# starlingonearth/MASt3R-SLAM-Quality-dualTSDF

Hardware: AMD Instinct MI355X
Metric: SLAM frames/sec (infer+match+TSDF+GN) @512x384 (higher is better)
Workload: dtype bf16

## Files before the change

include/mslam_hip.h:

```cpp
#ifndef MSLAM_HIP_H
#define MSLAM_HIP_H

#include <stddef.h>
#include <stdint.h>

#ifdef __cplusplus
extern "C" {
#endif

#define MSLAM_OK 0
#define MSLAM_EINVAL (-1)
#define MSLAM_EHIP (-2)
#define MSLAM_ENOMEM (-3)
#define MSLAM_ENODEV (-4)

const char* mslam_last_error(void);
int mslam_abi_version(void);
int mslam_device_check(void);


int mslam_iter_proj(const float* rays_img_with_grad, const float* pts_3d_norm,
                    const float* p_init, float* p_new, uint8_t* converged, int b, int h, int w,
                    int n, int max_iter, float lambda_init, float cost_thresh, void* stream);

int mslam_refine_matches(const uint16_t* D11, const uint16_t* D21, const int64_t* p1,
                         int64_t* p1_new, int b, int h, int w, int n, int fdim, int radius,
                         int dilation_max, void* stream);

int mslam_prep_iter_proj(const float* X11, const float* X21, const int64_t* idx_init,
                         float* rays_img_with_grad, float* pts_3d_norm, float* p_init, int b, int h,
                         int w, void* stream);

int mslam_match_occlusion(const float* X11, const float* X21, const float* p, int64_t* p1,
                          uint8_t* valid, int b, int h, int w, float dist_thresh, void* stream);

int mslam_pixel_to_lin(const int64_t* p1, int64_t* idx, int b, int n, int w, void* stream);

size_t mslam_gn_workspace_bytes(int num_poses, int num_edges, int num_points, int local_edges);

int mslam_gauss_newton_rays(float* Twc, const float* Xs, const float* Cs, const int64_t* ii,
                            const int64_t* jj, const int64_t* idx_ii2jj, const uint8_t* valid_match,
                            const float* Q, int num_poses, int num_points, int num_edges,
                            float sigma_ray, float sigma_dist, float C_thresh, float Q_thresh,
                            int max_iter, float delta_thresh, float* dx, void* workspace,
                            size_t workspace_bytes, void* stream);

int mslam_gauss_newton_calib(float* Twc, const float* Xs, const float* Cs, const float* K,
                             const int64_t* ii, const int64_t* jj, const int64_t* idx_ii2jj,
                             const uint8_t* valid_match, const float* Q, int num_poses, int num_points,
                             int num_edges, int height, int width, int pixel_border, float z_eps,
                             float sigma_pixel, float sigma_depth, float C_thresh, float Q_thresh,
                             int max_iter, float delta_thresh, float* dx, void* workspace,
                             size_t workspace_bytes, void* stream);

int mslam_gauss_newton_points(float* Twc, const float* Xs, const float* Cs, const int64_t* ii,
                              const int64_t* jj, const int64_t* idx_ii2jj, const uint8_t* valid_match,
                              const float* Q, int num_poses, int num_points, int num_edges,
                              float sigma_point, float C_thresh, float Q_thresh, int max_iter,
                              float delta_thresh, float* dx, void* workspace, size_t workspace_bytes,
                              void* stream);

int mslam_gn_begin(const int64_t* ii, const int64_t* jj, int num_poses, int num_edges, int num_points,
                   void* workspace, size_t workspace_bytes, void* stream);
int mslam_gn_compact(const float* Xs, const float* Cs, const int64_t* idx_ii2jj, const uint8_t* valid_match,
                     const float* Q, int num_poses, int num_points, int num_edges, int edge_begin,
                     int edge_count, float C_thresh, float Q_thresh, void* workspace, size_t workspace_bytes,
                     void* stream);
int mslam_gn_compact_at(const float* Xs, const float* Cs, const int64_t* idx_ii2jj, const uint8_t* valid_match,
                        const float* Q, int num_poses, int num_points, int num_edges, int edge_begin, int edge_count,
                        int slot_begin, int range_count, float C_thresh, float Q_thresh, void* workspace,
                        size_t workspace_bytes, void* stream);
int mslam_gn_accumulate(int kind, const float* Twc, const float* K, int num_poses, int num_points,
                        int num_edges, int edge_begin, int edge_count, float sigma_a, float sigma_b,
                        int height, int width, int pixel_border, float z_eps, float* Hs, float* gs,
                        void* workspace, size_t workspace_bytes, void* stream);
int mslam_gn_solve_retract(const float* Hs, const float* gs, int num_poses, int num_edges,
                           int num_points, float* Twc, float* dx, float delta_thresh, void* workspace,
                           size_t workspace_bytes, void* stream);
int mslam_gn_status(int* status4, int num_poses, int num_edges, int num_points, void* workspace,
                    size_t workspace_bytes, void* stream);

int mslam_sim3_act(const float* T, const float* X, float* Y, int num_poses, long long pts_per_pose,
                   int broadcast_pose, void* stream);
int mslam_sim3_op(int op, const float* A, const float* B, float* out, int n, int bcast_a, int bcast_b,
                  void* stream);

size_t mslam_tsdf_table_bytes(uint64_t capacity);
int mslam_tsdf_table_init(void* table, size_t table_bytes, uint64_t capacity, void* stream);

size_t mslam_tsdf_integrate_workspace_bytes(int n_points, double voxel_size, double trunc, double step_scale);
int mslam_tsdf_integrate(void* table, uint64_t capacity, const float* points_world, const double* conf,
                         const float* cam_origin, int n_points, double voxel_size, double trunc,
                         double max_weight, double step_scale, int shard_id, int num_shards,
                         void* workspace, size_t workspace_bytes, void* stream);

int mslam_tsdf_rehash(void* old_table, uint64_t old_capacity, void* new_table, uint64_t new_capacity, void* stream);
int mslam_tsdf_header(void* table, uint64_t capacity, uint32_t* out8_host, void* stream);

int mslam_tsdf_dump(void* table, uint64_t capacity, int64_t* keys, double* tsdf, double* weight,
                    uint32_t max_out, void* stream);

int mslam_tsdf_query(void* table, uint64_t capacity, const float* points, int n, double voxel_size,
                     double min_weight, double* value, double* grad, uint8_t* status, void* stream);

int mslam_tsdf_pose_step(void* table, uint64_t capacity, const float* points, const float* conf, int n,
                         float* pose, int points_in_camera_frame, double voxel_size, double min_weight,
                         double lambda, double damping, int update_pose, double* H_out, double* b_out,
                         int* used_out, void* workspace, size_t workspace_bytes, void* stream);

int mslam_tsdf_lookup7(void* table, uint64_t capacity, const float* points, int n, const float* pose,
                       double voxel_size, double* out, void* stream);
int mslam_tsdf_query_lookup(const double* lookup, int n, double voxel_size, double min_weight, double* value,
                            double* grad, uint8_t* status, void* stream);
int mslam_tsdf_pose_step_lookup(const double* lookup, const float* points, const float* conf, int n, float* pose,
                                int points_in_camera_frame, double voxel_size, double min_weight, double lambda,
                                double damping, int update_pose, double* H_out, double* b_out, int* used_out,
                                void* workspace, size_t workspace_bytes, void* stream);

size_t mslam_tsdf_mesh_workspace_bytes(uint64_t capacity);
int mslam_tsdf_mesh_keys(void* table, uint64_t capacity, double min_weight, int64_t* sort_keys, void* stream);
int mslam_tsdf_mesh_count(void* table, uint64_t capacity, double min_weight, double level, const int64_t* sorted_keys,
                          const int64_t* order, int32_t* counts, void* workspace, size_t workspace_bytes, void* stream);
int mslam_tsdf_mesh_emit(void* table, uint64_t capacity, double voxel_size, double min_weight, double level,
                         const int64_t* sorted_keys, const int64_t* order, const int64_t* vbase, const int64_t* fbase,
                         void* workspace, size_t workspace_bytes, float* vertices, float* normals, int32_t* faces,
                         int64_t n_vertices, int64_t n_faces, void* stream);
int mslam_tsdf_load(void* table, uint64_t capacity, const int64_t* keys, const double* tsdf, const double* weight,
                    int n, void* stream);

size_t mslam_tsdf_render_workspace_bytes(uint64_t capacity);
int mslam_tsdf_render_blocks(void* table, uint64_t capacity, double min_weight, void* workspace, size_t workspace_bytes,
                             void* stream);
int mslam_tsdf_render(void* table, uint64_t capacity, const float* rays, int h, int w, const float* pose8,
                      double voxel_size, double min_weight, double level, double near, double far, double step, int skip,
                      const void* workspace, size_t workspace_bytes, float* range, float* normal, uint8_t* hit,
                      void* stream);

size_t mslam_tsdf_color_bytes(uint64_t capacity);
int mslam_tsdf_color_init(void* color, size_t color_bytes, uint64_t capacity, void* stream);
int mslam_tsdf_integrate_color(void* table, uint64_t capacity, void* color, const float* points_world,
                               const double* conf, const float* rgb, const float* cam_origin, int n_points,
                               double voxel_size, double trunc, double step_scale, void* stream);
int mslam_tsdf_color_rehash(void* old_table, uint64_t old_capacity, const void* old_color, void* new_table,
                            uint64_t new_capacity, void* new_color, void* stream);
int mslam_tsdf_color_dump(void* table, uint64_t capacity, const void* color, const int64_t* keys, int n, uint64_t* sums,
                          void* stream);
int mslam_tsdf_color_load(void* table, uint64_t capacity, void* color, const int64_t* keys, const uint64_t* sums, int n,
                          void* stream);
int mslam_tsdf_color_sample(void* table, uint64_t capacity, const void* color, const float* points, int n, int image_w,
                            double voxel_size, double default_r, double default_g, double default_b, float* out_rgb,
                            uint8_t* out_count, void* stream);

int mslam_mast3r_create(void** handle_out, const int* cfg9_host, void* const* weight_ptrs_host,
                        const long long* weight_numels_host, int n_weights, void* stream);
int mslam_mast3r_destroy(void* handle);
size_t mslam_mast3r_workspace_bytes(void* handle, int batch, int H, int W);

int mslam_mast3r_encode(void* handle, const float* img, int batch, int H, int W, float* feat_out,
                        void* workspace, size_t workspace_bytes, void* stream);

int mslam_mast3r_decode(void* handle, const float* feat1, const float* feat2, int batch, int H, int W,
                        float* X1, float* C1, float* D1, float* Q1, float* X2, float* C2, float* D2,
                        float* Q2, float* dec_last1, float* dec_last2, void* workspace,
                        size_t workspace_bytes, void* stream);

size_t mslam_track_workspace_bytes(int n_points);
int mslam_track_pose(int use_calib, float* T_rel, const float* Xf, const float* Xk, const int64_t* idx_f2k,
                     const float* Qk, const uint8_t* valid, int n_points, const float* K, int width,
                     int height, float sigma_a, float sigma_b, float huber, int pixel_border, float z_eps,
                     int first_iter, int max_iters, float rel_error, float delta_norm, void* status_out, void* workspace,
                     size_t workspace_bytes, void* stream);

size_t mslam_track_prepare_workspace_bytes(int n_points);
int mslam_track_prepare(const int64_t* idx_f2k, const uint8_t* valid_match, const float* Qff, const float* Qkf,
                        const float* Cf_sum, float inv_nf, const float* Ck_sum, float inv_nk, float C_conf, float Q_conf,
                        int n_points, const float* T_WCk, const float* T_WCf, float* Qk, float* Ck_avg,
                        uint8_t* valid_opt, uint8_t* valid_kf, float* T_rel, void* workspace, size_t workspace_bytes,
                        void* stream);
int mslam_track_verdict(const void* prepare_workspace, const void* status, int n_points, float* verdict6, void* stream);
int mslam_track_fuse(const float* T_WCk, const float* T_rel, const float* Xkf, const float* Ckf, const float* X_canon,
                     const float* C, int n_points, float* T_WCf, float* X_new, float* C_new, void* stream);

int mslam_gemm_bf16(const void* A, const void* W, const float* bias, const void* residual_f32, void* out,
                    int M, int N, int K, int act, int out_is_bf16, void* stream);
int mslam_gemm_tile_override(int M, int N, int K, int cfg);
int mslam_gemm_profile_begin(int M, int N, int K, int max_samples);
int mslam_gemm_profile_end(double* avg_us, double* min_us, int* samples);
int mslam_conv2d_nhwc_bf16(const void* in, const void* W, const float* bias, const void* residual_bf16,
                           void* out_bf16, int B, int H, int Wd, int Cin, int Cout, int ks, int stride,
                           int relu_in, int act, void* stream);
int mslam_attention_bf16(const void* Q, const void* K, const void* VT, void* O, int batch, int heads,
                         int nq, int nk, void* stream);
int mslam_layernorm_f32(const float* x, const float* w, const float* b, void* out_bf16, float* out_f32,
                        int rows, int D, float eps, void* stream);

size_t mslam_tsdf_local_workspace_bytes(int n_points);
int mslam_tsdf_local_build(const float* X_world, const float* C, const float* origin, const float* xyz_min,
                           const float* xyz_max, int n_points, int nx, int ny, int nz, double voxel_size,
                           double trunc, float min_confidence, float* tsdf, float* weights, void* workspace,
                           size_t workspace_bytes, void* stream);
int mslam_tsdf_local_raycast(const float* tsdf, int nx, int ny, int nz, const float* xyz_min,
                             const float* xyz_max, const float* X_original, const int64_t* sel_pix, int n_sel,
                             int n_samples, float max_displacement, float* surf, uint8_t* hit, void* stream);

int mslam_quality_reduce_grid(const float* x, const float* y, const uint8_t* valid, int h, int w, int ps, int mode,
                              double c_thr, double q_thr, float* out, void* stream);
int mslam_quality_classify(const float* delta_cov, const float* r, const float* u, int n, float thr_zr, float thr_zu,
                           float thr_dc, int64_t* cls, float* pri, void* stream);

int mslam_room_pair(const float* ki, const float* kj, int batch, int h, int w, int n_frames, double fx, double fy,
                    double cx, double cy, double noise, const double* Wm_3x24, const double* phase_24, float* X1,
                    float* C1, float* D1, float* Q1, float* X2, float* C2, float* D2, float* Q2, void* stream);

int mslam_remap_bilinear_u8(const uint8_t* src, int src_h, int src_w, int channels, const float* mapx,
                            const float* mapy, uint8_t* dst, int dst_h, int dst_w, void* stream);

int mslam_gemm_f64(const void* A, int a_is_f32, const void* B, int b_is_f32, int b_transposed, const double* centre,
                   const double* bias, double* out, int M, int N, int K, void* stream);

int mslam_asmk_aggregate(const float* des, const float* centroids, const int64_t* assign, const int64_t* uniq_words,
                         uint32_t* sig_out, int n_des, int m_assign, int dim, int n_uniq, int n_centroids, void* stream);
int mslam_asmk_search(const int32_t* entry_word, const uint32_t* entry_sig, const int32_t* img_start, int n_images,
                      const int32_t* q_words, const uint32_t* q_sig, int n_q, int sig_words, float similarity_threshold,
                      float alpha, double* scores, void* stream);

#ifdef __cplusplus
}
#endif
#endif
```

mast3r-slam-quality-dualtsdf_amd/csrc/gemm.h:

```cpp
#pragma once
#include <hip/hip_runtime.h>
#include <stdint.h>

namespace mslam {

typedef __bf16 bf16;

enum GemmAct { ACT_NONE = 0, ACT_GELU = 1, ACT_RELU = 2 };
enum GemmKind { KIND_NONE = 0, KIND_F32 = 1, KIND_BF16 = 2 };
enum GemmEpi {
  EPI_PLAIN = 0,
  EPI_ATTN = 1,
  EPI_CONVT = 2,
};

struct GemmArgs {
  const bf16* A;
  const bf16* W;
  int M, N, K;
  int lda;
  int a_conv, cB, cH, cW, cC, cKs, cStride, cPad, cHo, cWo;
  int a_relu;
  const float* bias;
  int act;
  const void* res1; int res1_kind; int ldr1;
  const void* res2; int res2_kind; int ldr2;
  void* out; int out_kind; int ldc;
  int epi;
  bf16* q_out; bf16* k_out; bf16* vt_out;
  int sec_base;
  int sec_dim;
  int heads;
  int ntok;
  int tok_w;
  int kv_ntok;
  const float* rope_cos; const float* rope_sin;
  float q_scale;
  int ct_s, ct_cout, ct_h, ct_w;
  int groups;
  const bf16* W1; const float* bias1;
  size_t a_gstride;
  size_t out_gbytes, res1_gbytes, res2_gbytes;
  size_t qkv_gstride;
  const void* pf_ptr[2]; size_t pf_bytes[2];
  unsigned* pf_sink;
};

constexpr int kGemmPrefetchBlocks = 64;

int launch_gemm(const GemmArgs& a, hipStream_t stream);
int gemm_profile_begin(int M, int N, int K, int max_samples);
int gemm_profile_end(double* avg_us, double* min_us, int* samples);
int gemm_tile_override(int M, int N, int K, int cfg, bool conv);

}
```

mast3r-slam-quality-dualtsdf_amd/csrc/gemm.hip:

```cpp
#include <stdlib.h>
#include <mutex>
#include <unordered_map>
#include <vector>
#include "common.h"
#include "gemm.h"

namespace mslam {

int launch_gemm_t64(const GemmArgs& a, int stages, hipStream_t s);
int launch_gemm_t128(const GemmArgs& a, int waves, int stages, hipStream_t s);
int launch_gemm_t128x64(const GemmArgs& a, int stages, hipStream_t s);
int launch_gemm_t256(const GemmArgs& a, int bn, hipStream_t s);
int launch_gemm_t192(const GemmArgs& a, hipStream_t s);
int launch_gemm_t256w8(const GemmArgs& a, hipStream_t s);
int launch_gemm_8p(const GemmArgs& a, hipStream_t s);
bool gemm8p_supports(const GemmArgs& a);

static std::mutex g_tile_mu;
static inline uint64_t tile_key(int M, int N, int K, bool conv = false) {
  return (uint64_t)M | ((uint64_t)N << 22) | ((uint64_t)K << 42) | ((uint64_t)conv << 63);
}
static std::unordered_map<uint64_t, int> g_tile_override = {
    {tile_key(3072, 3072, 1024), 1262},
    {tile_key(3072, 768, 3072), 643},
    {tile_key(6144, 3072, 768), 1282},
    {tile_key(3072, 4096, 1024), 2192},
    {tile_key(6144, 4096, 1024), 1282},
    {tile_key(9216, 4096, 1024), 1282},
    {tile_key(9216, 1024, 4096), 8256},
    {tile_key(4608, 4096, 1024), 1282},
};

int gemm_tile_override(int M, int N, int K, int cfg, bool conv) {
  std::lock_guard<std::mutex> lk(g_tile_mu);
  if (cfg > 0) g_tile_override[tile_key(M, N, K, conv)] = cfg;
  else g_tile_override.erase(tile_key(M, N, K, conv));
  return 0;
}

static std::mutex g_prof_mu;
static struct {
  bool on = false;
  int M = 0, N = 0, K = 0, cap = 0, n = 0;
  std::vector<hipEvent_t> ev;
} g_prof;

int gemm_profile_begin(int M, int N, int K, int max_samples) {
  std::lock_guard<std::mutex> lk(g_prof_mu);
  MSLAM_REQUIRE(!g_prof.on, "gemm_profile_begin: already profiling");
  MSLAM_REQUIRE(max_samples > 0 && max_samples <= 65536, "gemm_profile_begin: max_samples out of range");
  g_prof.ev.resize(2 * (size_t)max_samples);
  for (auto& e : g_prof.ev) {
    int rc = check_hip(hipEventCreate(&e), "hipEventCreate");
    if (rc) return rc;
  }
  g_prof.M = M; g_prof.N = N; g_prof.K = K; g_prof.cap = max_samples; g_prof.n = 0;
  g_prof.on = true;
  return MSLAM_OK;
}

int gemm_profile_end(double* avg_us, double* min_us, int* samples) {
  std::lock_guard<std::mutex> lk(g_prof_mu);
  MSLAM_REQUIRE(g_prof.on, "gemm_profile_end: not profiling");
  g_prof.on = false;
  double sum = 0.0, mn = 1e30;
  int rc = MSLAM_OK;
  for (int i = 0; i < g_prof.n && !rc; i++) {
    float ms = 0.0f;
    rc = check_hip(hipEventSynchronize(g_prof.ev[2 * i + 1]), "hipEventSynchronize");
    if (!rc) rc = check_hip(hipEventElapsedTime(&ms, g_prof.ev[2 * i], g_prof.ev[2 * i + 1]), "hipEventElapsedTime");
    sum += 1e3 * ms;
    if (1e3 * ms < mn) mn = 1e3 * ms;
  }
  if (samples) *samples = g_prof.n;
  if (avg_us) *avg_us = g_prof.n ? sum / g_prof.n : 0.0;
  if (min_us) *min_us = g_prof.n ? mn : 0.0;
  for (auto& e : g_prof.ev) (void)hipEventDestroy(e);
  g_prof.ev.clear();
  return rc;
}

static int launch_gemm_impl(const GemmArgs& a, hipStream_t stream);

int launch_gemm(const GemmArgs& a, hipStream_t stream) {
  int slot = -1;
  if (g_prof.on) {
    std::lock_guard<std::mutex> lk(g_prof_mu);
    if (g_prof.on && !a.a_conv && a.groups <= 1 && a.M == g_prof.M && a.N == g_prof.N && a.K == g_prof.K &&
        g_prof.n < g_prof.cap) {
      slot = g_prof.n++;
      (void)hipEventRecord(g_prof.ev[2 * slot], stream);
    }
  }
  const int rc = launch_gemm_impl(a, stream);
  if (slot >= 0) (void)hipEventRecord(g_prof.ev[2 * slot + 1], stream);
  return rc;
}

static int launch_gemm_impl(const GemmArgs& a, hipStream_t stream) {
  MSLAM_REQUIRE(a.M > 0 && a.N > 0 && a.K > 0, "gemm: empty problem %dx%dx%d", a.M, a.N, a.K);
  MSLAM_REQUIRE(a.K % 8 == 0, "gemm: K=%d must be a multiple of 8", a.K);
  MSLAM_REQUIRE(!a.a_conv || a.cC % 8 == 0, "gemm: conv channels %d must be a multiple of 8", a.cC);
  MSLAM_REQUIRE(a.a_conv || a.lda % 8 == 0, "gemm: lda=%d must be a multiple of 8", a.lda);
  MSLAM_REQUIRE(!a.a_relu || a.a_conv, "gemm: ReLU-on-load is only built for the implicit-conv view");
  MSLAM_REQUIRE(((uintptr_t)a.A & 15) == 0 && ((uintptr_t)a.W & 15) == 0, "gemm: A and W must be 16-byte aligned");
  const size_t a_bytes = a.a_conv ? (size_t)a.cB * a.cH * a.cW * a.cC * 2 : ((size_t)(a.M - 1) * a.lda + a.K) * 2;
  MSLAM_REQUIRE(a_bytes < (1ull << 31) && (size_t)a.N * a.K * 2 < (1ull << 31), "gemm: operand larger than 2 GiB");
  MSLAM_REQUIRE(a.epi != EPI_ATTN || (a.sec_dim % 64 == 0 && a.ntok % 4 == 0 && a.kv_ntok % 4 == 0),
                "gemm: attention epilogue needs 64-wide heads and token counts divisible by 4");
  static int forced = -2;
  if (forced == -2) {
    const char* e = getenv("MSLAM_GEMM");
    forced = e ? atoi(e) : -1;
  }
  MSLAM_REQUIRE(a.groups <= 2 && (a.groups < 2 || (a.W1 && !a.a_conv)), "gemm: bad group description");
  const long ngrp = a.groups > 1 ? 2 : 1;
  auto blocks = [&](int bm, int bn) { return ngrp * ((a.M + bm - 1) / bm) * ((a.N + bn - 1) / bn); };
  int cfg = forced;
  if (cfg < 0 && a.groups <= 1 && a.M < (1 << 22) && a.N < (1 << 20) && a.K < (1 << 20)) {
    static const bool log_shapes = getenv("MSLAM_GEMM_LOG") != nullptr;
    static std::unordered_map<uint64_t, int> seen;
    std::lock_guard<std::mutex> lk(g_tile_mu);
    const uint64_t key = tile_key(a.M, a.N, a.K, a.a_conv != 0);
    auto it = g_tile_override.find(key);
    if (it != g_tile_override.end()) cfg = it->second;
    if (log_shapes && seen.emplace(key, 1).second) fprintf(stderr, "mslam_gemm_shape conv=%d %d %d %d\n", (int)(a.a_conv != 0), a.M, a.N, a.K);
  }
  if (cfg < 0) {
    const bool narrow = a.N <= 128 || (a.N > 256 && a.N <= 384);
    if (narrow && blocks(256, 128) >= 128) cfg = 2128;
    else if (blocks(256, 256) >= 128) cfg = 2256;
    else if (blocks(128, 128) >= 256) cfg = 1282;
    else if (blocks(64, 64) >= 512) cfg = 642;
    else if (a.K >= 2048) cfg = 644;
    else cfg = 643;
  }
  switch (cfg) {
    case 642: return launch_gemm_t64(a, 2, stream);
    case 643: return launch_gemm_t64(a, 3, stream);
    case 644: return launch_gemm_t64(a, 4, stream);
    case 1262: return launch_gemm_t128x64(a, 2, stream);
    case 1263: return launch_gemm_t128x64(a, 3, stream);
    case 1242: return launch_gemm_t128(a, 4, 2, stream);
    case 1282: return launch_gemm_t128(a, 8, 2, stream);
    case 1283: return launch_gemm_t128(a, 8, 3, stream);
    case 2128: return launch_gemm_t256(a, 128, stream);
    case 2256: return launch_gemm_t256(a, 256, stream);
    case 2192: return launch_gemm_t192(a, stream);
    case 2258: return launch_gemm_t256w8(a, stream);
    case 8256: return gemm8p_supports(a) ? launch_gemm_8p(a, stream) : launch_gemm_t256(a, 256, stream);
    default: MSLAM_REQUIRE(false, "gemm: unknown configuration %d", cfg);
  }
}

}
```

mast3r-slam-quality-dualtsdf_amd/csrc/gemm_kernel.h:

```cpp
#pragma once
#include <stdlib.h>
#include <type_traits>
#include <utility>
#include "common.h"
#include "gemm.h"

namespace mslam {

typedef __attribute__((ext_vector_type(8))) __bf16 bf16x8;
typedef __attribute__((ext_vector_type(8))) short short8;
typedef __attribute__((ext_vector_type(16))) float f32x16;
typedef __attribute__((ext_vector_type(4))) unsigned int u32x4_t;

constexpr int BK = 64;
#ifndef MSLAM_GEMM_ABLATE
#define MSLAM_GEMM_ABLATE 0
#endif
constexpr unsigned kOob = 0x80000000u;

#define MSLAM_LDS_PTR(p) ((__attribute__((address_space(3))) void*)(p))

__device__ __forceinline__ float bf16_to_f32(bf16 v) { return (float)v; }

template <int... Is, typename F>
__device__ __forceinline__ void static_for_impl(std::integer_sequence<int, Is...>, F&& f) {
  (f(std::integral_constant<int, Is>{}), ...);
}
template <int N, typename F>
__device__ __forceinline__ void static_for(F&& f) {
  static_for_impl(std::make_integer_sequence<int, N>{}, f);
}

__device__ __forceinline__ float gelu_erf(float x) {
  const float z = fabsf(x) * 0.70710678118654752f;
  const float t = __builtin_amdgcn_rcpf(fmaf(0.3275911f, z, 1.0f));
  float p = fmaf(1.061405429f, t, -1.453152027f);
  p = fmaf(p, t, 1.421413741f);
  p = fmaf(p, t, -0.284496736f);
  p = fmaf(p, t, 0.254829592f);
  const float erfc_z = p * t * __builtin_amdgcn_exp2f(-1.4426950408889634f * z * z);
  const float one_plus_erf = (x >= 0.0f) ? 2.0f - erfc_z : erfc_z;
  return 0.5f * x * one_plus_erf;
}

typedef __attribute__((ext_vector_type(2))) float f32x2;
__device__ __forceinline__ f32x2 gelu_erf2(f32x2 x) {
  const f32x2 ax = __builtin_elementwise_abs(x);
  const f32x2 z = ax * 0.70710678118654752f;
  const f32x2 den = __builtin_elementwise_fma(f32x2{0.3275911f, 0.3275911f}, z, f32x2{1.0f, 1.0f});
  const f32x2 t = {__builtin_amdgcn_rcpf(den[0]), __builtin_amdgcn_rcpf(den[1])};
  f32x2 p = __builtin_elementwise_fma(f32x2{1.061405429f, 1.061405429f}, t, f32x2{-1.453152027f, -1.453152027f});
  p = __builtin_elementwise_fma(p, t, f32x2{1.421413741f, 1.421413741f});
  p = __builtin_elementwise_fma(p, t, f32x2{-0.284496736f, -0.284496736f});
  p = __builtin_elementwise_fma(p, t, f32x2{0.254829592f, 0.254829592f});
  const f32x2 a = (z * -1.4426950408889634f) * z;
  const f32x2 e = {__builtin_amdgcn_exp2f(a[0]), __builtin_amdgcn_exp2f(a[1])};
  const f32x2 erfc_z = (p * t) * e;
  const f32x2 two_minus = f32x2{2.0f, 2.0f} - erfc_z;
  const f32x2 one_plus_erf = {x[0] >= 0.0f ? two_minus[0] : erfc_z[0], x[1] >= 0.0f ? two_minus[1] : erfc_z[1]};
  return (x * 0.5f) * one_plus_erf;
}

template <int N>
__device__ __forceinline__ void wait_vmcnt() {
  static_assert(N >= 0 && N < 64, "vmcnt is 6 bits");
  __builtin_amdgcn_s_waitcnt((N & 15) | ((N >> 4) << 14) | 0x0F70);
}

template <int WM, int WN, int MI, int NI, int S, bool CONV>
__global__ __launch_bounds__(64 * WM * WN) void gemm_bf16_kernel(GemmArgs g) {
  constexpr int NW = WM * WN;
  constexpr int BM = 32 * MI * WM, BN = 32 * NI * WN;
  static_assert(NW % 2 == 0 && BM % (8 * NW) == 0 && BN % (8 * NW) == 0, "DMA pieces must divide over the waves");
  constexpr int A_PC = BM / (8 * NW), B_PC = BN / (8 * NW);
  constexpr int N_DMA = A_PC + B_PC;
  constexpr int STAGE = (BM + BN) * 128;
  static_assert(S >= 2 && S <= 8, "ring depth");
  static_assert(N_DMA * (S - 1) < 64, "vmcnt range");
  extern __shared__ __attribute__((aligned(1024))) unsigned char smem[];

  const unsigned nbm = (g.M + BM - 1) / BM, nbn = (g.N + BN - 1) / BN;
  const unsigned ngrp = g.groups > 1 ? 2u : 1u;
  if (blockIdx.x >= nbm * nbn * ngrp) {
    typedef __attribute__((ext_vector_type(4))) unsigned int u32x4;
    const unsigned pb = blockIdx.x - nbm * nbn * ngrp, npb = gridDim.x - nbm * nbn * ngrp;
    u32x4 acc = {0u, 0u, 0u, 0u};
#pragma unroll
    for (int r = 0; r < 2; r++) {
      const char* base = reinterpret_cast<const char*>(g.pf_ptr[r]);
      const size_t bytes = g.pf_bytes[r] & ~(size_t)15;
      const size_t stride = (size_t)npb * (64 * NW) * 16;
      size_t off = ((size_t)pb * (64 * NW) + threadIdx.x) * 16;
      for (; off + 15 * stride < bytes; off += 16 * stride) {
        u32x4 v[16];
#pragma unroll
        for (int k = 0; k < 16; k++) v[k] = *reinterpret_cast<const u32x4*>(base + off + k * stride);
#pragma unroll
        for (int k = 0; k < 16; k++) acc ^= v[k];
      }
      for (; off < bytes; off += stride) acc ^= *reinterpret_cast<const u32x4*>(base + off);
    }
    if ((acc[0] ^ acc[1]) == 0x9e3779b9u && (acc[2] ^ acc[3]) == 0x7f4a7c15u && g.pf_sink) *g.pf_sink = acc[0];
    return;
  }
  const unsigned logical = xcd_remap(blockIdx.x, nbm * nbn * ngrp);
  const unsigned prob = logical / (nbm * nbn), tile = logical - prob * (nbm * nbn);
  if (prob) {
    g.A += g.a_gstride; g.W = g.W1; g.bias = g.bias1;
    g.out = reinterpret_cast<char*>(g.out) + g.out_gbytes;
    if (g.res1) g.res1 = reinterpret_cast<const char*>(g.res1) + g.res1_gbytes;
    if (g.res2) g.res2 = reinterpret_cast<const char*>(g.res2) + g.res2_gbytes;
    if (g.epi == EPI_ATTN) { g.q_out += g.qkv_gstride; g.k_out += g.qkv_gstride; g.vt_out += g.qkv_gstride; }
  }
  constexpr unsigned GM = 1024 / BM;
  const unsigned per_group = GM * nbn, grp = tile / per_group, in_grp = tile - grp * per_group;
  const unsigned gsz = min(nbm - grp * GM, GM);
  const int m0 = (grp * GM + in_grp % gsz) * BM, n0 = (in_grp / gsz) * BN;

  const int t = threadIdx.x, lane = t & 63;
  const int wid = __builtin_amdgcn_readfirstlane(t >> 6);
  const int wm = wid / WN, wn = wid % WN;

  const int lcol = lane & 31;
  float bias_v[NI];
#pragma unroll
  for (int ni = 0; ni < NI; ni++) {
    const int col = n0 + wn * NI * 32 + ni * 32 + lcol;
    bias_v[ni] = (g.bias && col < g.N) ? g.bias[g.epi == EPI_CONVT ? col / (g.ct_s * g.ct_s) : col] : 0.0f;
  }

  const int chunk = (lane & 7) ^ (4 * (wid & 1) + (lane >> 4));
  const size_t a_bytes = CONV ? (size_t)g.cB * g.cH * g.cW * g.cC * 2 : ((size_t)(g.M - 1) * g.lda + g.K) * 2;
  const __amdgpu_buffer_rsrc_t rsA = __builtin_amdgcn_make_buffer_rsrc((void*)g.A, 0, (int)a_bytes, 0x00020000);
  const __amdgpu_buffer_rsrc_t rsW =
      __builtin_amdgcn_make_buffer_rsrc((void*)g.W, 0, (int)((size_t)g.N * g.K * 2), 0x00020000);
  unsigned a_off[A_PC];
  int a_iy0[A_PC], a_ix0[A_PC];
#pragma unroll
  for (int i = 0; i < A_PC; i++) {
    const int m = m0 + (wid + NW * i) * 8 + (lane >> 3);
    if constexpr (CONV) {
      const int hw = g.cHo * g.cWo;
      const int b = m / hw, rem = m - b * hw;
      const int oy = rem / g.cWo, ox = rem - oy * g.cWo;
      a_iy0[i] = (m < g.M) ? oy * g.cStride - g.cPad : -(1 << 20);
      a_ix0[i] = ox * g.cStride - g.cPad;
      a_off[i] = (unsigned)b * (unsigned)(g.cH * g.cW * g.cC) * 2u;
    } else {
      a_off[i] = (m < g.M) ? ((unsigned)m * (unsigned)g.lda + (unsigned)chunk * 8u) * 2u : kOob;
      a_iy0[i] = a_ix0[i] = 0;
    }
  }
  unsigned b_off[B_PC];
#pragma unroll
  for (int i = 0; i < B_PC; i++) {
    const int n = n0 + (wid + NW * i) * 8 + (lane >> 3);
    b_off[i] = (n < g.N) ? ((unsigned)n * (unsigned)g.K + (unsigned)chunk * 8u) * 2u : kOob;
  }
  int c_cc = 0, c_dy = 0, c_dx = 0;
  if constexpr (CONV) {
    const int kk = chunk * 8, tap = kk / g.cC;
    c_cc = kk - tap * g.cC;
    c_dy = tap / g.cKs;
    c_dx = tap - c_dy * g.cKs;
  }

  const int nk = (g.K + BK - 1) / BK;
  auto issue = [&](int st, int kt) {
    if (MSLAM_GEMM_ABLATE == 1 && kt >= S - 1) return;
    unsigned char* sbase = smem + st * STAGE + wid * 1024;
    const int k0 = kt * BK;
    const unsigned k_bad = (unsigned)(g.K - 1 - (k0 + chunk * 8)) & kOob;
#pragma unroll
    for (int i = 0; i < A_PC; i++) {
      unsigned off;
      if constexpr (CONV) {
        const int iy = a_iy0[i] + c_dy, ix = a_ix0[i] + c_dx;
        const unsigned bad = (unsigned)(iy | (g.cH - 1 - iy) | ix | (g.cW - 1 - ix)) & kOob;
        off = (a_off[i] + (unsigned)((iy * g.cW + ix) * g.cC + c_cc) * 2u) | bad | k_bad;
      } else {
        off = (a_off[i] + (unsigned)k0 * 2u) | k_bad;
      }
      __builtin_amdgcn_raw_ptr_buffer_load_lds(rsA, MSLAM_LDS_PTR(sbase + i * (NW * 1024)), 16, off, 0, 0, 0);
    }
#pragma unroll
    for (int i = 0; i < B_PC; i++) {
      const unsigned off = (b_off[i] + (unsigned)k0 * 2u) | k_bad;
      __builtin_amdgcn_raw_ptr_buffer_load_lds(rsW, MSLAM_LDS_PTR(sbase + BM * 128 + i * (NW * 1024)), 16, off, 0, 0, 0);
    }
    if constexpr (CONV) {
      c_cc += BK;
      while (c_cc >= g.cC) {
        c_cc -= g.cC;
        if (++c_dx == g.cKs) { c_dx = 0; c_dy++; }
      }
    }
  };

  f32x16 acc[MI][NI];
#pragma unroll
  for (int mi = 0; mi < MI; mi++)
#pragma unroll
    for (int ni = 0; ni < NI; ni++)
#pragma unroll
      for (int r = 0; r < 16; r++) acc[mi][ni][r] = 0.0f;
#if MSLAM_GEMM_ABLATE == 4
  typedef __attribute__((ext_vector_type(4))) float f32x4q;
  f32x4q acc4[MI][NI][4];
#pragma unroll
  for (int mi = 0; mi < MI; mi++)
#pragma unroll
    for (int ni = 0; ni < NI; ni++)
#pragma unroll
      for (int r = 0; r < 4; r++) acc4[mi][ni][r] = f32x4q{0.0f, 0.0f, 0.0f, 0.0f};
#endif

  const int lr = lane & 31, kh = (lane >> 5) ^ ((lr >> 1) & 7);
  const unsigned fragA = (wm * MI * 32 + lr) * 128, fragB = BM * 128 + (wn * NI * 32 + lr) * 128;
  const bool relu_a = g.a_relu != 0;
  auto compute = [&](int st) {
    const unsigned char* sA = smem + st * STAGE + fragA;
    const unsigned char* sB = smem + st * STAGE + fragB;
    constexpr int KS = BK / 16, KG = (NW >= 16) ? 2 : KS;
#pragma unroll
    for (int kg = 0; kg < KS; kg += KG) {
      bf16x8 af[KG][MI], bfr[KG][NI];
#pragma unroll
      for (int k = 0; k < KG; k++) {
        const int so = ((2 * (kg + k)) ^ kh) * 16;
#pragma unroll
        for (int mi = 0; mi < MI; mi++) {
          if (MSLAM_GEMM_ABLATE == 3) af[k][mi] = __builtin_bit_cast(bf16x8, u32x4_t{(unsigned)so, 1u, 2u, 3u});
          else af[k][mi] = *reinterpret_cast<const bf16x8*>(sA + mi * 4096 + so);
        }
#pragma unroll
        for (int ni = 0; ni < NI; ni++) {
          if (MSLAM_GEMM_ABLATE == 3) bfr[k][ni] = __builtin_bit_cast(bf16x8, u32x4_t{(unsigned)so, 5u, 6u, 7u});
          else bfr[k][ni] = *reinterpret_cast<const bf16x8*>(sB + ni * 4096 + so);
        }
      }
      __builtin_amdgcn_sched_barrier(0);
#pragma unroll
      for (int k = 0; k < KG; k++) {
#pragma unroll
        for (int mi = 0; mi < MI; mi++) {
          if (CONV && relu_a) {
            const short8 z = {0, 0, 0, 0, 0, 0, 0, 0};
            af[k][mi] = __builtin_bit_cast(bf16x8, __builtin_elementwise_max(__builtin_bit_cast(short8, af[k][mi]), z));
          }
#pragma unroll
          for (int ni = 0; ni < NI; ni++) {
            if (MSLAM_GEMM_ABLATE == 2) {
              asm volatile("" ::"v"(af[k][mi]), "v"(bfr[k][ni]));
#if MSLAM_GEMM_ABLATE == 4
            } else if (true) {
              acc4[mi][ni][2 * (k & 1)] = __builtin_amdgcn_mfma_f32_16x16x32_bf16(af[k][mi], bfr[k][ni], acc4[mi][ni][2 * (k & 1)], 0, 0, 0);
              acc4[mi][ni][2 * (k & 1) + 1] = __builtin_amdgcn_mfma_f32_16x16x32_bf16(af[k][mi], bfr[k][ni], acc4[mi][ni][2 * (k & 1) + 1], 0, 0, 0);
#endif
            } else {
              acc[mi][ni] = __builtin_amdgcn_mfma_f32_32x32x16_bf16(af[k][mi], bfr[k][ni], acc[mi][ni], 0, 0, 0);
            }
          }
        }
      }
      if (kg + KG < KS) __builtin_amdgcn_sched_barrier(0);
    }
  };

#pragma unroll
  for (int s = 0; s < S - 1; s++)
    if (s < nk) issue(s, s);
  int kt = 0, st = 0, st_issue = S - 1;
  for (; kt < nk - (S - 2); kt++) {
    wait_vmcnt<N_DMA * (S - 2)>();
    __builtin_amdgcn_s_barrier();
    if (kt + S - 1 < nk) issue(st_issue, kt + S - 1);
    compute(st);
    st = (st + 1 == S) ? 0 : st + 1;
    st_issue = (st_issue + 1 == S) ? 0 : st_issue + 1;
  }
  for (; kt < nk; kt++) {
    const int behind = nk - 1 - kt;
    bool waited = false;
    if constexpr (S >= 4) {
      static_for<S - 3>([&](auto j_c) {
        constexpr int b = decltype(j_c)::value + 1;
        if (behind == b) { wait_vmcnt<N_DMA * b>(); waited = true; }
      });
    }
    if (!waited) wait_vmcnt<0>();
    __builtin_amdgcn_s_barrier();
    compute(st);
    st = (st + 1 == S) ? 0 : st + 1;
  }

#if MSLAM_GEMM_ABLATE == 4
#pragma unroll
  for (int mi = 0; mi < MI; mi++)
#pragma unroll
    for (int ni = 0; ni < NI; ni++)
#pragma unroll
      for (int r = 0; r < 16; r++) acc[mi][ni][r] = acc4[mi][ni][r >> 2][r & 3];
#endif
  __builtin_amdgcn_s_barrier();
  constexpr int TBS = 40;
  float* tb = reinterpret_cast<float*>(smem) + wid * (32 * TBS);
  typedef __attribute__((ext_vector_type(8))) __bf16 bf16x8s;
  const int half = lane >> 5;
  const int lrow0 = lane >> 2, lc = (lane & 3) * 8;
  const bool wide_plain = g.epi == EPI_PLAIN && (g.N & 7) == 0 && (g.ldc & 7) == 0 && (g.ldr1 & 7) == 0 && (g.ldr2 & 7) == 0;
  const bool wide_attn = g.epi == EPI_ATTN && (g.ntok & 31) == 0 && (g.kv_ntok & 31) == 0;
  auto load8 = [&](const void* base, int kind, size_t idx, float (&o)[8]) {
    if (kind == KIND_F32) {
      const float4 p = *reinterpret_cast<const float4*>(reinterpret_cast<const float*>(base) + idx);
      const float4 q = *reinterpret_cast<const float4*>(reinterpret_cast<const float*>(base) + idx + 4);
      o[0] += p.x; o[1] += p.y; o[2] += p.z; o[3] += p.w; o[4] += q.x; o[5] += q.y; o[6] += q.z; o[7] += q.w;
    } else if (kind == KIND_BF16) {
      const bf16x8s p = *reinterpret_cast<const bf16x8s*>(reinterpret_cast<const bf16*>(base) + idx);
#pragma unroll
      for (int e = 0; e < 8; e++) o[e] += (float)p[e];
    }
  };
  static_for<MI>([&](auto mi_c) {
    static_for<NI>([&](auto ni_c) {
      constexpr int mi = decltype(mi_c)::value, ni = decltype(ni_c)::value;
      const f32x16 accv = acc[mi][ni];
      const int col_base = n0 + wn * NI * 32 + ni * 32;
      const int col = col_base + lcol;
      const int row_base0 = m0 + wm * MI * 32 + mi * 32;
      const int row_base = row_base0 + 4 * half;
      const bool col_ok = col < g.N;
      const float bias = bias_v[ni];
      float v[16];
      static_for<8>([&](auto r_c) {
        constexpr int r = 2 * decltype(r_c)::value;
        f32x2 x = {accv[r] + bias, accv[r + 1] + bias};
        if (g.act == ACT_GELU) x = gelu_erf2(x);
        else if (g.act == ACT_RELU) x = __builtin_elementwise_max(x, f32x2{0.0f, 0.0f});
        v[r] = x[0]; v[r + 1] = x[1];
      });
      if (wide_plain) {
        static_for<16>([&](auto r_c) {
          constexpr int r = decltype(r_c)::value;
          tb[((r & 3) + 8 * (r >> 2) + 4 * half) * TBS + lcol] = v[r];
        });
#pragma unroll
        for (int j = 0; j < 2; j++) {
          const int lrow = lrow0 + 16 * j;
          const float4 p = *reinterpret_cast<const float4*>(tb + lrow * TBS + lc);
          const float4 q = *reinterpret_cast<const float4*>(tb + lrow * TBS + lc + 4);
          const int row = row_base0 + lrow, c0 = col_base + lc;
          if (row < g.M && c0 < g.N) {
            float o[8] = {p.x, p.y, p.z, p.w, q.x, q.y, q.z, q.w};
            load8(g.res1, g.res1_kind, (size_t)row * g.ldr1 + c0, o);
            load8(g.res2, g.res2_kind, (size_t)row * g.ldr2 + c0, o);
            if (g.out_kind == KIND_F32) {
              float* dst = reinterpret_cast<float*>(g.out) + (size_t)row * g.ldc + c0;
              *reinterpret_cast<float4*>(dst) = make_float4(o[0], o[1], o[2], o[3]);
              *reinterpret_cast<float4*>(dst + 4) = make_float4(o[4], o[5], o[6], o[7]);
            } else {
              bf16x8s pk;
#pragma unroll
              for (int e = 0; e < 8; e++) pk[e] = (bf16)o[e];
              *reinterpret_cast<bf16x8s*>(reinterpret_cast<bf16*>(g.out) + (size_t)row * g.ldc + c0) = pk;
            }
          }
        }
      } else if (wide_attn) {
        const int sec = g.sec_base + col_base / g.sec_dim;
        const int cs = col_base % g.sec_dim;
        const int head = cs >> 6, f0 = cs & 63;
        const int ntok = (sec == 0) ? g.ntok : g.kv_ntok;
        const int b = row_base0 / ntok, nb = row_base0 - b * ntok;
        if (sec < 2) {
          const bool use_y = f0 < 32;
          const bool lo = lcol < 16;
          const float scale = (sec == 0) ? g.q_scale : 1.0f;
          static_for<16>([&](auto r_c) {
            constexpr int r = decltype(r_c)::value;
            const int n = nb + 4 * half + (r & 3) + 8 * (r >> 2);
            const float partner = __shfl_xor(v[r], 16, 64);
            const int p = use_y ? n / g.tok_w : n % g.tok_w;
            const float c = g.rope_cos[p * 16 + (lcol & 15)], sn = g.rope_sin[p * 16 + (lcol & 15)];
            const float x = lo ? (v[r] * c - partner * sn) : (v[r] * c + partner * sn);
            tb[((r & 3) + 8 * (r >> 2) + 4 * half) * TBS + lcol] = x * scale;
          });
          bf16* dst = (sec == 0) ? g.q_out : g.k_out;
#pragma unroll
          for (int j = 0; j < 2; j++) {
            const int lrow = lrow0 + 16 * j;
            const float4 p = *reinterpret_cast<const float4*>(tb + lrow * TBS + lc);
            const float4 q = *reinterpret_cast<const float4*>(tb + lrow * TBS + lc + 4);
            if (row_base0 + lrow < g.M && col_base < g.N) {
              bf16x8s pk;
              pk[0] = (bf16)p.x; pk[1] = (bf16)p.y; pk[2] = (bf16)p.z; pk[3] = (bf16)p.w;
              pk[4] = (bf16)q.x; pk[5] = (bf16)q.y; pk[6] = (bf16)q.z; pk[7] = (bf16)q.w;
              *reinterpret_cast<bf16x8s*>(dst + (((size_t)b * g.heads + head) * ntok + nb + lrow) * 64 + f0 + lc) = pk;
            }
          }
        } else {
          static_for<16>([&](auto r_c) {
            constexpr int r = decltype(r_c)::value;
            tb[((r & 3) + 8 * (r >> 2) + 4 * half) * TBS + lcol] = v[r];
          });
          const int tok0 = half * 16;
          if (row_base0 + tok0 < g.M && col_ok) {
            bf16x8s pk0, pk1;
#pragma unroll
            for (int e = 0; e < 8; e++) {
              pk0[e] = (bf16)tb[(tok0 + e) * TBS + lcol];
              pk1[e] = (bf16)tb[(tok0 + 8 + e) * TBS + lcol];
            }
            bf16* dst = g.vt_out + (((size_t)b * g.heads + head) * 64 + f0 + lcol) * ntok + nb + tok0;
            *reinterpret_cast<bf16x8s*>(dst) = pk0;
            *reinterpret_cast<bf16x8s*>(dst + 8) = pk1;
          }
        }
      } else {
        if (g.epi == EPI_PLAIN) {
          static_for<16>([&](auto r_c) {
            constexpr int r = decltype(r_c)::value;
            const int row = row_base + (r & 3) + 8 * (r >> 2);
            if (row < g.M && col_ok) {
              float x = v[r];
              if (g.res1_kind == KIND_F32) x += reinterpret_cast<const float*>(g.res1)[(size_t)row * g.ldr1 + col];
              else if (g.res1_kind == KIND_BF16) x += bf16_to_f32(reinterpret_cast<const bf16*>(g.res1)[(size_t)row * g.ldr1 + col]);
              if (g.res2_kind == KIND_F32) x += reinterpret_cast<const float*>(g.res2)[(size_t)row * g.ldr2 + col];
              else if (g.res2_kind == KIND_BF16) x += bf16_to_f32(reinterpret_cast<const bf16*>(g.res2)[(size_t)row * g.ldr2 + col]);
              if (g.out_kind == KIND_F32) reinterpret_cast<float*>(g.out)[(size_t)row * g.ldc + col] = x;
              else reinterpret_cast<bf16*>(g.out)[(size_t)row * g.ldc + col] = (bf16)x;
            }
          });
        } else if (g.epi == EPI_ATTN) {
          const int sec = g.sec_base + col / g.sec_dim;
          const int cs = col % g.sec_dim;
          const int head = cs >> 6, f = cs & 63;
          const int ntok = (sec == 0) ? g.ntok : g.kv_ntok;
          if (sec < 2) {
            const bool use_y = f < 32;
            const bool lo = (f & 31) < 16;
            bf16* dst = (sec == 0) ? g.q_out : g.k_out;
            const float scale = (sec == 0) ? g.q_scale : 1.0f;
            static_for<16>([&](auto r_c) {
              constexpr int r = decltype(r_c)::value;
              const int row = row_base + (r & 3) + 8 * (r >> 2);
              const float partner = __shfl_xor(v[r], 16, 64);
              if (row < g.M && col_ok) {
                const int b = row / ntok, n = row - b * ntok;
                const int p = use_y ? n / g.tok_w : n % g.tok_w;
                const float c = g.rope_cos[p * 16 + (f & 15)], sn = g.rope_sin[p * 16 + (f & 15)];
                const float x = lo ? (v[r] * c - partner * sn) : (v[r] * c + partner * sn);
                dst[(((size_t)b * g.heads + head) * ntok + n) * 64 + f] = (bf16)(x * scale);
              }
            });
          } else {
            static_for<4>([&](auto gq_c) {
              constexpr int gq = decltype(gq_c)::value;
              const int row = row_base + 8 * gq;
              if (row < g.M && col_ok) {
                const int b = row / ntok, n = row - b * ntok;
                typedef __attribute__((ext_vector_type(4))) __bf16 bf16x4;
                bf16x4 pk;
                pk[0] = (bf16)v[4 * gq + 0]; pk[1] = (bf16)v[4 * gq + 1];
                pk[2] = (bf16)v[4 * gq + 2]; pk[3] = (bf16)v[4 * gq + 3];
                *reinterpret_cast<bf16x4*>(g.vt_out + (((size_t)b * g.heads + head) * 64 + f) * ntok + n) = pk;
              }
            });
          }
        } else {
          const int ss = g.ct_s * g.ct_s;
          const int co = col / ss, ij = col - co * ss, i = ij / g.ct_s, j = ij - i * g.ct_s;
          static_for<16>([&](auto r_c) {
            constexpr int r = decltype(r_c)::value;
            const int row = row_base + (r & 3) + 8 * (r >> 2);
            if (row < g.M && col_ok) {
              const int hw = g.ct_h * g.ct_w;
              const int b = row / hw, rem = row - b * hw, y = rem / g.ct_w, x = rem - y * g.ct_w;
              const size_t o = (((size_t)b * g.ct_h * g.ct_s + (size_t)y * g.ct_s + i) * (g.ct_w * g.ct_s) +
                                (size_t)x * g.ct_s + j) * g.ct_cout + co;
              reinterpret_cast<bf16*>(g.out)[o] = (bf16)v[r];
            }
          });
        }
      }
    });
  });
}


template <int WM, int WN, int MI, int NI, int S>
int launch_cfg(const GemmArgs& a, hipStream_t stream) {
  constexpr int NW = WM * WN, BM = 32 * MI * WM, BN = 32 * NI * WN;
  constexpr size_t ring = (size_t)S * (BM + BN) * 128, patch = (size_t)NW * 32 * 40 * sizeof(float);
  constexpr size_t shmem = ring > patch ? ring : patch;
  static_assert(shmem <= 160 * 1024, "LDS budget");
  const unsigned blocks = (unsigned)(((a.M + BM - 1) / BM) * ((a.N + BN - 1) / BN)) * (a.groups > 1 ? 2u : 1u) +
                          ((a.pf_bytes[0] + a.pf_bytes[1]) ? (unsigned)kGemmPrefetchBlocks : 0u);
  static bool attr_set = false;
  if (!attr_set) {
    const void* fns[2] = {(const void*)gemm_bf16_kernel<WM, WN, MI, NI, S, false>,
                          (const void*)gemm_bf16_kernel<WM, WN, MI, NI, S, true>};
    for (const void* fn : fns) {
      int rc = check_hip(hipFuncSetAttribute(fn, hipFuncAttributeMaxDynamicSharedMemorySize, (int)shmem), "gemm: attr");
      if (rc) return rc;
    }
    attr_set = true;
  }
  if (!a.a_conv)
    hipLaunchKernelGGL((gemm_bf16_kernel<WM, WN, MI, NI, S, false>), dim3(blocks), dim3(64 * NW), shmem, stream, a);
  else
    hipLaunchKernelGGL((gemm_bf16_kernel<WM, WN, MI, NI, S, true>), dim3(blocks), dim3(64 * NW), shmem, stream, a);
  return check_hip(hipGetLastError(), "gemm launch");
}

}
```

mast3r-slam-quality-dualtsdf_amd/csrc/gemm_t256.hip:

```cpp
#include "gemm_kernel.h"
namespace mslam {
int launch_gemm_t192(const GemmArgs& a, hipStream_t s) { return launch_cfg<2, 4, 3, 2, 2>(a, s); }

int launch_gemm_t256w8(const GemmArgs& a, hipStream_t s) { return launch_cfg<2, 4, 4, 2, 2>(a, s); }

int launch_gemm_t256(const GemmArgs& a, int bn, hipStream_t s) {
  if (bn == 256) return launch_cfg<4, 4, 2, 2, 2>(a, s);
  return launch_cfg<4, 2, 2, 2, 2>(a, s);
}
}
```

mast3r-slam-quality-dualtsdf_amd/csrc/mast3r.hip:

```cpp
#include <stdlib.h>
#include <vector>
#include "common.h"
#include "gemm.h"

namespace mslam {

int launch_attention(const bf16* Q, const bf16* K, const bf16* VT, bf16* O, int batch, int heads, int nq, int nk,
                     hipStream_t stream);

template <typename TIN>
__global__ __launch_bounds__(256) void layernorm_kernel(const TIN* __restrict__ x, const float* __restrict__ w,
                                                        const float* __restrict__ b, bf16* __restrict__ out_bf,
                                                        float* __restrict__ out_f, int rows, int D, float eps) {
  constexpr int MAXV = 32;
  const int row = blockIdx.x * 4 + (threadIdx.x >> 6);
  const int lane = threadIdx.x & 63;
  if (row >= rows) return;
  const TIN* xr = x + (size_t)row * D;
  float v[MAXV];
  float s = 0.0f;
#pragma unroll
  for (int c = 0; c < MAXV; c++) {
    const int i = lane + 64 * c;
    v[c] = (i < D) ? (float)xr[i] : 0.0f;
    s += v[c];
  }
#pragma unroll
  for (int off = 32; off > 0; off >>= 1) s += __shfl_xor(s, off, 64);
  const float mean = s / (float)D;
  float q = 0.0f;
#pragma unroll
  for (int c = 0; c < MAXV; c++) {
    const float d = (lane + 64 * c < D) ? v[c] - mean : 0.0f;
    q += d * d;
  }
#pragma unroll
  for (int off = 32; off > 0; off >>= 1) q += __shfl_xor(q, off, 64);
  const float rstd = rsqrtf(q / (float)D + eps);
#pragma unroll
  for (int c = 0; c < MAXV; c++) {
    const int i = lane + 64 * c;
    if (i < D) {
      const float y = (v[c] - mean) * rstd * w[i] + b[i];
      if (out_bf) out_bf[(size_t)row * D + i] = (bf16)y;
      if (out_f) out_f[(size_t)row * D + i] = y;
    }
  }
}

typedef __attribute__((ext_vector_type(4))) __bf16 bf16x4;

template <int NV>
__device__ __forceinline__ void ln_load_stats(const float* xrow, int lane, float4 (&v)[NV], float& mean, float& rstd,
                                              float eps) {
  constexpr int D = NV * 256;
  const float4* xr = reinterpret_cast<const float4*>(xrow);
#pragma unroll
  for (int c = 0; c < NV; c++) v[c] = xr[lane + 64 * c];
  float s = 0.0f;
#pragma unroll
  for (int c = 0; c < NV; c++) s += (v[c].x + v[c].y) + (v[c].z + v[c].w);
#pragma unroll
  for (int off = 32; off > 0; off >>= 1) s += __shfl_xor(s, off, 64);
  mean = s / (float)D;
  float q = 0.0f;
#pragma unroll
  for (int c = 0; c < NV; c++) {
    const float dx = v[c].x - mean, dy = v[c].y - mean, dz = v[c].z - mean, dw = v[c].w - mean;
    q += (dx * dx + dy * dy) + (dz * dz + dw * dw);
  }
#pragma unroll
  for (int off = 32; off > 0; off >>= 1) q += __shfl_xor(q, off, 64);
  rstd = rsqrtf(q / (float)D + eps);
}

__device__ __forceinline__ float4 ln_affine(const float4& v, float mean, float rstd, const float4& w, const float4& b) {
  float4 y;
  y.x = (v.x - mean) * rstd * w.x + b.x;
  y.y = (v.y - mean) * rstd * w.y + b.y;
  y.z = (v.z - mean) * rstd * w.z + b.z;
  y.w = (v.w - mean) * rstd * w.w + b.w;
  return y;
}

__device__ __forceinline__ void ln_store_bf16(bf16* out_row, int idx, const float4& y) {
  bf16x4 o;
  o[0] = (bf16)y.x; o[1] = (bf16)y.y; o[2] = (bf16)y.z; o[3] = (bf16)y.w;
  reinterpret_cast<bf16x4*>(out_row)[idx] = o;
}

template <int NV>
__global__ __launch_bounds__(256) void layernorm_vec_kernel(const float* __restrict__ x, const float* __restrict__ w,
                                                            const float* __restrict__ b, bf16* __restrict__ out_bf,
                                                            float* __restrict__ out_f, int rows, float eps) {
  constexpr int D = NV * 256;
  const int row = blockIdx.x * 4 + (threadIdx.x >> 6);
  const int lane = threadIdx.x & 63;
  if (row >= rows) return;
  float4 v[NV], wv[NV], bv[NV];
  float mean, rstd;
#pragma unroll
  for (int c = 0; c < NV; c++) {
    wv[c] = reinterpret_cast<const float4*>(w)[lane + 64 * c];
    bv[c] = reinterpret_cast<const float4*>(b)[lane + 64 * c];
  }
  ln_load_stats<NV>(x + (size_t)row * D, lane, v, mean, rstd, eps);
#pragma unroll
  for (int c = 0; c < NV; c++) {
    const float4 y = ln_affine(v[c], mean, rstd, wv[c], bv[c]);
    if (out_bf) ln_store_bf16(out_bf + (size_t)row * D, lane + 64 * c, y);
    if (out_f) reinterpret_cast<float4*>(out_f + (size_t)row * D)[lane + 64 * c] = y;
  }
}

struct LnSet { const float* w; const float* b; };

template <int NV, bool CROSS>
__global__ __launch_bounds__(256) void layernorm_group_vec_kernel(const float* __restrict__ x, LnSet self0, LnSet self1,
                                                                  LnSet mem0, LnSet mem1, bf16* __restrict__ out_self,
                                                                  bf16* __restrict__ out_mem, int M, float eps) {
  constexpr int D = NV * 256;
  const int row = blockIdx.x * 4 + (threadIdx.x >> 6);
  const int lane = threadIdx.x & 63;
  if (row >= 2 * M) return;
  const int side = row >= M;
  float4 v[NV];
  float mean, rstd;
  ln_load_stats<NV>(x + (size_t)row * D, lane, v, mean, rstd, eps);
#pragma unroll
  for (int k = 0; k < (CROSS ? 2 : 1); k++) {
    const LnSet ps = (k == 0) ? (side ? self1 : self0) : (side ? mem0 : mem1);
    bf16* out = (k == 0) ? out_self + (size_t)row * D : out_mem + (size_t)(side ? row - M : row + M) * D;
#pragma unroll
    for (int c = 0; c < NV; c++) {
      const float4 wv = reinterpret_cast<const float4*>(ps.w)[lane + 64 * c];
      const float4 bv = reinterpret_cast<const float4*>(ps.b)[lane + 64 * c];
      ln_store_bf16(out, lane + 64 * c, ln_affine(v[c], mean, rstd, wv, bv));
    }
  }
}

static void launch_layernorm(const float* x, const float* w, const float* b, bf16* out_bf, float* out_f, int rows, int D,
                             float eps, hipStream_t s) {
  const dim3 grid((rows + 3) / 4), block(256);
  if (D == 1024) hipLaunchKernelGGL(layernorm_vec_kernel<4>, grid, block, 0, s, x, w, b, out_bf, out_f, rows, eps);
  else if (D == 768) hipLaunchKernelGGL(layernorm_vec_kernel<3>, grid, block, 0, s, x, w, b, out_bf, out_f, rows, eps);
  else hipLaunchKernelGGL(layernorm_kernel<float>, grid, block, 0, s, x, w, b, out_bf, out_f, rows, D, eps);
}

__global__ void cast_f32_bf16_kernel(const float* __restrict__ x, bf16* __restrict__ y, size_t n) {
  const size_t i = ((size_t)blockIdx.x * blockDim.x + threadIdx.x) * 4;
  if (i + 3 < n) {
    const float4 v = *reinterpret_cast<const float4*>(x + i);
    bf16x4 o;
    o[0] = (bf16)v.x; o[1] = (bf16)v.y; o[2] = (bf16)v.z; o[3] = (bf16)v.w;
    *reinterpret_cast<bf16x4*>(y + i) = o;
  } else {
    for (size_t k = i; k < n; k++) y[k] = (bf16)x[k];
  }
}

__global__ void patchify_kernel(const float* __restrict__ img, bf16* __restrict__ out, int B, int H, int W, int P) {
  const int nh = H / P, nw = W / P, K = 3 * P * P;
  const size_t total = (size_t)B * nh * nw * K;
  const size_t i = (size_t)blockIdx.x * blockDim.x + threadIdx.x;
  if (i >= total) return;
  const int k = (int)(i % K);
  const size_t tok = i / K;
  const int tx = (int)(tok % nw), ty = (int)((tok / nw) % nh), b = (int)(tok / ((size_t)nw * nh));
  const int c = k / (P * P), ky = (k / P) % P, kx = k % P;
  out[i] = (bf16)img[(((size_t)b * 3 + c) * H + ty * P + ky) * W + tx * P + kx];
}

__global__ void concat2_kernel(const bf16* __restrict__ a, int ca, const bf16* __restrict__ b, int cb,
                               bf16* __restrict__ out, size_t rows) {
  const int C = ca + cb;
  const size_t i = (size_t)blockIdx.x * blockDim.x + threadIdx.x;
  if (i >= rows * C) return;
  const size_t r = i / C;
  const int c = (int)(i % C);
  out[i] = c < ca ? a[r * ca + c] : b[r * cb + (c - ca)];
}

__global__ void upsample2x_kernel(const bf16* __restrict__ in, bf16* __restrict__ out, int B, int H, int W, int C) {
  const int Ho = 2 * H, Wo = 2 * W;
  const int c8 = C / 8;
  const size_t total = (size_t)B * Ho * Wo * c8;
  const size_t i = (size_t)blockIdx.x * blockDim.x + threadIdx.x;
  if (i >= total) return;
  const int cc = (int)(i % c8) * 8;
  const size_t pix = i / c8;
  const int ox = (int)(pix % Wo), oy = (int)((pix / Wo) % Ho), b = (int)(pix / ((size_t)Wo * Ho));
  const float sy = Ho > 1 ? (float)(H - 1) / (float)(Ho - 1) : 0.0f;
  const float sx = Wo > 1 ? (float)(W - 1) / (float)(Wo - 1) : 0.0f;
  const float fy = sy * oy, fx = sx * ox;
  const int y0 = min((int)fy, H - 1), x0 = min((int)fx, W - 1);
  const int y1 = min(y0 + 1, H - 1), x1 = min(x0 + 1, W - 1);
  const float wy = fy - y0, wx = fx - x0;
  typedef __attribute__((ext_vector_type(8))) __bf16 bf16x8;
  const bf16* base = in + (size_t)b * H * W * C + cc;
  const bf16x8 v00 = *reinterpret_cast<const bf16x8*>(base + ((size_t)y0 * W + x0) * C);
  const bf16x8 v01 = *reinterpret_cast<const bf16x8*>(base + ((size_t)y0 * W + x1) * C);
  const bf16x8 v10 = *reinterpret_cast<const bf16x8*>(base + ((size_t)y1 * W + x0) * C);
  const bf16x8 v11 = *reinterpret_cast<const bf16x8*>(base + ((size_t)y1 * W + x1) * C);
  bf16x8 o;
#pragma unroll
  for (int k = 0; k < 8; k++) {
    const float top = (float)v00[k] + wx * ((float)v01[k] - (float)v00[k]);
    const float bot = (float)v10[k] + wx * ((float)v11[k] - (float)v10[k]);
    o[k] = (bf16)(top + wy * (bot - top));
  }
  *reinterpret_cast<bf16x8*>(out + pix * C + cc) = o;
}

constexpr int kHP = 16;
__global__ __launch_bounds__(256) void head_post_kernel(const bf16* __restrict__ feat, int fc,
                                                        const float* __restrict__ w4, const float* __restrict__ b4,
                                                        const float* __restrict__ lf, int lf_ld, int desc_dim,
                                                        int B, int H, int W, float* __restrict__ X,
                                                        float* __restrict__ Cf, float* __restrict__ D,
                                                        float* __restrict__ Q) {
  typedef __attribute__((ext_vector_type(8))) __bf16 bf16x8;
  __shared__ float l_s[kHP * kHP][4];
  __shared__ __attribute__((aligned(16))) float d_s[kHP * kHP * 24];
  __shared__ __attribute__((aligned(16))) float x_s[kHP * kHP * 3];
  const int t = threadIdx.x;
  const int nw = W / kHP, nh = H / kHP;
  const int tok = blockIdx.x;
  const int b = tok / (nh * nw), ty = (tok / nw) % nh, tx = tok % nw;
  const size_t pix00 = ((size_t)b * H + (size_t)ty * kHP) * W + (size_t)tx * kHP;
  const int cg = t & 15, ppx = t >> 4;
  float wr[4][8];
#pragma unroll
  for (int o = 0; o < 4; o++)
#pragma unroll
    for (int k = 0; k < 8; k++) wr[o][k] = w4[o * fc + cg * 8 + k];
  for (int r = 0; r < kHP; r++) {
    const bf16x8 v = *reinterpret_cast<const bf16x8*>(feat + (pix00 + (size_t)r * W + ppx) * fc + cg * 8);
    float p[4] = {0.0f, 0.0f, 0.0f, 0.0f};
#pragma unroll
    for (int k = 0; k < 8; k++) {
      const float fv = (float)v[k];
#pragma unroll
      for (int o = 0; o < 4; o++) p[o] = fmaf(wr[o][k], fv, p[o]);
    }
#pragma unroll
    for (int off = 8; off > 0; off >>= 1)
#pragma unroll
      for (int o = 0; o < 4; o++) p[o] += __shfl_xor(p[o], off, 64);
    if (cg == 0) {
#pragma unroll
      for (int o = 0; o < 4; o++) l_s[r * kHP + ppx][o] = p[o] + b4[o];
    }
  }
  __syncthreads();
  const int py = t >> 4, px = t & 15;
  const float l0 = l_s[t][0], l1 = l_s[t][1], l2 = l_s[t][2], l3 = l_s[t][3];
  const float d = sqrtf(l0 * l0 + l1 * l1 + l2 * l2);
  const float sc = expm1f(d) / fmaxf(d, 1e-8f);
  x_s[t * 3 + 0] = l0 * sc; x_s[t * 3 + 1] = l1 * sc; x_s[t * 3 + 2] = l2 * sc;
  const size_t pix = pix00 + (size_t)py * W + px;
  Cf[pix] = 1.0f + expf(l3);
  const float* lp = lf + (size_t)tok * lf_ld + t;
  float dv[24];
  float nn = 0.0f;
#pragma unroll
  for (int c = 0; c < 24; c++) { dv[c] = lp[c * kHP * kHP]; nn = fmaf(dv[c], dv[c], nn); }
  const float inv = 1.0f / sqrtf(nn);
#pragma unroll
  for (int c = 0; c < 24; c++) d_s[t * 24 + c] = dv[c] * inv;
  Q[pix] = expf(lp[24 * kHP * kHP]);
  __syncthreads();
#pragma unroll
  for (int k = 0; k < 6; k++) {
    const int e = t + 256 * k, r = e / 96, q = e - r * 96;
    *reinterpret_cast<float4*>(D + (pix00 + (size_t)r * W) * 24 + q * 4) = *reinterpret_cast<const float4*>(d_s + r * 384 + q * 4);
  }
  if (t < 192) {
    const int r = t / 12, q = t - r * 12;
    *reinterpret_cast<float4*>(X + (pix00 + (size_t)r * W) * 3 + q * 4) = *reinterpret_cast<const float4*>(x_s + r * 48 + q * 4);
  }
}

__global__ __launch_bounds__(256) void head_post_generic_kernel(const bf16* __restrict__ feat, int fc,
                                                        const float* __restrict__ w4, const float* __restrict__ b4,
                                                        const float* __restrict__ lf, int lf_ld, int desc_dim, int P,
                                                        int B, int H, int W, float* __restrict__ X,
                                                        float* __restrict__ Cf, float* __restrict__ D,
                                                        float* __restrict__ Q) {
  const size_t pix = (size_t)blockIdx.x * 256 + threadIdx.x;
  if (pix >= (size_t)B * H * W) return;
  const int x = (int)(pix % W), y = (int)((pix / W) % H), b = (int)(pix / ((size_t)W * H));
  float l[4] = {b4[0], b4[1], b4[2], b4[3]};
  const bf16* f = feat + pix * fc;
  typedef __attribute__((ext_vector_type(8))) __bf16 bf16x8;
  for (int c = 0; c < fc; c += 8) {
    const bf16x8 v = *reinterpret_cast<const bf16x8*>(f + c);
#pragma unroll
    for (int k = 0; k < 8; k++) {
      const float fv = (float)v[k];
#pragma unroll
      for (int o = 0; o < 4; o++) l[o] = fmaf(w4[o * fc + c + k], fv, l[o]);
    }
  }
  const float d = sqrtf(l[0] * l[0] + l[1] * l[1] + l[2] * l[2]);
  const float sc = expm1f(d) / fmaxf(d, 1e-8f);
  X[pix * 3 + 0] = l[0] * sc; X[pix * 3 + 1] = l[1] * sc; X[pix * 3 + 2] = l[2] * sc;
  Cf[pix] = 1.0f + expf(l[3]);
  const int nw = W / P;
  const size_t tok = (size_t)b * (H / P) * nw + (size_t)(y / P) * nw + x / P;
  const float* lp = lf + tok * lf_ld + (y % P) * P + (x % P);
  float dv[32];
  float nn = 0.0f;
  for (int c = 0; c < desc_dim; c++) { dv[c] = lp[c * P * P]; nn = fmaf(dv[c], dv[c], nn); }
  const float inv = 1.0f / sqrtf(nn);
  for (int c = 0; c < desc_dim; c++) D[pix * desc_dim + c] = dv[c] * inv;
  Q[pix] = expf(lp[desc_dim * P * P]);
}

struct Lin { const bf16* W; const float* b; int out, in; };
struct Norm { const float* w; const float* b; int d; };

struct EncBlock { Norm n1; Lin qkv, proj; Norm n2; Lin fc1, fc2; };
struct DecBlock { Norm n1; Lin qkv, proj; Norm n2, ny; Lin pq, pkv, cproj; Norm n3; Lin fc1, fc2; };
struct Rcu { Lin c1, c2; };
struct Fusion { Rcu r1, r2; Lin out; bool has_r1; };
struct Head {
  Lin a00, a01, a10, a11, a20, a30, a31;
  Lin rn[4];
  Fusion fus[4];
  Lin h0, h2;
  const float* h4w; const float* h4b;
  Lin fc1, fc2;
};

struct Mast3rModel {
  int E, enc_depth, enc_heads, Dd, dec_depth, dec_heads, P, desc_dim, fd;
  Lin pe;
  std::vector<EncBlock> enc;
  Norm enc_norm;
  Lin dec_embed;
  std::vector<DecBlock> dec[2];
  Norm dec_norm;
  Head head[2];
  float* rope_cos = nullptr;
  float* rope_sin = nullptr;
  int rope_len = 0;
  int hooks[4];
  unsigned* pf_sink = nullptr;
  bool prefetch = true;
};

struct PtrFeed {
  void* const* ptrs;
  const long long* numels;
  int count, pos = 0;
  bool ok = true;
  void* take(long long expect, const char* what) {
    if (pos >= count) { if (ok) set_error("mast3r_create: ran out of weights at %s (#%d)", what, pos); ok = false; return nullptr; }
    if (numels[pos] != expect) {
      if (ok) set_error("mast3r_create: weight #%d (%s) has %lld elements, expected %lld", pos, what, numels[pos], expect);
      ok = false;
    }
    return ptrs[pos++];
  }
  Lin lin(int out, int in, bool bias, const char* what) {
    Lin l; l.out = out; l.in = in;
    l.W = (const bf16*)take((long long)out * in, what);
    l.b = bias ? (const float*)take(out, what) : nullptr;
    return l;
  }
  Norm norm(int d, const char* what) {
    Norm n; n.d = d;
    n.w = (const float*)take(d, what);
    n.b = (const float*)take(d, what);
    return n;
  }
};

struct Arena {
  char* base; size_t off = 0, cap; bool dry; bool overflow = false;
  size_t peak = 0;
  template <typename T> T* get(size_t n) {
    const size_t bytes = (n * sizeof(T) + 255) / 256 * 256;
    T* p = dry ? nullptr : reinterpret_cast<T*>(base + off);
    off += bytes;
    if (off > peak) peak = off;
    if (!dry && off > cap) { overflow = true; return reinterpret_cast<T*>(base); }
    return p;
  }
};

struct Ctx {
  const Mast3rModel* m;
  Arena ar;
  hipStream_t s;
  int rc = MSLAM_OK;
  bool dry() const { return ar.dry; }
  void fail(int r) { if (rc == MSLAM_OK) rc = r; }
};

static void dbg(Ctx& c, const char* what, int a = 0, int b = 0, int d = 0) {
  static const bool on = getenv("MSLAM_DEBUG") != nullptr;
  if (!on || c.dry()) return;
  fprintf(stderr, "[mslam] %s %d %d %d ...", what, a, b, d);
  fflush(stderr);
  hipError_t e = hipStreamSynchronize(c.s);
  fprintf(stderr, " %s\n", hipGetErrorString(e));
}

static void run_gemm(Ctx& c, GemmArgs& g) {
  if (c.dry() || c.rc) return;
  c.fail(launch_gemm(g, c.s));
  dbg(c, g.epi == EPI_ATTN ? "gemm_attn" : (g.a_conv ? "gemm_conv" : "gemm"), g.M, g.N, g.K);
}

struct Pf { const Lin* a = nullptr; const Lin* b = nullptr; };
static void set_pf(const Ctx& c, GemmArgs& g, const Pf& pf) {
  if (!c.m->prefetch) return;
  const Lin* l[2] = {pf.a, pf.b};
  for (int k = 0; k < 2; k++)
    if (l[k]) { g.pf_ptr[k] = l[k]->W; g.pf_bytes[k] = (size_t)l[k]->out * l[k]->in * sizeof(bf16); }
  g.pf_sink = c.m->pf_sink;
}

static GemmArgs dense_args(const bf16* A, int M, const Lin& l) {
  GemmArgs g = {};
  g.A = A; g.W = l.W; g.M = M; g.N = l.out; g.K = l.in; g.lda = l.in; g.bias = l.b;
  g.ldc = l.out; g.ldr1 = l.out; g.ldr2 = l.out;
  return g;
}

static void group2(GemmArgs& g, const Lin& l1, size_t a_gstride, size_t out_gbytes) {
  g.groups = 2; g.W1 = l1.W; g.bias1 = l1.b; g.a_gstride = a_gstride; g.out_gbytes = out_gbytes;
}

static void layernorm(Ctx& c, const float* x, const Norm& n, int rows, bf16* out_bf, float* out_f) {
  if (c.dry() || c.rc) return;
  launch_layernorm(x, n.w, n.b, out_bf, out_f, rows, n.d, 1e-6f, c.s);
  dbg(c, "layernorm", rows, n.d);
}

static void cast_bf16(Ctx& c, const float* x, bf16* y, size_t n) {
  if (c.dry() || c.rc) return;
  hipLaunchKernelGGL(cast_f32_bf16_kernel, dim3((unsigned)((n / 4 + 255) / 256 + 1)), dim3(256), 0, c.s, x, y, n);
  dbg(c, "cast", (int)n);
}

struct AttnBufs { bf16 *q, *k, *vt, *o; };

static void attn_project(Ctx& c, const bf16* A, int M, const Lin& l, int sec_base, int heads, int ntok, int kv_ntok,
                         int tok_w, const AttnBufs& ab, const Pf& pf = Pf(), const Lin* l1 = nullptr) {
  GemmArgs g = dense_args(A, M, l);
  set_pf(c, g, pf);
  g.epi = EPI_ATTN; g.sec_base = sec_base; g.sec_dim = heads * 64; g.heads = heads; g.ntok = ntok; g.kv_ntok = kv_ntok;
  g.tok_w = tok_w; g.q_out = ab.q; g.k_out = ab.k; g.vt_out = ab.vt; g.rope_cos = c.m->rope_cos;
  g.rope_sin = c.m->rope_sin; g.q_scale = 0.125f;
  if (l1) {
    group2(g, *l1, (size_t)M * l.in, 0);
    g.qkv_gstride = (size_t)(M / ntok) * heads * 64 * (sec_base == 0 ? ntok : kv_ntok);
  }
  run_gemm(c, g);
}

static void attention(Ctx& c, const AttnBufs& ab, int B, int heads, int nq, int nk) {
  if (c.dry() || c.rc) return;
  c.fail(launch_attention(ab.q, ab.k, ab.vt, ab.o, B, heads, nq, nk, c.s));
  dbg(c, "attention", B * heads, nq, nk);
}

static void linear_residual(Ctx& c, const bf16* A, int M, const Lin& l, float* x, const Pf& pf = Pf(),
                            const Lin* l1 = nullptr) {
  GemmArgs g = dense_args(A, M, l);
  set_pf(c, g, pf);
  g.res1 = x; g.res1_kind = KIND_F32; g.out = x; g.out_kind = KIND_F32;
  if (l1) {
    group2(g, *l1, (size_t)M * l.in, (size_t)M * l.out * sizeof(float));
    g.res1_gbytes = g.out_gbytes;
  }
  run_gemm(c, g);
}

static void linear_bf16(Ctx& c, const bf16* A, int M, const Lin& l, bf16* out, int act, const Pf& pf = Pf(),
                        const Lin* l1 = nullptr) {
  GemmArgs g = dense_args(A, M, l);
  set_pf(c, g, pf);
  g.out = out; g.out_kind = KIND_BF16; g.act = act;
  if (l1) group2(g, *l1, (size_t)M * l.in, (size_t)M * l.out * sizeof(bf16));
  run_gemm(c, g);
}

static void linear_f32(Ctx& c, const bf16* A, int M, const Lin& l, float* out) {
  GemmArgs g = dense_args(A, M, l);
  g.out = out; g.out_kind = KIND_F32;
  run_gemm(c, g);
}

struct BlockScratch { bf16* h; bf16* u; AttnBufs ab; };

static BlockScratch block_scratch(Ctx& c, int M, int D) {
  BlockScratch s;
  s.h = c.ar.get<bf16>((size_t)M * D);
  s.u = c.ar.get<bf16>((size_t)M * 4 * D);
  s.ab.q = c.ar.get<bf16>((size_t)M * D);
  s.ab.k = c.ar.get<bf16>((size_t)M * D);
  s.ab.vt = c.ar.get<bf16>((size_t)M * D);
  s.ab.o = c.ar.get<bf16>((size_t)M * D);
  return s;
}

static void mlp_residual(Ctx& c, float* x, int M, const Norm& n, const Lin& fc1, const Lin& fc2, BlockScratch& s,
                         const Pf& pf1 = Pf(), const Pf& pf2 = Pf()) {
  layernorm(c, x, n, M, s.h, nullptr);
  linear_bf16(c, s.h, M, fc1, s.u, ACT_GELU, pf1);
  linear_residual(c, s.u, M, fc2, x, pf2);
}

static void encode(Ctx& c, const float* img, int B, int H, int W, float* feat_out) {
  const Mast3rModel& m = *c.m;
  const int nh = H / m.P, nw = W / m.P, N = nh * nw, M = B * N, KP = 3 * m.P * m.P;
  bf16* patches = c.ar.get<bf16>((size_t)M * KP);
  float* x = c.ar.get<float>((size_t)M * m.E);
  BlockScratch s = block_scratch(c, M, m.E);
  if (!c.dry() && !c.rc) {
    const size_t total = (size_t)M * KP;
    hipLaunchKernelGGL(patchify_kernel, dim3((unsigned)((total + 255) / 256)), dim3(256), 0, c.s, img, patches, B, H, W,
                       m.P);
    dbg(c, "patchify", B, H, W);
  }
  linear_f32(c, patches, M, m.pe, x);
  for (int i = 0; i < m.enc_depth; i++) {
    const EncBlock& b = m.enc[i];
    const EncBlock* nb = i + 1 < m.enc_depth ? &m.enc[i + 1] : nullptr;
    layernorm(c, x, b.n1, M, s.h, nullptr);
    attn_project(c, s.h, M, b.qkv, 0, m.enc_heads, N, N, nw, s.ab, Pf{nb ? &nb->qkv : nullptr});
    attention(c, s.ab, B, m.enc_heads, N, N);
    linear_residual(c, s.ab.o, M, b.proj, x, Pf{nb ? &nb->proj : nullptr});
    mlp_residual(c, x, M, b.n2, b.fc1, b.fc2, s, Pf{nb ? &nb->fc1 : nullptr}, Pf{nb ? &nb->fc2 : nullptr});
  }
  layernorm(c, x, m.enc_norm, M, nullptr, feat_out);
}

static GemmArgs conv_args(const bf16* in, int B, int H, int W, int C, const Lin& l, int ks, int stride) {
  GemmArgs g = {};
  const int pad = ks / 2;
  const int Ho = (H + 2 * pad - ks) / stride + 1, Wo = (W + 2 * pad - ks) / stride + 1;
  g.A = in; g.W = l.W; g.M = B * Ho * Wo; g.N = l.out; g.K = ks * ks * C; g.bias = l.b;
  g.a_conv = 1; g.cB = B; g.cH = H; g.cW = W; g.cC = C; g.cKs = ks; g.cStride = stride; g.cPad = pad; g.cHo = Ho; g.cWo = Wo;
  g.ldc = l.out; g.ldr1 = l.out; g.ldr2 = l.out; g.out_kind = KIND_BF16;
  return g;
}

static bf16* conv(Ctx& c, const bf16* in, int B, int H, int W, int C, const Lin& l, int ks, int stride, int a_relu,
                  int act, const bf16* res1, const bf16* res2) {
  GemmArgs g = conv_args(in, B, H, W, C, l, ks, stride);
  bf16* out = c.ar.get<bf16>((size_t)g.M * l.out);
  g.out = out; g.a_relu = a_relu; g.act = act;
  if (res1) { g.res1 = res1; g.res1_kind = KIND_BF16; }
  if (res2) { g.res2 = res2; g.res2_kind = KIND_BF16; }
  run_gemm(c, g);
  return out;
}

static bf16* conv_transpose(Ctx& c, const bf16* in, int B, int H, int W, int C, const Lin& l, int s, int cout) {
  GemmArgs g = {};
  g.A = in; g.W = l.W; g.M = B * H * W; g.N = cout * s * s; g.K = C; g.lda = C; g.bias = l.b;
  g.epi = EPI_CONVT; g.ct_s = s; g.ct_cout = cout; g.ct_h = H; g.ct_w = W; g.out_kind = KIND_BF16;
  bf16* out = c.ar.get<bf16>((size_t)B * H * s * W * s * cout);
  g.out = out;
  run_gemm(c, g);
  return out;
}

static bf16* upsample2x(Ctx& c, const bf16* in, int B, int H, int W, int C) {
  bf16* out = c.ar.get<bf16>((size_t)B * 4 * H * W * C);
  if (!c.dry() && !c.rc) {
    const size_t total = (size_t)B * 4 * H * W * (C / 8);
    hipLaunchKernelGGL(upsample2x_kernel, dim3((unsigned)((total + 255) / 256)), dim3(256), 0, c.s, in, out, B, H, W, C);
    dbg(c, "upsample2x", H, W, C);
  }
  return out;
}

static bf16* rcu(Ctx& c, const bf16* x, int B, int H, int W, int C, const Rcu& r, const bf16* extra) {
  bf16* t = conv(c, x, B, H, W, C, r.c1, 3, 1,  1, ACT_RELU, nullptr, nullptr);
  return conv(c, t, B, H, W, C, r.c2, 3, 1, 0, ACT_NONE, x, extra);
}

static bf16* fusion(Ctx& c, const Fusion& f, const bf16* path, const bf16* layer, int B, int H, int W, int C) {
  const bf16* s = path;
  if (f.has_r1) s = rcu(c, layer, B, H, W, C, f.r1, path);
  bf16* r = rcu(c, s, B, H, W, C, f.r2, nullptr);
  bf16* o = conv(c, r, B, H, W, C, f.out, 1, 1, 0, ACT_NONE, nullptr, nullptr);
  return upsample2x(c, o, B, H, W, C);
}

struct HeadOut { float *X, *C, *D, *Q; };

static void run_head(Ctx& c, const Head& hd, const bf16* const toks[4], int B, int H, int W, const HeadOut& out) {
  const Mast3rModel& m = *c.m;
  const int nh = H / m.P, nw = W / m.P, M = B * nh * nw;
  bf16* t0 = conv(c, toks[0], B, nh, nw, m.E, hd.a00, 1, 1, 0, ACT_NONE, nullptr, nullptr);
  bf16* l0 = conv_transpose(c, t0, B, nh, nw, hd.a00.out, hd.a01, 4, hd.a00.out);
  bf16* t1 = conv(c, toks[1], B, nh, nw, m.Dd, hd.a10, 1, 1, 0, ACT_NONE, nullptr, nullptr);
  bf16* l1 = conv_transpose(c, t1, B, nh, nw, hd.a10.out, hd.a11, 2, hd.a10.out);
  bf16* l2 = conv(c, toks[2], B, nh, nw, m.Dd, hd.a20, 1, 1, 0, ACT_NONE, nullptr, nullptr);
  bf16* t3 = conv(c, toks[3], B, nh, nw, m.Dd, hd.a30, 1, 1, 0, ACT_NONE, nullptr, nullptr);
  bf16* l3 = conv(c, t3, B, nh, nw, hd.a30.out, hd.a31, 3, 2, 0, ACT_NONE, nullptr, nullptr);
  const int h3 = (nh + 2 - 3) / 2 + 1, w3 = (nw + 2 - 3) / 2 + 1;
  bf16* r0 = conv(c, l0, B, 4 * nh, 4 * nw, hd.a00.out, hd.rn[0], 3, 1, 0, ACT_NONE, nullptr, nullptr);
  bf16* r1 = conv(c, l1, B, 2 * nh, 2 * nw, hd.a10.out, hd.rn[1], 3, 1, 0, ACT_NONE, nullptr, nullptr);
  bf16* r2 = conv(c, l2, B, nh, nw, hd.a20.out, hd.rn[2], 3, 1, 0, ACT_NONE, nullptr, nullptr);
  bf16* r3 = conv(c, l3, B, h3, w3, hd.a30.out, hd.rn[3], 3, 1, 0, ACT_NONE, nullptr, nullptr);
  if (2 * h3 != nh || 2 * w3 != nw) {
    if (!c.dry()) set_error("mast3r head: token grid %dx%d must be even", nh, nw);
    c.fail(MSLAM_EINVAL);
    return;
  }
  const int fd = m.fd;
  bf16* p4 = fusion(c, hd.fus[3], r3, nullptr, B, h3, w3, fd);
  bf16* p3 = fusion(c, hd.fus[2], p4, r2, B, nh, nw, fd);
  bf16* p2 = fusion(c, hd.fus[1], p3, r1, B, 2 * nh, 2 * nw, fd);
  bf16* p1 = fusion(c, hd.fus[0], p2, r0, B, 4 * nh, 4 * nw, fd);
  bf16* h0 = conv(c, p1, B, 8 * nh, 8 * nw, fd, hd.h0, 3, 1, 0, ACT_NONE, nullptr, nullptr);
  bf16* hu = upsample2x(c, h0, B, 8 * nh, 8 * nw, hd.h0.out);
  bf16* h2 = conv(c, hu, B, H, W, hd.h0.out, hd.h2, 3, 1, 0, ACT_RELU, nullptr, nullptr);
  const int idim = m.E + m.Dd;
  bf16* cat = c.ar.get<bf16>((size_t)M * idim);
  bf16* hid = c.ar.get<bf16>((size_t)M * hd.fc1.out);
  float* lf = c.ar.get<float>((size_t)M * hd.fc2.out);
  if (!c.dry() && !c.rc) {
    const size_t total = (size_t)M * idim;
    hipLaunchKernelGGL(concat2_kernel, dim3((unsigned)((total + 255) / 256)), dim3(256), 0, c.s, toks[0], m.E, toks[3],
                       m.Dd, cat, (size_t)M);
    dbg(c, "concat2", M);
  }
  linear_bf16(c, cat, M, hd.fc1, hid, ACT_GELU);
  linear_f32(c, hid, M, hd.fc2, lf);
  if (!c.dry() && !c.rc) {
    if (m.P == kHP && hd.h2.out == 128 && m.desc_dim == 24) {
      hipLaunchKernelGGL(head_post_kernel, dim3((unsigned)(B * (H / m.P) * (W / m.P))), dim3(256), 0, c.s, h2, hd.h2.out,
                         hd.h4w, hd.h4b, lf, hd.fc2.out, m.desc_dim, B, H, W, out.X, out.C, out.D, out.Q);
    } else {
      const size_t npix = (size_t)B * H * W;
      hipLaunchKernelGGL(head_post_generic_kernel, dim3((unsigned)((npix + 255) / 256)), dim3(256), 0, c.s, h2, hd.h2.out,
                         hd.h4w, hd.h4b, lf, hd.fc2.out, m.desc_dim, m.P, B, H, W, out.X, out.C, out.D, out.Q);
    }
    dbg(c, "head_post", B, H, W);
  }
}

static void g_layernorm(Ctx& c, const float* x, const Norm& n0, const Norm& n1, int M, bf16* out) {
  if (c.dry() || c.rc) return;
  const LnSet s0{n0.w, n0.b}, s1{n1.w, n1.b};
  const dim3 grid((2 * M + 3) / 4), block(256);
  if (n0.d == 768) hipLaunchKernelGGL((layernorm_group_vec_kernel<3, false>), grid, block, 0, c.s, x, s0, s1, s0, s1, out, out, M, 1e-6f);
  else if (n0.d == 1024) hipLaunchKernelGGL((layernorm_group_vec_kernel<4, false>), grid, block, 0, c.s, x, s0, s1, s0, s1, out, out, M, 1e-6f);
  else {
    launch_layernorm(x, n0.w, n0.b, out, nullptr, M, n0.d, 1e-6f, c.s);
    launch_layernorm(x + (size_t)M * n0.d, n1.w, n1.b, out + (size_t)M * n0.d, nullptr, M, n0.d, 1e-6f, c.s);
  }
  dbg(c, "g_layernorm", M, n0.d);
}

static void g_layernorm_cross(Ctx& c, const float* x, const DecBlock& b0, const DecBlock& b1, int M, bf16* h, bf16* yn) {
  if (c.dry() || c.rc) return;
  const int D = b0.n1.d;
  const dim3 grid((2 * M + 3) / 4), block(256);
  const LnSet self0{b0.n1.w, b0.n1.b}, self1{b1.n1.w, b1.n1.b}, mem0{b0.ny.w, b0.ny.b}, mem1{b1.ny.w, b1.ny.b};
  if (D == 768) hipLaunchKernelGGL((layernorm_group_vec_kernel<3, true>), grid, block, 0, c.s, x, self0, self1, mem0, mem1, h, yn, M, 1e-6f);
  else if (D == 1024) hipLaunchKernelGGL((layernorm_group_vec_kernel<4, true>), grid, block, 0, c.s, x, self0, self1, mem0, mem1, h, yn, M, 1e-6f);
  else {
    const size_t MD = (size_t)M * D;
    launch_layernorm(x, b0.n1.w, b0.n1.b, h, nullptr, M, D, 1e-6f, c.s);
    launch_layernorm(x + MD, b1.n1.w, b1.n1.b, h + MD, nullptr, M, D, 1e-6f, c.s);
    launch_layernorm(x + MD, b0.ny.w, b0.ny.b, yn, nullptr, M, D, 1e-6f, c.s);
    launch_layernorm(x, b1.ny.w, b1.ny.b, yn + MD, nullptr, M, D, 1e-6f, c.s);
  }
  dbg(c, "g_layernorm_cross", M, D);
}

static void dec_layer_grouped(Ctx& c, const DecBlock& b0, const DecBlock& b1, const DecBlock* n0, const DecBlock* n1,
                              float* x, bf16* yn, int B, int N, int nw, BlockScratch& s) {
  const Mast3rModel& m = *c.m;
  const int M = B * N;
  const auto pf = [&](Lin DecBlock::*f) { return n0 ? Pf{&(n0->*f), &(n1->*f)} : Pf{}; };
  g_layernorm_cross(c, x, b0, b1, M, s.h, yn);
  attn_project(c, s.h, M, b0.qkv, 0, m.dec_heads, N, N, nw, s.ab, pf(&DecBlock::qkv), &b1.qkv);
  attention(c, s.ab, 2 * B, m.dec_heads, N, N);
  linear_residual(c, s.ab.o, M, b0.proj, x, pf(&DecBlock::proj), &b1.proj);
  g_layernorm(c, x, b0.n2, b1.n2, M, s.h);
  attn_project(c, s.h, M, b0.pq, 0, m.dec_heads, N, N, nw, s.ab, pf(&DecBlock::pq), &b1.pq);
  attn_project(c, yn, M, b0.pkv, 1, m.dec_heads, N, N, nw, s.ab, pf(&DecBlock::pkv), &b1.pkv);
  attention(c, s.ab, 2 * B, m.dec_heads, N, N);
  linear_residual(c, s.ab.o, M, b0.cproj, x, pf(&DecBlock::cproj), &b1.cproj);
  g_layernorm(c, x, b0.n3, b1.n3, M, s.h);
  linear_bf16(c, s.h, M, b0.fc1, s.u, ACT_GELU, pf(&DecBlock::fc1), &b1.fc1);
  linear_residual(c, s.u, M, b0.fc2, x, pf(&DecBlock::fc2), &b1.fc2);
}

static void decode(Ctx& c, const float* feat1, const float* feat2, int B, int H, int W, const HeadOut out[2],
                   float* dec_last1, float* dec_last2) {
  const Mast3rModel& m = *c.m;
  const int nh = H / m.P, nw = W / m.P, N = nh * nw, M = B * N;
  float* dec_last[2] = {dec_last1, dec_last2};
  const size_t ME = (size_t)M * m.E, MD = (size_t)M * m.Dd;
  bf16* fb_all = c.ar.get<bf16>(2 * ME);
  float* x_all = c.ar.get<float>(2 * MD);
  bf16* yn_all = c.ar.get<bf16>(2 * MD);
  bf16* tok_all[4] = {fb_all, c.ar.get<bf16>(2 * MD), c.ar.get<bf16>(2 * MD), c.ar.get<bf16>(2 * MD)};
  BlockScratch bs_all = block_scratch(c, 2 * M, m.Dd);
  cast_bf16(c, feat1, fb_all, ME);
  cast_bf16(c, feat2, c.dry() ? nullptr : fb_all + ME, ME);
  linear_f32(c, fb_all, 2 * M, m.dec_embed, x_all);
  for (int l = 0; l < m.dec_depth; l++) {
    const bool more = l + 1 < m.dec_depth;
    dec_layer_grouped(c, m.dec[0][l], m.dec[1][l], more ? &m.dec[0][l + 1] : nullptr, more ? &m.dec[1][l + 1] : nullptr,
                      x_all, yn_all, B, N, nw, bs_all);
    for (int k = 1; k < 3; k++)
      if (l + 1 == m.hooks[k]) cast_bf16(c, x_all, tok_all[k], 2 * MD);
  }
  const size_t mark = c.ar.off;
  for (int s = 0; s < 2; s++) {
    bf16* tok[4];
    for (int k = 0; k < 4; k++) tok[k] = c.dry() ? nullptr : tok_all[k] + s * (k ? MD : ME);
    layernorm(c, c.dry() ? nullptr : x_all + s * MD, m.dec_norm, M, tok[3], dec_last[s]);
    c.ar.off = mark;
    run_head(c, m.head[s], tok, B, H, W, out[s]);
  }
}

}

using namespace mslam;

extern "C" int mslam_mast3r_create(void** handle_out, const int* cfg9, void* const* weight_ptrs,
                                   const long long* weight_numels, int n_weights, void* stream) {
  MSLAM_REQUIRE(handle_out && cfg9 && weight_ptrs && weight_numels, "mast3r_create: null pointer");
  Mast3rModel* m = new Mast3rModel();
  m->E = cfg9[0]; m->enc_depth = cfg9[1]; m->enc_heads = cfg9[2]; m->Dd = cfg9[3]; m->dec_depth = cfg9[4];
  m->dec_heads = cfg9[5]; m->P = cfg9[6]; m->desc_dim = cfg9[7]; m->fd = cfg9[8];
  if (m->E != m->enc_heads * 64 || m->Dd != m->dec_heads * 64 || m->desc_dim > 31 || m->P < 1 || m->fd % 8) {
    set_error("mast3r_create: head_dim must be 64 (enc %d/%d, dec %d/%d), desc_dim <= 31", m->E, m->enc_heads, m->Dd,
              m->dec_heads);
    delete m;
    return MSLAM_EINVAL;
  }
  const int l2 = m->dec_depth;
  m->hooks[0] = 0; m->hooks[1] = l2 * 2 / 4; m->hooks[2] = l2 * 3 / 4; m->hooks[3] = l2;
  PtrFeed f{weight_ptrs, weight_numels, n_weights};
  const int E = m->E, D = m->Dd, P = m->P;
  m->pe = f.lin(E, 3 * P * P, true, "patch_embed");
  for (int i = 0; i < m->enc_depth; i++) {
    EncBlock b;
    b.n1 = f.norm(E, "enc.norm1"); b.qkv = f.lin(3 * E, E, true, "enc.qkv"); b.proj = f.lin(E, E, true, "enc.proj");
    b.n2 = f.norm(E, "enc.norm2"); b.fc1 = f.lin(4 * E, E, true, "enc.fc1"); b.fc2 = f.lin(E, 4 * E, true, "enc.fc2");
    m->enc.push_back(b);
  }
  m->enc_norm = f.norm(E, "enc_norm");
  m->dec_embed = f.lin(D, E, true, "decoder_embed");
  for (int s = 0; s < 2; s++)
    for (int i = 0; i < m->dec_depth; i++) {
      DecBlock b;
      b.n1 = f.norm(D, "dec.norm1"); b.qkv = f.lin(3 * D, D, true, "dec.qkv"); b.proj = f.lin(D, D, true, "dec.proj");
      b.n2 = f.norm(D, "dec.norm2"); b.ny = f.norm(D, "dec.norm_y");
      b.pq = f.lin(D, D, true, "dec.projq"); b.pkv = f.lin(2 * D, D, true, "dec.projkv");
      b.cproj = f.lin(D, D, true, "dec.cross_proj");
      b.n3 = f.norm(D, "dec.norm3"); b.fc1 = f.lin(4 * D, D, true, "dec.fc1"); b.fc2 = f.lin(D, 4 * D, true, "dec.fc2");
      m->dec[s].push_back(b);
    }
  m->dec_norm = f.norm(D, "dec_norm");
  const int dims[4] = {96, 192, 384, 768};
  const int fd = m->fd;
  for (int s = 0; s < 2; s++) {
    Head& h = m->head[s];
    h.a00 = f.lin(dims[0], E, true, "act0.0"); h.a01 = f.lin(dims[0] * 16, dims[0], false, "act0.1");
    h.a01.b = (const float*)f.take(dims[0], "act0.1.bias");
    h.a10 = f.lin(dims[1], D, true, "act1.0"); h.a11 = f.lin(dims[1] * 4, dims[1], false, "act1.1");
    h.a11.b = (const float*)f.take(dims[1], "act1.1.bias");
    h.a20 = f.lin(dims[2], D, true, "act2.0");
    h.a30 = f.lin(dims[3], D, true, "act3.0"); h.a31 = f.lin(dims[3], 9 * dims[3], true, "act3.1");
    for (int k = 0; k < 4; k++) h.rn[k] = f.lin(fd, 9 * dims[k], false, "layer_rn");
    for (int k = 3; k >= 0; k--) {
      Fusion& fu = h.fus[k];
      fu.has_r1 = (k != 3);
      if (fu.has_r1) { fu.r1.c1 = f.lin(fd, 9 * fd, true, "rcu1.conv1"); fu.r1.c2 = f.lin(fd, 9 * fd, true, "rcu1.conv2"); }
      fu.r2.c1 = f.lin(fd, 9 * fd, true, "rcu2.conv1"); fu.r2.c2 = f.lin(fd, 9 * fd, true, "rcu2.conv2");
      fu.out = f.lin(fd, fd, true, "out_conv");
    }
    h.h0 = f.lin(fd / 2, 9 * fd, true, "head.0"); h.h2 = f.lin(fd / 2, 9 * (fd / 2), true, "head.2");
    h.h4w = (const float*)f.take(4 * (fd / 2), "head.4.weight"); h.h4b = (const float*)f.take(4, "head.4.bias");
    const int idim = E + D;
    h.fc1 = f.lin(4 * idim, idim, true, "lf.fc1"); h.fc2 = f.lin((m->desc_dim + 1) * P * P, 4 * idim, true, "lf.fc2");
  }
  if (!f.ok) { delete m; return MSLAM_EINVAL; }
  if (f.pos != n_weights) {
    set_error("mast3r_create: %d weights supplied, %d consumed", n_weights, f.pos);
    delete m;
    return MSLAM_EINVAL;
  }
  m->rope_len = 1024;
  std::vector<float> hc((size_t)m->rope_len * 16), hs((size_t)m->rope_len * 16);
  for (int p = 0; p < m->rope_len; p++)
    for (int i = 0; i < 16; i++) {
      const float inv_freq = 1.0f / powf(100.0f, (float)(2 * i) / 32.0f);
      const float fr = (float)p * inv_freq;
      hc[(size_t)p * 16 + i] = cosf(fr);
      hs[(size_t)p * 16 + i] = sinf(fr);
    }
  int rc = check_hip(hipMalloc(&m->rope_cos, hc.size() * 4 + 16), "rope hipMalloc");
  if (!rc) m->pf_sink = reinterpret_cast<unsigned*>(m->rope_cos + hc.size());
  if (!rc) rc = check_hip(hipMalloc(&m->rope_sin, hs.size() * 4), "rope hipMalloc");
  if (!rc) rc = check_hip(hipMemcpyAsync(m->rope_cos, hc.data(), hc.size() * 4, hipMemcpyHostToDevice, (hipStream_t)stream), "rope copy");
  if (!rc) rc = check_hip(hipMemcpyAsync(m->rope_sin, hs.data(), hs.size() * 4, hipMemcpyHostToDevice, (hipStream_t)stream), "rope copy");
  if (!rc) rc = check_hip(hipStreamSynchronize((hipStream_t)stream), "rope sync");
  if (const char* e = getenv("MSLAM_PREFETCH")) m->prefetch = atoi(e) != 0;
  if (rc) { delete m; return rc; }
  *handle_out = m;
  return MSLAM_OK;
}

extern "C" int mslam_mast3r_destroy(void* handle) {
  Mast3rModel* m = (Mast3rModel*)handle;
  if (!m) return MSLAM_OK;
  if (m->rope_cos) (void)hipFree(m->rope_cos);
  if (m->rope_sin) (void)hipFree(m->rope_sin);
  delete m;
  return MSLAM_OK;
}

static int check_shape(const Mast3rModel* m, int B, int H, int W, const char* who) {
  MSLAM_REQUIRE(m, "%s: null model", who);
  MSLAM_REQUIRE(B >= 1 && H >= m->P && W >= m->P && H % m->P == 0 && W % m->P == 0,
                "%s: image %dx%d must be a positive multiple of the patch size %d", who, H, W, m->P);
  const int N = (H / m->P) * (W / m->P);
  MSLAM_REQUIRE(N % 8 == 0, "%s: token count %d must be a multiple of 8", who, N);
  MSLAM_REQUIRE(m->E <= 2048 && m->Dd <= 2048, "%s: embedding dims above 2048 unsupported", who);
  MSLAM_REQUIRE(H / m->P < m->rope_len && W / m->P < m->rope_len, "%s: token grid exceeds the RoPE table", who);
  return MSLAM_OK;
}

extern "C" size_t mslam_mast3r_workspace_bytes(void* handle, int batch, int H, int W) {
  const Mast3rModel* m = (const Mast3rModel*)handle;
  if (!m || check_shape(m, batch, H, W, "mast3r_workspace_bytes")) return 0;
  Ctx c{m, Arena{nullptr, 0, 0, true}, nullptr};
  encode(c, nullptr, batch, H, W, nullptr);
  c.ar.off = 0;
  HeadOut out[2] = {};
  decode(c, nullptr, nullptr, batch, H, W, out, nullptr, nullptr);
  return c.ar.peak + 4096;
}

extern "C" int mslam_mast3r_encode(void* handle, const float* img, int batch, int H, int W, float* feat_out,
                                   void* workspace, size_t workspace_bytes, void* stream) {
  const Mast3rModel* m = (const Mast3rModel*)handle;
  int rc = check_shape(m, batch, H, W, "mast3r_encode");
  if (rc) return rc;
  MSLAM_REQUIRE(img && feat_out && workspace, "mast3r_encode: null pointer");
  MSLAM_REQUIRE(workspace_bytes >= mslam_mast3r_workspace_bytes(handle, batch, H, W), "mast3r_encode: workspace too small");
  Ctx c{m, Arena{(char*)workspace, 0, workspace_bytes, false}, (hipStream_t)stream};
  encode(c, img, batch, H, W, feat_out);
  MSLAM_REQUIRE(!c.ar.overflow, "mast3r_encode: workspace arena overflow (%zu > %zu)", c.ar.peak, c.ar.cap);
  if (c.rc) return c.rc;
  return check_hip(hipGetLastError(), "mast3r_encode launch");
}

extern "C" int mslam_mast3r_decode(void* handle, const float* feat1, const float* feat2, int batch, int H, int W,
                                   float* X1, float* C1, float* D1, float* Q1, float* X2, float* C2, float* D2,
                                   float* Q2, float* dec_last1, float* dec_last2, void* workspace,
                                   size_t workspace_bytes, void* stream) {
  const Mast3rModel* m = (const Mast3rModel*)handle;
  int rc = check_shape(m, batch, H, W, "mast3r_decode");
  if (rc) return rc;
  MSLAM_REQUIRE(feat1 && feat2 && X1 && C1 && D1 && Q1 && X2 && C2 && D2 && Q2 && workspace, "mast3r_decode: null pointer");
  MSLAM_REQUIRE(workspace_bytes >= mslam_mast3r_workspace_bytes(handle, batch, H, W), "mast3r_decode: workspace too small");
  Ctx c{m, Arena{(char*)workspace, 0, workspace_bytes, false}, (hipStream_t)stream};
  HeadOut out[2] = {{X1, C1, D1, Q1}, {X2, C2, D2, Q2}};
  decode(c, feat1, feat2, batch, H, W, out, dec_last1, dec_last2);
  MSLAM_REQUIRE(!c.ar.overflow, "mast3r_decode: workspace arena overflow (%zu > %zu)", c.ar.peak, c.ar.cap);
  if (c.rc) return c.rc;
  return check_hip(hipGetLastError(), "mast3r_decode launch");
}

extern "C" int mslam_gemm_tile_override(int M, int N, int K, int cfg) {
  MSLAM_REQUIRE(M != 0 && N > 0 && K > 0 && cfg >= 0, "gemm_tile_override: bad arguments");
  return gemm_tile_override(M < 0 ? -M : M, N, K, cfg, M < 0);
}

extern "C" int mslam_gemm_profile_begin(int M, int N, int K, int max_samples) {
  return gemm_profile_begin(M, N, K, max_samples);
}

extern "C" int mslam_gemm_profile_end(double* avg_us, double* min_us, int* samples) {
  return gemm_profile_end(avg_us, min_us, samples);
}

extern "C" int mslam_gemm_bf16(const void* A, const void* Wt, const float* bias, const void* residual_f32, void* out,
                               int M, int N, int K, int act, int out_is_bf16, void* stream) {
  MSLAM_REQUIRE(A && Wt && out, "gemm_bf16: null pointer");
  GemmArgs g = {};
  g.A = (const bf16*)A; g.W = (const bf16*)Wt; g.M = M; g.N = N; g.K = K; g.lda = K; g.bias = bias; g.act = act;
  g.out = out; g.out_kind = out_is_bf16 ? KIND_BF16 : KIND_F32; g.ldc = N; g.ldr1 = N; g.ldr2 = N;
  if (residual_f32) { g.res1 = residual_f32; g.res1_kind = KIND_F32; }
  return launch_gemm(g, (hipStream_t)stream);
}

extern "C" int mslam_conv2d_nhwc_bf16(const void* in, const void* Wt, const float* bias, const void* residual_bf16,
                                      void* out_bf16, int B, int H, int Wd, int Cin, int Cout, int ks, int stride,
                                      int relu_in, int act, void* stream) {
  MSLAM_REQUIRE(in && Wt && out_bf16, "conv2d: null pointer");
  MSLAM_REQUIRE((ks == 1 || ks == 3) && (stride == 1 || stride == 2), "conv2d: unsupported ks/stride");
  Lin l; l.W = (const bf16*)Wt; l.b = bias; l.out = Cout; l.in = ks * ks * Cin;
  GemmArgs g = conv_args((const bf16*)in, B, H, Wd, Cin, l, ks, stride);
  g.out = out_bf16; g.a_relu = relu_in; g.act = act;
  if (residual_bf16) { g.res1 = residual_bf16; g.res1_kind = KIND_BF16; }
  return launch_gemm(g, (hipStream_t)stream);
}

extern "C" int mslam_attention_bf16(const void* Q, const void* K, const void* VT, void* O, int batch, int heads,
                                    int nq, int nk, void* stream) {
  MSLAM_REQUIRE(Q && K && VT && O, "attention: null pointer");
  return launch_attention((const bf16*)Q, (const bf16*)K, (const bf16*)VT, (bf16*)O, batch, heads, nq, nk,
                          (hipStream_t)stream);
}

extern "C" int mslam_layernorm_f32(const float* x, const float* w, const float* b, void* out_bf16, float* out_f32,
                                   int rows, int D, float eps, void* stream) {
  MSLAM_REQUIRE(x && w && b && (out_bf16 || out_f32), "layernorm: null pointer");
  MSLAM_REQUIRE(D <= 2048 && rows > 0, "layernorm: D=%d must be <= 2048", D);
  launch_layernorm(x, w, b, (bf16*)out_bf16, out_f32, rows, D, eps, (hipStream_t)stream);
  MSLAM_LAUNCH_CHECK("layernorm");
  return MSLAM_OK;
}
```

mast3r-slam-quality-dualtsdf_amd/mast3r_slam/mast3r_model.py:

```python
import ctypes
import os

import torch

import mslam_hip as _m


class Mast3rConfig:
    def __init__(self, enc_dim=1024, enc_depth=24, enc_heads=16, dec_dim=768, dec_depth=12, dec_heads=12,
                 patch=16, desc_dim=24, feature_dim=256):
        self.enc_dim, self.enc_depth, self.enc_heads = enc_dim, enc_depth, enc_heads
        self.dec_dim, self.dec_depth, self.dec_heads = dec_dim, dec_depth, dec_heads
        self.patch, self.desc_dim, self.feature_dim = patch, desc_dim, feature_dim

    def as_list(self):
        return [self.enc_dim, self.enc_depth, self.enc_heads, self.dec_dim, self.dec_depth, self.dec_heads,
                self.patch, self.desc_dim, self.feature_dim]


def canonical_weights(sd, cfg, device):
    out = []

    def get(name):
        if name not in sd:
            alt = name.replace("dec_blocks2.", "dec_blocks.")
            for i in range(4):
                alt = alt.replace(f"scratch.layer_rn.{i}.", f"scratch.layer{i + 1}_rn.")
            if alt not in sd:
                raise KeyError(f"checkpoint is missing {name}")
            name = alt
        return sd[name]

    def mat(name):
        w = get(name + ".weight").float()
        if w.ndim == 4:
            w = w.permute(0, 2, 3, 1).reshape(w.shape[0], -1)
        out.append(w.to(device=device, dtype=torch.bfloat16).contiguous())

    def vec(name):
        out.append(get(name).to(device=device, dtype=torch.float32).contiguous())

    def lin(name, bias=True):
        mat(name)
        if bias:
            vec(name + ".bias")

    def norm(name):
        vec(name + ".weight")
        vec(name + ".bias")

    def convT(name):
        w = get(name + ".weight").float()
        out.append(w.permute(1, 2, 3, 0).reshape(-1, w.shape[0]).to(device=device, dtype=torch.bfloat16).contiguous())
        vec(name + ".bias")

    w = get("patch_embed.proj.weight").float()
    out.append(w.reshape(w.shape[0], -1).to(device=device, dtype=torch.bfloat16).contiguous())
    vec("patch_embed.proj.bias")
    for i in range(cfg.enc_depth):
        p = f"enc_blocks.{i}"
        norm(p + ".norm1"); lin(p + ".attn.qkv"); lin(p + ".attn.proj")
        norm(p + ".norm2"); lin(p + ".mlp.fc1"); lin(p + ".mlp.fc2")
    norm("enc_norm")
    lin("decoder_embed")
    for blocks in ("dec_blocks", "dec_blocks2"):
        for i in range(cfg.dec_depth):
            p = f"{blocks}.{i}"
            norm(p + ".norm1"); lin(p + ".attn.qkv"); lin(p + ".attn.proj")
            norm(p + ".norm2"); norm(p + ".norm_y")
            lin(f"{p}.cross_attn.projq")
            wk, wv = get(f"{p}.cross_attn.projk.weight").float(), get(f"{p}.cross_attn.projv.weight").float()
            out.append(torch.cat((wk, wv), 0).to(device=device, dtype=torch.bfloat16).contiguous())
            out.append(torch.cat((get(f"{p}.cross_attn.projk.bias"), get(f"{p}.cross_attn.projv.bias")), 0)
                       .to(device=device, dtype=torch.float32).contiguous())
            lin(f"{p}.cross_attn.proj")
            norm(p + ".norm3"); lin(p + ".mlp.fc1"); lin(p + ".mlp.fc2")
    norm("dec_norm")
    for h in (1, 2):
        p = f"downstream_head{h}.dpt"
        a = p + ".act_postprocess"
        lin(a + ".0.0"); convT(a + ".0.1")
        lin(a + ".1.0"); convT(a + ".1.1")
        lin(a + ".2.0")
        lin(a + ".3.0"); lin(a + ".3.1")
        for i in range(4):
            lin(f"{p}.scratch.layer_rn.{i}", bias=False)
        for r in (4, 3, 2, 1):
            q = f"{p}.scratch.refinenet{r}"
            if r != 4:
                lin(q + ".resConfUnit1.conv1"); lin(q + ".resConfUnit1.conv2")
            lin(q + ".resConfUnit2.conv1"); lin(q + ".resConfUnit2.conv2")
            lin(q + ".out_conv")
        lin(p + ".head.0"); lin(p + ".head.2")
        w4 = get(p + ".head.4.weight").float()
        out.append(w4.reshape(w4.shape[0], -1).to(device=device, dtype=torch.float32).contiguous())
        vec(p + ".head.4.bias")
        lin(f"downstream_head{h}.head_local_features.fc1"); lin(f"downstream_head{h}.head_local_features.fc2")
    return out


class Mast3rHIP:
    def __init__(self, state_dict, cfg: Mast3rConfig = None, device="cuda", use_graphs=False):
        self.cfg = cfg or Mast3rConfig()
        self.device = torch.device(device)
        self.use_graphs = bool(use_graphs)
        self._graphs = {}
        self._pos_cache = {}
        self._weights = canonical_weights(state_dict, self.cfg, self.device)
        n = len(self._weights)
        ptrs = (ctypes.c_void_p * n)(*[w.data_ptr() for w in self._weights])
        numels = (ctypes.c_longlong * n)(*[w.numel() for w in self._weights])
        cfg9 = (ctypes.c_int * 9)(*self.cfg.as_list())
        handle = ctypes.c_void_p()
        rc = _m.lib().mslam_mast3r_create(ctypes.byref(handle), cfg9, ptrs, numels, n, _m.stream_ptr())
        _m.check(rc, "mast3r_create")
        self._h = handle
        self._ws = None
        self._head_cache = {}

    def __del__(self):
        try:
            _m.lib().mslam_mast3r_destroy(self._h)
        except Exception:
            pass

    def share_memory(self):
        return self

    def to(self, *a, **k):
        return self

    def eval(self):
        return self

    def _workspace(self, B, H, W, kind="dec"):
        need = _m.lib().mslam_mast3r_workspace_bytes(self._h, B, H, W)
        if need == 0:
            _m.check(-1, "mast3r_workspace_bytes")
        if self._ws is None:
            self._ws = {}
        key = (kind, _m.stream_ptr())
        if key not in self._ws or self._ws[key].numel() < need:
            self._ws[key] = torch.empty(need, dtype=torch.uint8, device=self.device)
        return self._ws[key]

    def positions(self, B, H, W):
        key = (B, H, W)
        if key not in self._pos_cache:
            nh, nw = H // self.cfg.patch, W // self.cfg.patch
            y, x = torch.meshgrid(torch.arange(nh, device=self.device), torch.arange(nw, device=self.device), indexing="ij")
            self._pos_cache[key] = torch.stack((y.reshape(-1), x.reshape(-1)), -1)[None].expand(B, -1, 2).contiguous()
        return self._pos_cache[key].clone()

    @torch.inference_mode()
    def _encode_image(self, image, true_shape=None):
        image = image.to(self.device, torch.float32).contiguous()
        B, _, H, W = image.shape
        N = (H // self.cfg.patch) * (W // self.cfg.patch)
        self._last_hw = (H, W)
        if self.use_graphs:
            return self._replay(("enc", B, H, W), (image,))[0].clone(), self.positions(B, H, W), None
        feat = torch.empty((B, N, self.cfg.enc_dim), dtype=torch.float32, device=self.device)
        self._run_encode(image, feat, self._workspace(B, H, W, "enc"))
        return feat, self.positions(B, H, W), None

    def _run_encode(self, image, feat, ws):
        B, _, H, W = image.shape
        rc = _m.lib().mslam_mast3r_encode(self._h, _m.ptr(image), B, H, W, _m.ptr(feat), _m.ptr(ws), ws.numel(),
                                         _m.stream_ptr())
        _m.check(rc, "mast3r_encode")

    def _run_decode(self, feat1, feat2, H, W, outs, d1, d2, ws):
        a, b = outs
        rc = _m.lib().mslam_mast3r_decode(
            self._h, _m.ptr(feat1), _m.ptr(feat2), feat1.shape[0], H, W, _m.ptr(a["pts3d"]), _m.ptr(a["conf"]),
            _m.ptr(a["desc"]), _m.ptr(a["desc_conf"]), _m.ptr(b["pts3d"]), _m.ptr(b["conf"]), _m.ptr(b["desc"]),
            _m.ptr(b["desc_conf"]), _m.ptr(d1), _m.ptr(d2), _m.ptr(ws), ws.numel(), _m.stream_ptr())
        _m.check(rc, "mast3r_decode")

    def _decode_buffers(self, B, H, W, N):
        dd = self.cfg.desc_dim
        f32 = dict(dtype=torch.float32, device=self.device)
        outs = [dict(pts3d=torch.empty((B, H, W, 3), **f32), conf=torch.empty((B, H, W), **f32),
                     desc=torch.empty((B, H, W, dd), **f32), desc_conf=torch.empty((B, H, W), **f32)) for _ in range(2)]
        return outs, torch.empty((B, N, self.cfg.dec_dim), **f32), torch.empty((B, N, self.cfg.dec_dim), **f32)

    def _replay(self, key, inputs):
        ent = self._graphs.get(key)
        if ent is None:
            kind, B, H, W = key
            N = (H // self.cfg.patch) * (W // self.cfg.patch)
            need = _m.lib().mslam_mast3r_workspace_bytes(self._h, B, H, W)
            ws = torch.empty(need, dtype=torch.uint8, device=self.device)
            static_in = [torch.empty_like(x) for x in inputs]
            if kind == "enc":
                feat = torch.empty((B, N, self.cfg.enc_dim), dtype=torch.float32, device=self.device)
                run = lambda: self._run_encode(static_in[0], feat, ws)
                outs = (feat,)
            else:
                o, d1, d2 = self._decode_buffers(B, H, W, N)
                run = lambda: self._run_decode(static_in[0], static_in[1], H, W, o, d1, d2, ws)
                outs = (o, d1, d2)
            for dst, src in zip(static_in, inputs):
                dst.copy_(src)
            side = torch.cuda.Stream(device=self.device)
            side.wait_stream(torch.cuda.current_stream(self.device))
            with torch.cuda.stream(side):
                run()
            torch.cuda.current_stream(self.device).wait_stream(side)
            g = torch.cuda.CUDAGraph()
            with torch.cuda.graph(g, stream=side, capture_error_mode="thread_local"):
                run()
            ent = self._graphs[key] = (g, static_in, outs, ws)
        g, static_in, outs, _ = ent
        for dst, src in zip(static_in, inputs):
            dst.copy_(src)
        g.replay()
        return outs

    @torch.inference_mode()
    def decode_pair(self, feat1, feat2, H, W, return_tokens=False):
        feat1 = feat1.to(self.device, torch.float32).contiguous()
        feat2 = feat2.to(self.device, torch.float32).contiguous()
        B, N = feat1.shape[0], feat1.shape[1]
        if self.use_graphs:
            (a, b), d1, d2 = self._replay(("dec", B, H, W), (feat1, feat2))
            a, b = {k: v.clone() for k, v in a.items()}, {k: v.clone() for k, v in b.items()}
            d1, d2 = d1.clone(), d2.clone()
        else:
            (a, b), d1, d2 = self._decode_buffers(B, H, W, N)
            self._run_decode(feat1, feat2, H, W, (a, b), d1, d2, self._workspace(B, H, W))
        if return_tokens:
            return a, b, d1, d2
        return a, b

    def _decoder(self, f1, pos1, f2, pos2):
        nw = int(pos1[..., 1].max().item()) + 1
        nh = int(pos1[..., 0].max().item()) + 1
        H, W = nh * self.cfg.patch, nw * self.cfg.patch
        r1, r2, d1, d2 = self.decode_pair(f1, f2, H, W, return_tokens=True)
        self._head_cache = {d1.data_ptr(): r1, d2.data_ptr(): r2}
        n = self.cfg.dec_depth + 1
        return [f1] + [d1] * (n - 1), [f2] + [d2] * (n - 1)

    def _downstream_head(self, head_num, decout, img_shape):
        key = decout[-1].data_ptr()
        if key not in self._head_cache:
            raise RuntimeError("_downstream_head: tokens do not come from the last _decoder call of this model")
        return self._head_cache[key]


def load_mast3r_state_dict(path):
    if not os.path.isfile(path):
        raise FileNotFoundError(
            f"{path}: MASt3R checkpoint not found (the reference downloads it, README.md:63-65; no network here)")
    import argparse

    with torch.serialization.safe_globals([argparse.Namespace]):
        ckpt = torch.load(path, map_location="cpu", weights_only=True)
    return ckpt["model"] if "model" in ckpt else ckpt


def random_state_dict(cfg: Mast3rConfig, seed=0):
    g = torch.Generator().manual_seed(seed)
    sd = {}

    def lin(name, o, i, bias=True):
        sd[name + ".weight"] = (torch.rand(o, i, generator=g) * 2 - 1) * (6.0 / (i + o)) ** 0.5
        if bias:
            sd[name + ".bias"] = (torch.rand(o, generator=g) * 2 - 1) * 0.02

    def ln(name, d):
        sd[name + ".weight"] = 1 + 0.1 * (torch.rand(d, generator=g) * 2 - 1)
        sd[name + ".bias"] = 0.05 * (torch.rand(d, generator=g) * 2 - 1)

    def conv(name, o, i, k, bias=True, transpose=False):
        shape = (i, o, k, k) if transpose else (o, i, k, k)
        sd[name + ".weight"] = (torch.rand(*shape, generator=g) * 2 - 1) * (3.0 / (i * k * k)) ** 0.5
        if bias:
            sd[name + ".bias"] = (torch.rand(o, generator=g) * 2 - 1) * 0.02

    E, D, P = cfg.enc_dim, cfg.dec_dim, cfg.patch
    conv("patch_embed.proj", E, 3, P)
    for i in range(cfg.enc_depth):
        p = f"enc_blocks.{i}"
        ln(p + ".norm1", E); lin(p + ".attn.qkv", 3 * E, E); lin(p + ".attn.proj", E, E)
        ln(p + ".norm2", E); lin(p + ".mlp.fc1", 4 * E, E); lin(p + ".mlp.fc2", E, 4 * E)
    ln("enc_norm", E)
    lin("decoder_embed", D, E)
    for blocks in ("dec_blocks", "dec_blocks2"):
        for i in range(cfg.dec_depth):
            p = f"{blocks}.{i}"
            ln(p + ".norm1", D); lin(p + ".attn.qkv", 3 * D, D); lin(p + ".attn.proj", D, D)
            ln(p + ".norm2", D); ln(p + ".norm_y", D)
            for q in ("projq", "projk", "projv", "proj"):
                lin(f"{p}.cross_attn.{q}", D, D)
            ln(p + ".norm3", D); lin(p + ".mlp.fc1", 4 * D, D); lin(p + ".mlp.fc2", D, 4 * D)
    ln("dec_norm", D)
    fd, dims = cfg.feature_dim, [96, 192, 384, 768]
    for h in (1, 2):
        p = f"downstream_head{h}.dpt"
        a = p + ".act_postprocess"
        conv(a + ".0.0", dims[0], E, 1); conv(a + ".0.1", dims[0], dims[0], 4, transpose=True)
        conv(a + ".1.0", dims[1], D, 1); conv(a + ".1.1", dims[1], dims[1], 2, transpose=True)
        conv(a + ".2.0", dims[2], D, 1)
        conv(a + ".3.0", dims[3], D, 1); conv(a + ".3.1", dims[3], dims[3], 3)
        for i, d in enumerate(dims):
            conv(f"{p}.scratch.layer_rn.{i}", fd, d, 3, bias=False)
        for r in (1, 2, 3, 4):
            q = f"{p}.scratch.refinenet{r}"
            conv(q + ".out_conv", fd, fd, 1)
            for u in (1, 2):
                conv(f"{q}.resConfUnit{u}.conv1", fd, fd, 3); conv(f"{q}.resConfUnit{u}.conv2", fd, fd, 3)
        conv(p + ".head.0", fd // 2, fd, 3); conv(p + ".head.2", fd // 2, fd // 2, 3); conv(p + ".head.4", 4, fd // 2, 1)
        sd[p + ".head.4.weight"] *= 0.1
        idim = E + D
        lin(f"downstream_head{h}.head_local_features.fc1", 4 * idim, idim)
        lin(f"downstream_head{h}.head_local_features.fc2", (cfg.desc_dim + 1) * P * P, 4 * idim)
    return sd
```

mast3r-slam-quality-dualtsdf_amd/mast3r_slam/mast3r_utils.py:

```python
import numpy as np
import torch

import mast3r_slam.matching as matching
from mast3r_slam.config import config
from mast3r_slam.mast3r_model import Mast3rConfig, Mast3rHIP, load_mast3r_state_dict


def load_mast3r(path=None, device="cuda"):
    weights_path = "checkpoints/MASt3R_ViTLarge_BaseDecoder_512_catmlpdpt_metric.pth" if path is None else path
    return Mast3rHIP(load_mast3r_state_dict(weights_path), Mast3rConfig(), device=device)


def load_retriever(mast3r_model, retriever_path=None, device="cuda"):
    from mast3r_slam.retrieval_database import RetrievalDatabase

    retriever_path = ("checkpoints/MASt3R_ViTLarge_BaseDecoder_512_catmlpdpt_metric_retrieval_trainingfree.pth"
                      if retriever_path is None else retriever_path)
    return RetrievalDatabase.from_checkpoint(retriever_path, device=device)


def _hw(shape):
    s = shape[0] if (hasattr(shape, "ndim") and shape.ndim == 2) or isinstance(shape[0], (list, tuple)) else shape
    return int(s[0]), int(s[1])


@torch.inference_mode()
def decoder(model, feat1, feat2, pos1, pos2, shape1, shape2):
    H, W = _hw(shape1)
    res1, res2 = model.decode_pair(feat1, feat2, H, W)
    return res1, res2


def downsample(X, C, D, Q):
    ds = config["dataset"]["img_downsample"]
    if ds > 1:
        X = X[..., ::ds, ::ds, :].contiguous()
        C = C[..., ::ds, ::ds].contiguous()
        D = D[..., ::ds, ::ds, :].contiguous()
        Q = Q[..., ::ds, ::ds].contiguous()
    return X, C, D, Q


def _ensure_feat(model, frame):
    if frame.feat is None:
        frame.feat, frame.pos, _ = model._encode_image(frame.img, frame.img_true_shape)


def _stack(res):
    X, C, D, Q = zip(*[(r["pts3d"][0], r["conf"][0], r["desc"][0], r["desc_conf"][0]) for r in res])
    return torch.stack(X), torch.stack(C), torch.stack(D), torch.stack(Q)


@torch.inference_mode()
def mast3r_symmetric_inference(model, frame_i, frame_j):
    _ensure_feat(model, frame_i)
    _ensure_feat(model, frame_j)
    res11, res21 = decoder(model, frame_i.feat, frame_j.feat, frame_i.pos, frame_j.pos, frame_i.img_true_shape,
                           frame_j.img_true_shape)
    res22, res12 = decoder(model, frame_j.feat, frame_i.feat, frame_j.pos, frame_i.pos, frame_j.img_true_shape,
                           frame_i.img_true_shape)
    return downsample(*_stack([res11, res21, res22, res12]))


@torch.inference_mode()
def mast3r_decode_symmetric_batch(model, feat_i, pos_i, feat_j, pos_j, shape_i, shape_j, cached=None):
    H, W = _hw(shape_i[0])
    B = feat_i.shape[0]
    f1, f2 = torch.cat((feat_i, feat_j)), torch.cat((feat_j, feat_i))
    keys = ("pts3d", "conf", "desc", "desc_conf")
    if not cached:
        ra, rb = model.decode_pair(f1, f2, H, W)
        pick = lambda k: torch.stack((ra[k][:B], rb[k][:B], ra[k][B:], rb[k][B:]))
        return downsample(pick("pts3d"), pick("conf"), pick("desc"), pick("desc_conf"))
    keep = [r for r in range(2 * B) if r not in cached]
    out = []
    if f1.is_cuda:
        cur = torch.cuda.current_stream(f1.device)
        for res in cached.values():
            for t in res:
                t.record_stream(cur)
    if keep:
        sel = torch.tensor(keep, device=f1.device)
        ra, rb = model.decode_pair(f1[sel].contiguous(), f2[sel].contiguous(), H, W)
        part = downsample(*(torch.stack((ra[k], rb[k])) for k in keys))
    some = cached[next(iter(cached))]
    for q in range(4):
        full = torch.empty((2, 2 * B) + tuple(some[q].shape[1:]), dtype=some[q].dtype, device=some[q].device)
        if keep:
            full[:, sel] = part[q]
        for r, res in cached.items():
            full[:, r] = res[q]
        out.append(torch.stack((full[0, :B], full[1, :B], full[0, B:], full[1, B:])))
    return tuple(out)


@torch.inference_mode()
def mast3r_inference_mono(model, frame):
    _ensure_feat(model, frame)
    res11, res21 = decoder(model, frame.feat, frame.feat, frame.pos, frame.pos, frame.img_true_shape,
                           frame.img_true_shape)
    X, C, D, Q = downsample(*_stack([res11, res21]))
    return X[0].reshape(-1, 3), C[0].reshape(-1, 1)


def mast3r_match_symmetric(model, feat_i, pos_i, feat_j, pos_j, shape_i, shape_j, cached=None):
    X, C, D, Q = mast3r_decode_symmetric_batch(model, feat_i, pos_i, feat_j, pos_j, shape_i, shape_j, cached=cached)
    b = X.shape[1]
    Xii, Xji, Xjj, Xij = X[0], X[1], X[2], X[3]
    Dii, Dji, Djj, Dij = D[0], D[1], D[2], D[3]
    Qii, Qji, Qjj, Qij = Q[0], Q[1], Q[2], Q[3]
    X11 = torch.cat((Xii, Xjj), dim=0)
    X21 = torch.cat((Xji, Xij), dim=0)
    D11 = torch.cat((Dii, Djj), dim=0)
    D21 = torch.cat((Dji, Dij), dim=0)
    idx_1_to_2, valid_match_2 = matching.match(X11, X21, D11, D21)
    match_b = X11.shape[0] // 2
    return (idx_1_to_2[:match_b], idx_1_to_2[match_b:], valid_match_2[:match_b], valid_match_2[match_b:],
            Qii.reshape(b, -1, 1), Qjj.reshape(b, -1, 1), Qji.reshape(b, -1, 1), Qij.reshape(b, -1, 1))


@torch.inference_mode()
def encode_frames(model, frames):
    todo = [f for f in frames if f.feat is None]
    if not todo:
        return
    feat, pos, _ = model._encode_image(torch.cat([f.img for f in todo]), todo[0].img_true_shape)
    for k, f in enumerate(todo):
        f.feat, f.pos = feat[k:k + 1], pos[k:k + 1]


@torch.inference_mode()
def mast3r_asymmetric_inference_group(model, frames, keyframe):
    frames = list(frames)
    encode_frames(model, frames)
    _ensure_feat(model, keyframe)
    B = len(frames)
    feat_i = torch.cat([f.feat for f in frames])
    res11, res21 = decoder(model, feat_i, keyframe.feat.expand(B, -1, -1).contiguous(), None, None,
                           frames[0].img_true_shape, keyframe.img_true_shape)
    for k, f in enumerate(frames):
        pick = lambda key: torch.stack((res11[key][k], res21[key][k]))
        f.decoded = (int(keyframe.frame_id), downsample(pick("pts3d"), pick("conf"), pick("desc"), pick("desc_conf")))


@torch.inference_mode()
def mast3r_asymmetric_inference(model, frame_i, frame_j):
    stash = getattr(frame_i, "decoded", None)
    if stash is not None:
        frame_i.decoded = None
        if stash[0] == int(frame_j.frame_id):
            frame_i.pair_decode = stash
            return stash[1]
    _ensure_feat(model, frame_i)
    _ensure_feat(model, frame_j)
    res11, res21 = decoder(model, frame_i.feat, frame_j.feat, frame_i.pos, frame_j.pos, frame_i.img_true_shape,
                           frame_j.img_true_shape)
    out = downsample(*_stack([res11, res21]))
    if hasattr(frame_j, "frame_id"):
        frame_i.pair_decode = (int(frame_j.frame_id), out)
    return out


def mast3r_match_asymmetric(model, frame_i, frame_j, idx_i2j_init=None):
    X, C, D, Q = mast3r_asymmetric_inference(model, frame_i, frame_j)
    b, h, w = X.shape[:-1]
    b = b // 2
    Xii, Xji = X[:b], X[b:]
    Dii, Dji = D[:b], D[b:]
    idx_i2j, valid_match_j = matching.match(Xii, Xji, Dii, Dji, idx_1_to_2_init=idx_i2j_init)
    Xii, Xji = X.reshape(2, h * w, 3)
    Cii, Cji = C.reshape(2, h * w, 1)
    Qii, Qji = Q.reshape(2, h * w, 1)
    return idx_i2j, valid_match_j, Xii, Cii, Qii, Xji, Cji, Qji


def _resize_pil_image(img, long_edge_size):
    import PIL.Image

    S = max(img.size)
    interp = PIL.Image.LANCZOS if S > long_edge_size else PIL.Image.BICUBIC
    new_size = tuple(int(round(x * long_edge_size / S)) for x in img.size)
    return img.resize(new_size, interp)


def resize_img(img, size, square_ok=False, return_transformation=False):
    import PIL.Image

    assert size == 224 or size == 512
    img = PIL.Image.fromarray(np.uint8(img * 255))
    W1, H1 = img.size
    if size == 224:
        img = _resize_pil_image(img, round(size * max(W1 / H1, H1 / W1)))
    else:
        img = _resize_pil_image(img, size)
    W, H = img.size
    cx, cy = W // 2, H // 2
    if size == 224:
        half = min(cx, cy)
        img = img.crop((cx - half, cy - half, cx + half, cy + half))
    else:
        halfw, halfh = ((2 * cx) // 16) * 8, ((2 * cy) // 16) * 8
        if not square_ok and W == H:
            halfh = 3 * halfw / 4
        img = img.crop((cx - halfw, cy - halfh, cx + halfw, cy + halfh))
    arr = np.asarray(img)
    norm = (torch.from_numpy(arr.copy()).permute(2, 0, 1).float() / 255.0 - 0.5) / 0.5
    res = dict(img=norm[None], true_shape=np.int32([img.size[::-1]]), unnormalized_img=arr)
    if return_transformation:
        return res, (W1 / W, H1 / H, (W - img.size[0]) / 2, (H - img.size[1]) / 2)
    return res
```

mast3r-slam-quality-dualtsdf_amd/mast3r_slam/matching.py:

```python
import torch

import mast3r_slam_backends
import mslam_hip as _m
from mast3r_slam.config import config


def match(X11, X21, D11, D21, idx_1_to_2_init=None):
    idx_1_to_2, valid_match2 = match_iterative_proj(X11, X21, D11, D21, idx_1_to_2_init)
    return idx_1_to_2, valid_match2


def pixel_to_lin(p1, w):
    p1 = p1.contiguous()
    lead = p1.shape[:-1]
    n = 1
    for s in lead:
        n *= s
    idx = torch.empty(lead, dtype=torch.int64, device=p1.device)
    rc = _m.lib().mslam_pixel_to_lin(_m.ptr(p1), _m.ptr(idx), 1, n, int(w), _m.stream_ptr())
    _m.check(rc, "pixel_to_lin")
    return idx


def lin_to_pixel(idx_1_to_2, w):
    u = idx_1_to_2 % w
    v = idx_1_to_2 // w
    return torch.stack((u, v), dim=-1)


def prep_for_iter_proj(X11, X21, idx_1_to_2_init):
    b, h, w, _ = X11.shape
    X11 = X11.contiguous()
    X21 = X21.contiguous()
    dev = X11.device
    rays = torch.empty((b, h, w, 9), dtype=torch.float32, device=dev)
    pts = torch.empty((b, h * w, 3), dtype=torch.float32, device=dev)
    p_init = torch.empty((b, h * w, 2), dtype=torch.float32, device=dev)
    if idx_1_to_2_init is not None:
        idx_1_to_2_init = idx_1_to_2_init.contiguous()
        _m.require_dtype(idx_1_to_2_init, torch.int64, "idx_1_to_2_init")
    rc = _m.lib().mslam_prep_iter_proj(
        _m.ptr(X11), _m.ptr(X21), _m.ptr(idx_1_to_2_init), _m.ptr(rays), _m.ptr(pts), _m.ptr(p_init),
        b, h, w, _m.stream_ptr(),
    )
    _m.check(rc, "prep_for_iter_proj")
    return rays, pts, p_init


def match_iterative_proj(X11, X21, D11, D21, idx_1_to_2_init=None):
    cfg = config["matching"]
    b, h, w = X21.shape[:3]
    X11 = X11.contiguous()
    X21 = X21.contiguous()

    rays_with_grad_img, pts3d_norm, p_init = prep_for_iter_proj(X11, X21, idx_1_to_2_init)
    p1f, valid_proj2 = mast3r_slam_backends.iter_proj(
        rays_with_grad_img, pts3d_norm, p_init, cfg["max_iter"], cfg["lambda_init"], cfg["convergence_thresh"]
    )

    p1 = torch.empty((b, h * w, 2), dtype=torch.int64, device=X11.device)
    rc = _m.lib().mslam_match_occlusion(
        _m.ptr(X11), _m.ptr(X21), _m.ptr(p1f), _m.ptr(p1), _m.ptr(valid_proj2), b, h, w,
        float(cfg["dist_thresh"]), _m.stream_ptr(),
    )
    _m.check(rc, "match_occlusion")

    if cfg["radius"] > 0:
        (p1,) = mast3r_slam_backends.refine_matches(
            D11.half().contiguous(), D21.reshape(b, h * w, -1).half().contiguous(), p1,
            cfg["radius"], cfg["dilation_max"],
        )

    idx_1_to_2 = pixel_to_lin(p1, w)
    return idx_1_to_2, valid_proj2.unsqueeze(-1)
```

mast3r-slam-quality-dualtsdf_amd/mast3r_slam/tracker.py:

```python
import copy
import time

import numpy as np
import torch

import mslam_hip as _m
from lietorch_hip import Sim3
from mast3r_slam.config import config
from mast3r_slam.geometry import act_Sim3, constrain_points_to_ray, point_to_ray_dist
from mast3r_slam.mast3r_utils import mast3r_match_asymmetric


class _Pending:
    __slots__ = ("frame", "init_T", "prev_idx", "prev_shadow", "stash", "base", "shadow", "slot", "job", "verdict",
                 "event", "quality", "T_WCf", "T_CkCf", "T_WCk", "Xkf", "Ckf", "Qkf", "Qff", "status", "n_points", "replayed",
                 "kind", "vals", "new_kf")


class FrameTracker:
    IN_PLACE_MODES = ("indep_conf",)

    def __init__(self, model, frames, device):
        self.cfg = config["tracking"]
        self.model = model
        self.keyframes = frames
        self.device = device
        self.reset_idx_f2k()
        self.N_SLOTS = 4
        self._slots = [dict(ws=None, status=None, host=None, prep=None) for _ in range(self.N_SLOTS)]
        self._slot = 0
        self._shadow = None
        self.quality_service = None
        self.last_kf_value = None
        self.verdict_wait_s = 0.0

    def reset_idx_f2k(self):
        self.idx_f2k = None

    def track(self, frame):
        h = self.track_begin(frame)
        self.track_resolve(h)
        return self.track_finish(h)

    def track_begin(self, frame):
        h = _Pending()
        h.frame, h.replayed = frame, False
        h.init_T, h.prev_idx, h.prev_shadow = frame.T_WC, self.idx_f2k, self._shadow
        h.stash = getattr(frame, "decoded", None)
        stored = self.keyframes.last_keyframe()
        keyframe = self._shadow if self._shadow is not None else stored
        idx_f2k, valid_match_k, Xff, Cff, Qff, Xkf, Ckf, Qkf = mast3r_match_asymmetric(
            self.model, frame, keyframe, idx_i2j_init=self.idx_f2k)
        self.idx_f2k = idx_f2k.clone()
        idx_f2k = idx_f2k[0]
        valid_match_k = valid_match_k[0]
        frame.update_pointmap(Xff, Cff)

        use_calib = config["use_calib"]
        img_size = frame.img.shape[-2:]
        K = keyframe.K if use_calib else None
        T_WCk = stored.T_WC
        Xf, Xk = frame.X_canon, keyframe.X_canon
        if use_calib:
            Xf = constrain_points_to_ray(img_size, Xf[None], K).squeeze(0)
            Xk = constrain_points_to_ray(img_size, Xk[None], K).squeeze(0)
        self._idx = idx_f2k

        h.slot = self._slot
        self._slot = (self._slot + 1) % self.N_SLOTS
        self._cur = h
        Qk, Ck, valid_opt, valid_kf, T_rel = self._prepare(h, frame, keyframe, idx_f2k, valid_match_k, Qff, Qkf,
                                                           T_WCk, frame.T_WC)
        T_WCf, T_CkCf, status = self._run_async(use_calib, Xf, Xk, None, T_WCk, Qk, valid_opt, K if use_calib else None,
                                                img_size if use_calib else None, chunked=True, T_rel=T_rel, pose=False)
        h.job, h.T_WCk = getattr(self, "_job", None), T_WCk
        h.status = status
        self._post_verdict(h)
        h.quality = None
        if self.quality_service is not None and not use_calib:
            h.quality = dict(Xf=Xf, idx=idx_f2k, Xk=Xk, valid_kf=valid_kf.view(-1), Ck=Ck.view(-1), Qk=Qk.view(-1),
                             kf_id=int(len(self.keyframes) - 1), frame_id=int(keyframe.frame_id), H=int(img_size[0]),
                             W=int(img_size[1]))
        h.base, h.Xkf, h.Ckf, h.Qkf, h.Qff = keyframe, Xkf, Ckf, Qkf, Qff
        self._apply(h, T_WCf, T_CkCf)
        return h

    def _prepare(self, h, frame, keyframe, idx_f2k, valid_match_k, Qff, Qkf, T_WCk, T_WCf):
        n = int(keyframe.X_canon.shape[0])
        dev = idx_f2k.device
        L = _m.lib()
        sl = self._slots[h.slot]
        need = L.mslam_track_prepare_workspace_bytes(n)
        if sl.get("prep") is None or sl["prep"].numel() < need:
            sl["prep"] = torch.empty(need, dtype=torch.uint8, device=dev)
        Qk = torch.empty((n, 1), dtype=torch.float32, device=dev)
        Ck = torch.empty((n, 1), dtype=torch.float32, device=dev)
        valid_opt = torch.empty((n, 1), dtype=torch.bool, device=dev)
        valid_kf = torch.empty((n, 1), dtype=torch.bool, device=dev)
        T_rel = torch.empty(8, dtype=torch.float32, device=dev)
        idx_c, vm_c = idx_f2k.contiguous(), valid_match_k.contiguous()
        Qff_c, Qkf_c = Qff.contiguous(), Qkf.contiguous()
        Cf_c, Ck_c = frame.C.contiguous(), keyframe.C.contiguous()
        Tk_c, Tf_c = T_WCk.data.reshape(8).contiguous(), T_WCf.data.reshape(8).contiguous()
        _m.require_dtype(idx_c, torch.int64, "idx_f2k")
        _m.require_dtype(vm_c, torch.bool, "valid_match_k")
        inv_nf = float(np.float32(1.0) / np.float32(frame.N))
        inv_nk = float(np.float32(1.0) / np.float32(keyframe.N))
        rc = L.mslam_track_prepare(_m.ptr(idx_c), _m.ptr(vm_c), _m.ptr(Qff_c), _m.ptr(Qkf_c), _m.ptr(Cf_c), inv_nf,
                                   _m.ptr(Ck_c), inv_nk, float(self.cfg["C_conf"]), float(self.cfg["Q_conf"]), n,
                                   _m.ptr(Tk_c), _m.ptr(Tf_c), _m.ptr(Qk), _m.ptr(Ck), _m.ptr(valid_opt),
                                   _m.ptr(valid_kf), _m.ptr(T_rel), _m.ptr(sl["prep"]), sl["prep"].numel(),
                                   _m.stream_ptr())
        _m.check(rc, "track_prepare")
        h.n_points = n
        return Qk, Ck, valid_opt, valid_kf, T_rel

    def _post_verdict(self, h):
        sl = self._slots[h.slot]
        dev = torch.empty(6, dtype=torch.float32, device=h.status.device)
        rc = _m.lib().mslam_track_verdict(_m.ptr(sl["prep"]), _m.ptr(h.status), int(h.n_points), _m.ptr(dev),
                                          _m.stream_ptr())
        _m.check(rc, "track_verdict")
        if sl["host"] is None:
            sl["host"] = torch.empty(6, dtype=torch.float32).pin_memory()
        sl["host"].copy_(dev, non_blocking=True)
        h.event = torch.cuda.Event()
        h.event.record()
        h.verdict = sl["host"]

    def _apply(self, h, T_WCf, T_CkCf):
        h.T_CkCf = T_CkCf
        base = h.base
        shadow = copy.copy(base)
        shadow._in_store, shadow._replaced_by = False, None
        T_WCk = h.T_WCk
        if config["tracking"]["filtering_mode"] == "weighted_pointmap" and base.N > 0:
            n = int(base.X_canon.shape[0])
            dev = base.X_canon.device
            T_out = torch.empty((1, 8), dtype=torch.float32, device=dev)
            X_new, C_new = torch.empty_like(base.X_canon), torch.empty_like(base.C)
            Tk_c, Tr_c = T_WCk.data.reshape(8).contiguous(), T_CkCf.data.reshape(8).contiguous()
            Xkf_c, Ckf_c = h.Xkf.contiguous(), h.Ckf.contiguous()
            Xc_c, Cc_c = base.X_canon.contiguous(), base.C.contiguous()
            assert X_new.is_contiguous() and C_new.is_contiguous()
            rc = _m.lib().mslam_track_fuse(_m.ptr(Tk_c), _m.ptr(Tr_c), _m.ptr(Xkf_c), _m.ptr(Ckf_c), _m.ptr(Xc_c),
                                           _m.ptr(Cc_c), n, _m.ptr(T_out), _m.ptr(X_new), _m.ptr(C_new), _m.stream_ptr())
            _m.check(rc, "track_fuse")
            if T_WCf is None:
                T_WCf = Sim3(T_out)
            shadow.X_canon, shadow.C = X_new, C_new
            shadow.N, shadow.N_updates = base.N + 1, base.N_updates + 1
        else:
            if T_WCf is None:
                T_WCf = T_WCk * T_CkCf
            Xkk = T_CkCf.act(h.Xkf)
            if config["tracking"]["filtering_mode"] in self.IN_PLACE_MODES:
                shadow.X_canon, shadow.C = shadow.X_canon.clone(), shadow.C.clone()
            shadow.update_pointmap(Xkk, h.Ckf)
        h.T_WCf = T_WCf
        h.frame.T_WC = T_WCf
        h.shadow = shadow
        self._shadow = shadow

    def track_resolve(self, h):
        t_wait = time.perf_counter()
        h.event.synchronize()
        self.verdict_wait_s += time.perf_counter() - t_wait
        v = h.verdict.tolist()
        if v[0] >= self.cfg["min_match_frac"] and int(v[5]) == 0 and int(v[2]) == 0 and int(v[1]) < int(self.cfg["max_iters"]):
            self._cur = h
            _, T_CkCf, h.status = self._run_rest()
            self._post_verdict(h)
            h.event.synchronize()
            v = h.verdict.tolist()
            stale = h.shadow
            later = self._shadow if self._shadow is not stale else None
            self._apply(h, None, T_CkCf)
            stale._replaced_by = h.shadow
            if later is not None:
                self._shadow = later
            h.replayed = True
        h.vals = v
        self.last_iters = int(v[1])
        skip = v[0] < self.cfg["min_match_frac"] or int(v[2]) != 0
        h.kind = "skip" if skip else "ok"
        h.new_kf = (not skip) and min(float(v[3]), float(v[4])) < self.cfg["match_frac_thresh"]
        return h.kind

    def track_finish(self, h):
        frame = h.frame
        if h.kind == "skip":
            frame.T_WC = h.init_T
            if self._shadow is h.shadow:
                self._shadow = self._live(h.prev_shadow)
            return False, [], True
        if h.quality is not None:
            q = h.quality
            T_CkCf = h.T_CkCf

            def residual_map(q=q, T=T_CkCf):
                Xf_g = q["Xf"][q["idx"]]
                rd_k = point_to_ray_dist(q["Xk"], jacobian=False)
                rd_f = point_to_ray_dist(act_Sim3(T, Xf_g, jacobian=False), jacobian=False)
                vec = T.data.view(-1, 8)
                w = vec[..., 6].clamp(-1.0, 1.0).abs()
                return {"r_pix": torch.linalg.norm(rd_k - rd_f, dim=1), "t_norm": vec[..., :3].norm(dim=-1).mean(),
                        "theta": (2.0 * torch.arccos(w)).mean()}

            self.quality_service.submit({
                "kf_id": q["kf_id"], "frame_id": q["frame_id"], "H": q["H"], "W": q["W"], "valid_kf": q["valid_kf"],
                "Ck": q["Ck"], "Qk": q["Qk"], "lazy": residual_map, "keep": (q["Xf"], q["idx"], q["Xk"], T_CkCf.data)})
        keyframe = h.shadow
        keyframe.T_WC = self.keyframes.last_keyframe().T_WC
        self.keyframes[len(self.keyframes) - 1] = keyframe
        keyframe._in_store = True
        if self._shadow is h.shadow:
            self._shadow = None
        match_frac_k, unique_frac_f = float(h.vals[3]), float(h.vals[4])
        self.last_kf_value = min(match_frac_k, unique_frac_f)
        new_kf = h.new_kf
        if new_kf:
            self.reset_idx_f2k()
            self._shadow = None
        return (new_kf, [keyframe.X_canon, keyframe.get_average_conf(), frame.X_canon, frame.get_average_conf(),
                         h.Qkf, h.Qff], False)

    @staticmethod
    def _live(shadow):
        while shadow is not None and getattr(shadow, "_replaced_by", None) is not None:
            shadow = shadow._replaced_by
        return None if shadow is None or getattr(shadow, "_in_store", False) else shadow

    def rollback(self, h):
        self.idx_f2k, self._shadow = h.prev_idx, self._live(h.prev_shadow)
        f = h.frame
        f.T_WC, f.X_canon, f.C, f.N, f.N_updates = h.init_T, None, None, 0, 0
        if h.stash is not None:
            f.decoded = h.stash

    def get_points_poses(self, frame, keyframe, idx_f2k, img_size, use_calib, K=None):
        Xf, Xk = frame.X_canon, keyframe.X_canon
        Cf, Ck = frame.get_average_conf(), keyframe.get_average_conf()
        meas_k = valid_meas_k = None
        if use_calib:
            Xf = constrain_points_to_ray(img_size, Xf[None], K).squeeze(0)
            Xk = constrain_points_to_ray(img_size, Xk[None], K).squeeze(0)
        self._idx = idx_f2k
        return Xf, Xk, frame.T_WC, keyframe.T_WC, Cf[idx_f2k], Ck, meas_k, valid_meas_k

    def _run(self, use_calib, Xf, Xk, T_WCf, T_WCk, Qk, valid, K, img_size, idx=None):
        T_WCf_new, T_CkCf, status = self._run_async(use_calib, Xf, Xk, T_WCf, T_WCk, Qk, valid, K, img_size, idx)
        st = status.cpu()
        self.last_iters = int(st[1])
        return T_WCf_new, T_CkCf, int(st[2]) == 0

    FIRST_CHUNK = 8

    def _run_async(self, use_calib, Xf, Xk, T_WCf, T_WCk, Qk, valid, K, img_size, idx=None, chunked=False, T_rel=None,
                   pose=True):
        cfg = self.cfg
        dev = Xf.device
        idx = self._idx if idx is None else idx
        n = Xk.shape[0]
        if T_rel is None:
            T_rel = (T_WCk.inv() * T_WCf).data.reshape(8).contiguous().clone()
        L = _m.lib()
        need = L.mslam_track_workspace_bytes(n)
        cur = getattr(self, "_cur", None)
        sl = self._slots[cur.slot if cur is not None else 0]
        if sl["ws"] is None or sl["ws"].numel() < need:
            sl["ws"] = torch.empty(need, dtype=torch.uint8, device=dev)
            sl["status"] = torch.zeros(8, dtype=torch.int32, device=dev)
        h, w = (int(img_size[0]), int(img_size[1])) if img_size is not None else (0, 0)
        sa, sb = (cfg["sigma_pixel"], cfg["sigma_depth"]) if use_calib else (cfg["sigma_ray"], cfg["sigma_dist"])
        Xf_c, Xk_c, idx_c = Xf.contiguous(), Xk.contiguous(), idx.contiguous()
        Qk_c, valid_c = Qk.reshape(-1).contiguous(), valid.reshape(-1).contiguous()
        K_c = K.contiguous() if use_calib else None
        self._job = dict(args=(int(use_calib), _m.ptr(T_rel), _m.ptr(Xf_c), _m.ptr(Xk_c), _m.ptr(idx_c), _m.ptr(Qk_c),
                               _m.ptr(valid_c), n, _m.ptr(K_c) if use_calib else 0,
                               w, h, float(sa), float(sb), float(cfg["huber"]), int(cfg["pixel_border"]),
                               float(cfg["depth_eps"])),
                         keep=(T_rel, Xf_c, Xk_c, idx_c, Qk_c, valid_c, K_c), T_rel=T_rel, T_WCk=T_WCk, slot=sl, pose=pose)
        last = min(self.FIRST_CHUNK, int(cfg["max_iters"])) if chunked else int(cfg["max_iters"])
        return self._enqueue(self._job, 0, last)

    def _enqueue(self, job, first, last):
        cfg, sl = self.cfg, job["slot"]
        rc = _m.lib().mslam_track_pose(*job["args"], int(first), int(last), float(cfg["rel_error"]),
                                       float(cfg["delta_norm"]), _m.ptr(sl["status"]), _m.ptr(sl["ws"]),
                                       sl["ws"].numel(), _m.stream_ptr())
        _m.check(rc, "track_pose")
        T_CkCf = Sim3(job["T_rel"].reshape(1, 8))
        return (job["T_WCk"] * T_CkCf if job["pose"] else None), T_CkCf, sl["status"]

    def _run_rest(self):
        job = self._cur.job if getattr(self, "_cur", None) is not None and self._cur.job is not None else self._job
        return self._enqueue(job, min(self.FIRST_CHUNK, int(self.cfg["max_iters"])), int(self.cfg["max_iters"]))

    def opt_pose_ray_dist_sim3(self, Xf, Xk, T_WCf, T_WCk, Qk, valid, idx=None):
        return self._run(False, Xf, Xk, T_WCf, T_WCk, Qk, valid, None, None, idx)

    def opt_pose_calib_sim3(self, Xf, Xk, T_WCf, T_WCk, Qk, valid, meas_k, valid_meas_k, K, img_size, idx=None):
        return self._run(True, Xf, Xk, T_WCf, T_WCk, Qk, valid, K, img_size, idx)
```

Baseline: 164.2.

## Fuse head 3x3 conv with logits projection and emit fp16 descriptors directly

Adds a GEMM epilogue (EPI_HEAD) that applies ReLU, projects the 128-channel conv output onto the 4 head logits inside the conv kernel, and writes float4 logits. This removes the intermediate bf16 feature map write and its re-read in head_post. The head_post kernel also writes an fp16 copy of the descriptors, so matching no longer has to run separate .half() conversion passes. Decode outputs can be written paired via an output stride, and the tracker releases cached pair decodes early. The cost is more LDS use and register pressure in the fused epilogue, plus extra API plumbing.

```diff
diff --git a/include/mslam_hip.h b/include/mslam_hip.h
--- a/include/mslam_hip.h
+++ b/include/mslam_hip.h
@@ -154,14 +154,15 @@
 int mslam_mast3r_create(void** handle_out, const int* cfg9_host, void* const* weight_ptrs_host,
                         const long long* weight_numels_host, int n_weights, void* stream);
 int mslam_mast3r_destroy(void* handle);
-size_t mslam_mast3r_workspace_bytes(void* handle, int batch, int H, int W);
+size_t mslam_mast3r_workspace_bytes(void* handle, int batch, int H, int W, int unfused_head_tail);
 
 int mslam_mast3r_encode(void* handle, const float* img, int batch, int H, int W, float* feat_out,
                         void* workspace, size_t workspace_bytes, void* stream);
 
 int mslam_mast3r_decode(void* handle, const float* feat1, const float* feat2, int batch, int H, int W,
                         float* X1, float* C1, float* D1, float* Q1, float* X2, float* C2, float* D2,
-                        float* Q2, float* dec_last1, float* dec_last2, void* workspace,
+                        float* Q2, uint16_t* D16_1, uint16_t* D16_2, int out_image_stride,
+                        int unfused_head_tail, float* dec_last1, float* dec_last2, void* workspace,
                         size_t workspace_bytes, void* stream);
 
 size_t mslam_track_workspace_bytes(int n_points);
@@ -189,6 +190,8 @@
 int mslam_conv2d_nhwc_bf16(const void* in, const void* W, const float* bias, const void* residual_bf16,
                            void* out_bf16, int B, int H, int Wd, int Cin, int Cout, int ks, int stride,
                            int relu_in, int act, void* stream);
+int mslam_conv3x3_head_logits(const void* in, const void* W, const float* bias, const float* w4, const float* b4,
+                              float* logits, int B, int H, int Wd, int Cin, int Cout, void* stream);
 int mslam_attention_bf16(const void* Q, const void* K, const void* VT, void* O, int batch, int heads,
                          int nq, int nk, void* stream);
 int mslam_layernorm_f32(const float* x, const float* w, const float* b, void* out_bf16, float* out_f32,
diff --git a/mast3r-slam-quality-dualtsdf_amd/csrc/gemm.h b/mast3r-slam-quality-dualtsdf_amd/csrc/gemm.h
--- a/mast3r-slam-quality-dualtsdf_amd/csrc/gemm.h
+++ b/mast3r-slam-quality-dualtsdf_amd/csrc/gemm.h
@@ -12,6 +12,7 @@
   EPI_PLAIN = 0,
   EPI_ATTN = 1,
   EPI_CONVT = 2,
+  EPI_HEAD = 3,
 };
 
 struct GemmArgs {
@@ -37,6 +38,7 @@
   const float* rope_cos; const float* rope_sin;
   float q_scale;
   int ct_s, ct_cout, ct_h, ct_w;
+  const float* head_w4; const float* head_b4; float* head_logits;
   int groups;
   const bf16* W1; const float* bias1;
   size_t a_gstride;
diff --git a/mast3r-slam-quality-dualtsdf_amd/csrc/gemm.hip b/mast3r-slam-quality-dualtsdf_amd/csrc/gemm.hip
--- a/mast3r-slam-quality-dualtsdf_amd/csrc/gemm.hip
+++ b/mast3r-slam-quality-dualtsdf_amd/csrc/gemm.hip
@@ -11,6 +11,7 @@
 int launch_gemm_t128(const GemmArgs& a, int waves, int stages, hipStream_t s);
 int launch_gemm_t128x64(const GemmArgs& a, int stages, hipStream_t s);
 int launch_gemm_t256(const GemmArgs& a, int bn, hipStream_t s);
+int launch_gemm_t256_head(const GemmArgs& a, hipStream_t s);
 int launch_gemm_t192(const GemmArgs& a, hipStream_t s);
 int launch_gemm_t256w8(const GemmArgs& a, hipStream_t s);
 int launch_gemm_8p(const GemmArgs& a, hipStream_t s);
@@ -108,6 +109,15 @@
   MSLAM_REQUIRE(a_bytes < (1ull << 31) && (size_t)a.N * a.K * 2 < (1ull << 31), "gemm: operand larger than 2 GiB");
   MSLAM_REQUIRE(a.epi != EPI_ATTN || (a.sec_dim % 64 == 0 && a.ntok % 4 == 0 && a.kv_ntok % 4 == 0),
                 "gemm: attention epilogue needs 64-wide heads and token counts divisible by 4");
+  if (a.epi == EPI_HEAD) {
+    MSLAM_REQUIRE(a.a_conv && a.N == 128 && a.act == ACT_RELU && !a.res1 && !a.res2 && !a.res1_kind && !a.res2_kind &&
+                      a.groups <= 1 && !a.pf_bytes[0] && !a.pf_bytes[1],
+                  "gemm: the head epilogue needs the conv view with N == 128 (got %d), ReLU and no residuals", a.N);
+    MSLAM_REQUIRE(a.head_w4 && a.head_b4 && a.head_logits && ((uintptr_t)a.head_w4 & 15) == 0 &&
+                      ((uintptr_t)a.head_b4 & 15) == 0 && ((uintptr_t)a.head_logits & 15) == 0,
+                  "gemm: the head epilogue needs 16-byte aligned w4, b4 and logits");
+    return launch_gemm_t256_head(a, stream);
+  }
   static int forced = -2;
   if (forced == -2) {
     const char* e = getenv("MSLAM_GEMM");
diff --git a/mast3r-slam-quality-dualtsdf_amd/csrc/gemm_kernel.h b/mast3r-slam-quality-dualtsdf_amd/csrc/gemm_kernel.h
--- a/mast3r-slam-quality-dualtsdf_amd/csrc/gemm_kernel.h
+++ b/mast3r-slam-quality-dualtsdf_amd/csrc/gemm_kernel.h
@@ -67,7 +67,9 @@
   __builtin_amdgcn_s_waitcnt((N & 15) | ((N >> 4) << 14) | 0x0F70);
 }
 
-template <int WM, int WN, int MI, int NI, int S, bool CONV>
+constexpr int kHeadPartStride = 4;
+
+template <int WM, int WN, int MI, int NI, int S, bool CONV, bool HEAD = false>
 __global__ __launch_bounds__(64 * WM * WN) void gemm_bf16_kernel(GemmArgs g) {
   constexpr int NW = WM * WN;
   constexpr int BM = 32 * MI * WM, BN = 32 * NI * WN;
@@ -305,6 +307,61 @@
   __builtin_amdgcn_s_barrier();
   constexpr int TBS = 40;
   float* tb = reinterpret_cast<float*>(smem) + wid * (32 * TBS);
+  if constexpr (HEAD) {
+    static_assert(BN == 128, "EPI_HEAD: one block holds all 128 channels of its pixels");
+    constexpr int PST = BM + kHeadPartStride;
+    float4* part = reinterpret_cast<float4*>(smem + NW * 32 * TBS * sizeof(float));
+    const int lrow0 = lane >> 2, lc = (lane & 3) * 8, half = lane >> 5;
+    static_for<MI>([&](auto mi_c) {
+      static_for<NI>([&](auto ni_c) {
+        constexpr int mi = decltype(mi_c)::value, ni = decltype(ni_c)::value;
+        const f32x16 accv = acc[mi][ni];
+        const float bias = bias_v[ni];
+        const int cg = wn * NI * 4 + ni * 4 + (lane & 3);
+        float4 wlo[4], whi[4];
+#pragma unroll
+        for (int o = 0; o < 4; o++) {
+          wlo[o] = *reinterpret_cast<const float4*>(g.head_w4 + o * 128 + cg * 8);
+          whi[o] = *reinterpret_cast<const float4*>(g.head_w4 + o * 128 + cg * 8 + 4);
+        }
+        static_for<16>([&](auto r_c) {
+          constexpr int r = decltype(r_c)::value;
+          tb[((r & 3) + 8 * (r >> 2) + 4 * half) * TBS + lcol] = fmaxf(accv[r] + bias, 0.0f);
+        });
+#pragma unroll
+        for (int j = 0; j < 2; j++) {
+          const int lrow = lrow0 + 16 * j;
+          const float4 p = *reinterpret_cast<const float4*>(tb + lrow * TBS + lc);
+          const float4 q = *reinterpret_cast<const float4*>(tb + lrow * TBS + lc + 4);
+          const float x[8] = {p.x, p.y, p.z, p.w, q.x, q.y, q.z, q.w};
+          float pp[4] = {0.0f, 0.0f, 0.0f, 0.0f};
+#pragma unroll
+          for (int k = 0; k < 8; k++) {
+            const float fv = (float)(bf16)x[k];
+#pragma unroll
+            for (int o = 0; o < 4; o++) {
+              const float4 w = k < 4 ? wlo[o] : whi[o];
+              const float wk = (k & 3) == 0 ? w.x : (k & 3) == 1 ? w.y : (k & 3) == 2 ? w.z : w.w;
+              pp[o] = fmaf(wk, fv, pp[o]);
+            }
+          }
+          part[cg * PST + wm * MI * 32 + mi * 32 + lrow] = make_float4(pp[0], pp[1], pp[2], pp[3]);
+        }
+      });
+    });
+    __syncthreads();
+    if (t < BM && m0 + t < g.M) {
+      float4 c[16];
+#pragma unroll
+      for (int k = 0; k < 16; k++) c[k] = part[k * PST + t];
+      const auto add = [](float4 a, float4 b) { return make_float4(a.x + b.x, a.y + b.y, a.z + b.z, a.w + b.w); };
+      const float4 even = add(add(add(c[0], c[8]), add(c[4], c[12])), add(add(c[2], c[10]), add(c[6], c[14])));
+      const float4 odd = add(add(add(c[1], c[9]), add(c[5], c[13])), add(add(c[3], c[11]), add(c[7], c[15])));
+      const float4 b4 = *reinterpret_cast<const float4*>(g.head_b4);
+      reinterpret_cast<float4*>(g.head_logits)[(size_t)(m0 + t)] = add(add(even, odd), b4);
+    }
+    return;
+  }
   typedef __attribute__((ext_vector_type(8))) __bf16 bf16x8s;
   const int half = lane >> 5;
   const int lrow0 = lane >> 2, lc = (lane & 3) * 8;
@@ -513,4 +570,24 @@
   return check_hip(hipGetLastError(), "gemm launch");
 }
 
-}
+template <int WM, int WN, int MI, int NI, int S>
+int launch_cfg_head(const GemmArgs& a, hipStream_t stream) {
+  constexpr int NW = WM * WN, BM = 32 * MI * WM, BN = 32 * NI * WN;
+  static_assert(BN == 128, "EPI_HEAD needs all 128 channels in one block");
+  constexpr size_t ring = (size_t)S * (BM + BN) * 128;
+  constexpr size_t tail = (size_t)NW * 32 * 40 * sizeof(float) + (size_t)16 * (BM + kHeadPartStride) * sizeof(float4);
+  constexpr size_t shmem = ring > tail ? ring : tail;
+  static_assert(shmem <= 160 * 1024, "LDS budget");
+  const unsigned blocks = (unsigned)((a.M + BM - 1) / BM);
+  static bool attr_set = false;
+  if (!attr_set) {
+    int rc = check_hip(hipFuncSetAttribute((const void*)gemm_bf16_kernel<WM, WN, MI, NI, S, true, true>,
+                                           hipFuncAttributeMaxDynamicSharedMemorySize, (int)shmem), "gemm: attr");
+    if (rc) return rc;
+    attr_set = true;
+  }
+  hipLaunchKernelGGL((gemm_bf16_kernel<WM, WN, MI, NI, S, true, true>), dim3(blocks), dim3(64 * NW), shmem, stream, a);
+  return check_hip(hipGetLastError(), "gemm launch");
+}
+
+}
diff --git a/mast3r-slam-quality-dualtsdf_amd/csrc/gemm_t256.hip b/mast3r-slam-quality-dualtsdf_amd/csrc/gemm_t256.hip
--- a/mast3r-slam-quality-dualtsdf_amd/csrc/gemm_t256.hip
+++ b/mast3r-slam-quality-dualtsdf_amd/csrc/gemm_t256.hip
@@ -8,4 +8,6 @@
   if (bn == 256) return launch_cfg<4, 4, 2, 2, 2>(a, s);
   return launch_cfg<4, 2, 2, 2, 2>(a, s);
 }
+
+int launch_gemm_t256_head(const GemmArgs& a, hipStream_t s) { return launch_cfg_head<4, 2, 2, 2, 2>(a, s); }
 }
diff --git a/mast3r-slam-quality-dualtsdf_amd/csrc/mast3r.hip b/mast3r-slam-quality-dualtsdf_amd/csrc/mast3r.hip
--- a/mast3r-slam-quality-dualtsdf_amd/csrc/mast3r.hip
+++ b/mast3r-slam-quality-dualtsdf_amd/csrc/mast3r.hip
@@ -214,13 +214,16 @@
 }
 
 constexpr int kHP = 16;
+template <bool LOGITS>
 __global__ __launch_bounds__(256) void head_post_kernel(const bf16* __restrict__ feat, int fc,
                                                         const float* __restrict__ w4, const float* __restrict__ b4,
+                                                        const float4* __restrict__ logits,
                                                         const float* __restrict__ lf, int lf_ld, int desc_dim,
-                                                        int B, int H, int W, float* __restrict__ X,
+                                                        int B, int H, int W, int out_stride, float* __restrict__ X,
                                                         float* __restrict__ Cf, float* __restrict__ D,
-                                                        float* __restrict__ Q) {
+                                                        float* __restrict__ Q, _Float16* __restrict__ D16) {
   typedef __attribute__((ext_vector_type(8))) __bf16 bf16x8;
+  typedef __attribute__((ext_vector_type(4))) _Float16 f16x4;
   __shared__ float l_s[kHP * kHP][4];
   __shared__ __attribute__((aligned(16))) float d_s[kHP * kHP * 24];
   __shared__ __attribute__((aligned(16))) float x_s[kHP * kHP * 3];
@@ -228,7 +231,13 @@
   const int nw = W / kHP, nh = H / kHP;
   const int tok = blockIdx.x;
   const int b = tok / (nh * nw), ty = (tok / nw) % nh, tx = tok % nw;
-  const size_t pix00 = ((size_t)b * H + (size_t)ty * kHP) * W + (size_t)tx * kHP;
+  const size_t in00 = ((size_t)b * H + (size_t)ty * kHP) * W + (size_t)tx * kHP;
+  const size_t pix00 = in00 + (size_t)b * (out_stride - 1) * H * W;
+  float l0, l1, l2, l3;
+  if constexpr (LOGITS) {
+    const float4 l = logits[in00 + (size_t)(threadIdx.x >> 4) * W + (threadIdx.x & 15)];
+    l0 = l.x; l1 = l.y; l2 = l.z; l3 = l.w;
+  } else {
   const int cg = t & 15, ppx = t >> 4;
   float wr[4][8];
 #pragma unroll
@@ -236,7 +245,7 @@
 #pragma unroll
     for (int k = 0; k < 8; k++) wr[o][k] = w4[o * fc + cg * 8 + k];
   for (int r = 0; r < kHP; r++) {
-    const bf16x8 v = *reinterpret_cast<const bf16x8*>(feat + (pix00 + (size_t)r * W + ppx) * fc + cg * 8);
+    const bf16x8 v = *reinterpret_cast<const bf16x8*>(feat + (in00 + (size_t)r * W + ppx) * fc + cg * 8);
     float p[4] = {0.0f, 0.0f, 0.0f, 0.0f};
 #pragma unroll
     for (int k = 0; k < 8; k++) {
@@ -254,8 +263,9 @@
     }
   }
   __syncthreads();
+  l0 = l_s[t][0]; l1 = l_s[t][1]; l2 = l_s[t][2]; l3 = l_s[t][3];
+  }
   const int py = t >> 4, px = t & 15;
-  const float l0 = l_s[t][0], l1 = l_s[t][1], l2 = l_s[t][2], l3 = l_s[t][3];
   const float d = sqrtf(l0 * l0 + l1 * l1 + l2 * l2);
   const float sc = expm1f(d) / fmaxf(d, 1e-8f);
   x_s[t * 3 + 0] = l0 * sc; x_s[t * 3 + 1] = l1 * sc; x_s[t * 3 + 2] = l2 * sc;
@@ -274,7 +284,12 @@
 #pragma unroll
   for (int k = 0; k < 6; k++) {
     const int e = t + 256 * k, r = e / 96, q = e - r * 96;
-    *reinterpret_cast<float4*>(D + (pix00 + (size_t)r * W) * 24 + q * 4) = *reinterpret_cast<const float4*>(d_s + r * 384 + q * 4);
+    const float4 dq = *reinterpret_cast<const float4*>(d_s + r * 384 + q * 4);
+    *reinterpret_cast<float4*>(D + (pix00 + (size_t)r * W) * 24 + q * 4) = dq;
+    if (D16) {
+      const f16x4 h = {(_Float16)dq.x, (_Float16)dq.y, (_Float16)dq.z, (_Float16)dq.w};
+      *reinterpret_cast<f16x4*>(D16 + (pix00 + (size_t)r * W) * 24 + q * 4) = h;
+    }
   }
   if (t < 192) {
     const int r = t / 12, q = t - r * 12;
@@ -285,14 +300,15 @@
 __global__ __launch_bounds__(256) void head_post_generic_kernel(const bf16* __restrict__ feat, int fc,
                                                         const float* __restrict__ w4, const float* __restrict__ b4,
                                                         const float* __restrict__ lf, int lf_ld, int desc_dim, int P,
-                                                        int B, int H, int W, float* __restrict__ X,
+                                                        int B, int H, int W, int out_stride, float* __restrict__ X,
                                                         float* __restrict__ Cf, float* __restrict__ D,
-                                                        float* __restrict__ Q) {
-  const size_t pix = (size_t)blockIdx.x * 256 + threadIdx.x;
-  if (pix >= (size_t)B * H * W) return;
-  const int x = (int)(pix % W), y = (int)((pix / W) % H), b = (int)(pix / ((size_t)W * H));
+                                                        float* __restrict__ Q, _Float16* __restrict__ D16) {
+  const size_t ipix = (size_t)blockIdx.x * 256 + threadIdx.x;
+  if (ipix >= (size_t)B * H * W) return;
+  const int x = (int)(ipix % W), y = (int)((ipix / W) % H), b = (int)(ipix / ((size_t)W * H));
+  const size_t pix = ipix + (size_t)b * (out_stride - 1) * H * W;
   float l[4] = {b4[0], b4[1], b4[2], b4[3]};
-  const bf16* f = feat + pix * fc;
+  const bf16* f = feat + ipix * fc;
   typedef __attribute__((ext_vector_type(8))) __bf16 bf16x8;
   for (int c = 0; c < fc; c += 8) {
     const bf16x8 v = *reinterpret_cast<const bf16x8*>(f + c);
@@ -314,7 +330,11 @@
   float nn = 0.0f;
   for (int c = 0; c < desc_dim; c++) { dv[c] = lp[c * P * P]; nn = fmaf(dv[c], dv[c], nn); }
   const float inv = 1.0f / sqrtf(nn);
-  for (int c = 0; c < desc_dim; c++) D[pix * desc_dim + c] = dv[c] * inv;
+  for (int c = 0; c < desc_dim; c++) {
+    const float dn = dv[c] * inv;
+    D[pix * desc_dim + c] = dn;
+    if (D16) D16[pix * desc_dim + c] = (_Float16)dn;
+  }
   Q[pix] = expf(lp[desc_dim * P * P]);
 }
 
@@ -396,6 +416,8 @@
   Arena ar;
   hipStream_t s;
   int rc = MSLAM_OK;
+  bool unfused_tail = false;
+  int out_stride = 1;
   bool dry() const { return ar.dry; }
   void fail(int r) { if (rc == MSLAM_OK) rc = r; }
 };
@@ -595,7 +617,7 @@
   return upsample2x(c, o, B, H, W, C);
 }
 
-struct HeadOut { float *X, *C, *D, *Q; };
+struct HeadOut { float *X, *C, *D, *Q; _Float16* D16; };
 
 static void run_head(Ctx& c, const Head& hd, const bf16* const toks[4], int B, int H, int W, const HeadOut& out) {
   const Mast3rModel& m = *c.m;
@@ -624,7 +646,18 @@
   bf16* p1 = fusion(c, hd.fus[0], p2, r0, B, 4 * nh, 4 * nw, fd);
   bf16* h0 = conv(c, p1, B, 8 * nh, 8 * nw, fd, hd.h0, 3, 1, 0, ACT_NONE, nullptr, nullptr);
   bf16* hu = upsample2x(c, h0, B, 8 * nh, 8 * nw, hd.h0.out);
-  bf16* h2 = conv(c, hu, B, H, W, hd.h0.out, hd.h2, 3, 1, 0, ACT_RELU, nullptr, nullptr);
+  const bool patch_post = m.P == kHP && hd.h2.out == 128 && m.desc_dim == 24;
+  const bool fused = patch_post && hd.h0.out % 8 == 0 && !c.unfused_tail;
+  bf16* h2 = nullptr;
+  float* logits = nullptr;
+  if (fused) {
+    GemmArgs g = conv_args(hu, B, H, W, hd.h0.out, hd.h2, 3, 1);
+    logits = c.ar.get<float>((size_t)g.M * 4);
+    g.act = ACT_RELU; g.epi = EPI_HEAD; g.head_w4 = hd.h4w; g.head_b4 = hd.h4b; g.head_logits = logits;
+    run_gemm(c, g);
+  } else {
+    h2 = conv(c, hu, B, H, W, hd.h0.out, hd.h2, 3, 1, 0, ACT_RELU, nullptr, nullptr);
+  }
   const int idim = m.E + m.Dd;
   bf16* cat = c.ar.get<bf16>((size_t)M * idim);
   bf16* hid = c.ar.get<bf16>((size_t)M * hd.fc1.out);
@@ -638,13 +671,19 @@
   linear_bf16(c, cat, M, hd.fc1, hid, ACT_GELU);
   linear_f32(c, hid, M, hd.fc2, lf);
   if (!c.dry() && !c.rc) {
-    if (m.P == kHP && hd.h2.out == 128 && m.desc_dim == 24) {
-      hipLaunchKernelGGL(head_post_kernel, dim3((unsigned)(B * (H / m.P) * (W / m.P))), dim3(256), 0, c.s, h2, hd.h2.out,
-                         hd.h4w, hd.h4b, lf, hd.fc2.out, m.desc_dim, B, H, W, out.X, out.C, out.D, out.Q);
+    const dim3 patches((unsigned)(B * (H / m.P) * (W / m.P)));
+    if (fused) {
+      hipLaunchKernelGGL(head_post_kernel<true>, patches, dim3(256), 0, c.s, nullptr, hd.h2.out, hd.h4w, hd.h4b,
+                         reinterpret_cast<const float4*>(logits), lf, hd.fc2.out, m.desc_dim, B, H, W, c.out_stride,
+                         out.X, out.C, out.D, out.Q, out.D16);
+    } else if (patch_post) {
+      hipLaunchKernelGGL(head_post_kernel<false>, patches, dim3(256), 0, c.s, h2, hd.h2.out, hd.h4w, hd.h4b, nullptr, lf,
+                         hd.fc2.out, m.desc_dim, B, H, W, c.out_stride, out.X, out.C, out.D, out.Q, out.D16);
     } else {
       const size_t npix = (size_t)B * H * W;
       hipLaunchKernelGGL(head_post_generic_kernel, dim3((unsigned)((npix + 255) / 256)), dim3(256), 0, c.s, h2, hd.h2.out,
-                         hd.h4w, hd.h4b, lf, hd.fc2.out, m.desc_dim, m.P, B, H, W, out.X, out.C, out.D, out.Q);
+                         hd.h4w, hd.h4b, lf, hd.fc2.out, m.desc_dim, m.P, B, H, W, c.out_stride, out.X, out.C, out.D,
+                         out.Q, out.D16);
     }
     dbg(c, "head_post", B, H, W);
   }
@@ -840,10 +879,11 @@
   return MSLAM_OK;
 }
 
-extern "C" size_t mslam_mast3r_workspace_bytes(void* handle, int batch, int H, int W) {
+extern "C" size_t mslam_mast3r_workspace_bytes(void* handle, int batch, int H, int W, int unfused_head_tail) {
   const Mast3rModel* m = (const Mast3rModel*)handle;
   if (!m || check_shape(m, batch, H, W, "mast3r_workspace_bytes")) return 0;
   Ctx c{m, Arena{nullptr, 0, 0, true}, nullptr};
+  c.unfused_tail = unfused_head_tail != 0;
   encode(c, nullptr, batch, H, W, nullptr);
   c.ar.off = 0;
   HeadOut out[2] = {};
@@ -857,7 +897,7 @@
   int rc = check_shape(m, batch, H, W, "mast3r_encode");
   if (rc) return rc;
   MSLAM_REQUIRE(img && feat_out && workspace, "mast3r_encode: null pointer");
-  MSLAM_REQUIRE(workspace_bytes >= mslam_mast3r_workspace_bytes(handle, batch, H, W), "mast3r_encode: workspace too small");
+  MSLAM_REQUIRE(workspace_bytes >= mslam_mast3r_workspace_bytes(handle, batch, H, W, 0), "mast3r_encode: workspace too small");
   Ctx c{m, Arena{(char*)workspace, 0, workspace_bytes, false}, (hipStream_t)stream};
   encode(c, img, batch, H, W, feat_out);
   MSLAM_REQUIRE(!c.ar.overflow, "mast3r_encode: workspace arena overflow (%zu > %zu)", c.ar.peak, c.ar.cap);
@@ -867,15 +907,20 @@
 
 extern "C" int mslam_mast3r_decode(void* handle, const float* feat1, const float* feat2, int batch, int H, int W,
                                    float* X1, float* C1, float* D1, float* Q1, float* X2, float* C2, float* D2,
-                                   float* Q2, float* dec_last1, float* dec_last2, void* workspace,
+                                   float* Q2, uint16_t* D16_1, uint16_t* D16_2, int out_image_stride,
+                                   int unfused_head_tail, float* dec_last1, float* dec_last2, void* workspace,
                                    size_t workspace_bytes, void* stream) {
   const Mast3rModel* m = (const Mast3rModel*)handle;
   int rc = check_shape(m, batch, H, W, "mast3r_decode");
   if (rc) return rc;
   MSLAM_REQUIRE(feat1 && feat2 && X1 && C1 && D1 && Q1 && X2 && C2 && D2 && Q2 && workspace, "mast3r_decode: null pointer");
-  MSLAM_REQUIRE(workspace_bytes >= mslam_mast3r_workspace_bytes(handle, batch, H, W), "mast3r_decode: workspace too small");
+  MSLAM_REQUIRE(out_image_stride >= 1, "mast3r_decode: out_image_stride %d must be positive", out_image_stride);
+  MSLAM_REQUIRE(workspace_bytes >= mslam_mast3r_workspace_bytes(handle, batch, H, W, unfused_head_tail),
+                "mast3r_decode: workspace too small");
   Ctx c{m, Arena{(char*)workspace, 0, workspace_bytes, false}, (hipStream_t)stream};
-  HeadOut out[2] = {{X1, C1, D1, Q1}, {X2, C2, D2, Q2}};
+  c.unfused_tail = unfused_head_tail != 0;
+  c.out_stride = out_image_stride;
+  HeadOut out[2] = {{X1, C1, D1, Q1, (_Float16*)D16_1}, {X2, C2, D2, Q2, (_Float16*)D16_2}};
   decode(c, feat1, feat2, batch, H, W, out, dec_last1, dec_last2);
   MSLAM_REQUIRE(!c.ar.overflow, "mast3r_decode: workspace arena overflow (%zu > %zu)", c.ar.peak, c.ar.cap);
   if (c.rc) return c.rc;
@@ -917,6 +962,16 @@
   return launch_gemm(g, (hipStream_t)stream);
 }
 
+extern "C" int mslam_conv3x3_head_logits(const void* in, const void* Wt, const float* bias, const float* w4,
+                                         const float* b4, float* logits, int B, int H, int Wd, int Cin, int Cout,
+                                         void* stream) {
+  MSLAM_REQUIRE(in && Wt && w4 && b4 && logits, "conv3x3_head_logits: null pointer");
+  Lin l; l.W = (const bf16*)Wt; l.b = bias; l.out = Cout; l.in = 9 * Cin;
+  GemmArgs g = conv_args((const bf16*)in, B, H, Wd, Cin, l, 3, 1);
+  g.act = ACT_RELU; g.epi = EPI_HEAD; g.head_w4 = w4; g.head_b4 = b4; g.head_logits = logits;
+  return launch_gemm(g, (hipStream_t)stream);
+}
+
 extern "C" int mslam_attention_bf16(const void* Q, const void* K, const void* VT, void* O, int batch, int heads,
                                     int nq, int nk, void* stream) {
   MSLAM_REQUIRE(Q && K && VT && O, "attention: null pointer");
diff --git a/mast3r-slam-quality-dualtsdf_amd/mast3r_slam/mast3r_model.py b/mast3r-slam-quality-dualtsdf_amd/mast3r_slam/mast3r_model.py
--- a/mast3r-slam-quality-dualtsdf_amd/mast3r_slam/mast3r_model.py
+++ b/mast3r-slam-quality-dualtsdf_amd/mast3r_slam/mast3r_model.py
@@ -100,6 +100,8 @@
 
 
 class Mast3rHIP:
+    supports_paired_decode = True
+
     def __init__(self, state_dict, cfg: Mast3rConfig = None, device="cuda", use_graphs=False):
         self.cfg = cfg or Mast3rConfig()
         self.device = torch.device(device)
@@ -133,8 +135,8 @@
     def eval(self):
         return self
 
-    def _workspace(self, B, H, W, kind="dec"):
-        need = _m.lib().mslam_mast3r_workspace_bytes(self._h, B, H, W)
+    def _workspace(self, B, H, W, kind="dec", unfused_head_tail=False):
+        need = _m.lib().mslam_mast3r_workspace_bytes(self._h, B, H, W, int(unfused_head_tail))
         if need == 0:
             _m.check(-1, "mast3r_workspace_bytes")
         if self._ws is None:
@@ -170,19 +172,30 @@
                                          _m.stream_ptr())
         _m.check(rc, "mast3r_encode")
 
-    def _run_decode(self, feat1, feat2, H, W, outs, d1, d2, ws):
-        a, b = outs
+    def _run_decode(self, feat1, feat2, H, W, outs, d1, d2, ws, unfused_head_tail=False):
+        a, b = outs[0], outs[1]
+        stride = 1 if a["pts3d"].is_contiguous() else 2
+        if stride == 2:
+            for k, t in a.items():
+                n = t[0].numel()
+                if (not t[0].is_contiguous() or t.stride(0) != 2 * n or b[k].stride(0) != 2 * n
+                        or b[k].data_ptr() - t.data_ptr() != n * t.element_size()):
+                    raise RuntimeError(f"mast3r_decode: output {k} is neither dense nor the [B, 2] pair layout")
         rc = _m.lib().mslam_mast3r_decode(
             self._h, _m.ptr(feat1), _m.ptr(feat2), feat1.shape[0], H, W, _m.ptr(a["pts3d"]), _m.ptr(a["conf"]),
             _m.ptr(a["desc"]), _m.ptr(a["desc_conf"]), _m.ptr(b["pts3d"]), _m.ptr(b["conf"]), _m.ptr(b["desc"]),
-            _m.ptr(b["desc_conf"]), _m.ptr(d1), _m.ptr(d2), _m.ptr(ws), ws.numel(), _m.stream_ptr())
+            _m.ptr(b["desc_conf"]), _m.ptr(a["desc16"]), _m.ptr(b["desc16"]), stride, int(unfused_head_tail),
+            _m.ptr(d1), _m.ptr(d2), _m.ptr(ws), ws.numel(), _m.stream_ptr())
         _m.check(rc, "mast3r_decode")
 
-    def _decode_buffers(self, B, H, W, N):
+    def _decode_buffers(self, B, H, W, N, paired=False):
         dd = self.cfg.desc_dim
         f32 = dict(dtype=torch.float32, device=self.device)
-        outs = [dict(pts3d=torch.empty((B, H, W, 3), **f32), conf=torch.empty((B, H, W), **f32),
-                     desc=torch.empty((B, H, W, dd), **f32), desc_conf=torch.empty((B, H, W), **f32)) for _ in range(2)]
+        lead = (B, 2) if paired else (2, B)
+        full = dict(pts3d=torch.empty(lead + (H, W, 3), **f32), conf=torch.empty(lead + (H, W), **f32),
+                    desc=torch.empty(lead + (H, W, dd), **f32), desc_conf=torch.empty(lead + (H, W), **f32),
+                    desc16=torch.empty(lead + (H, W, dd), dtype=torch.float16, device=self.device))
+        outs = [{k: (v[:, s] if paired else v[s]) for k, v in full.items()} for s in range(2)] + [full]
         return outs, torch.empty((B, N, self.cfg.dec_dim), **f32), torch.empty((B, N, self.cfg.dec_dim), **f32)
 
     def _replay(self, key, inputs):
@@ -190,7 +203,7 @@
         if ent is None:
             kind, B, H, W = key
             N = (H // self.cfg.patch) * (W // self.cfg.patch)
-            need = _m.lib().mslam_mast3r_workspace_bytes(self._h, B, H, W)
+            need = _m.lib().mslam_mast3r_workspace_bytes(self._h, B, H, W, 0)
             ws = torch.empty(need, dtype=torch.uint8, device=self.device)
             static_in = [torch.empty_like(x) for x in inputs]
             if kind == "enc":
@@ -198,7 +211,7 @@
                 run = lambda: self._run_encode(static_in[0], feat, ws)
                 outs = (feat,)
             else:
-                o, d1, d2 = self._decode_buffers(B, H, W, N)
+                o, d1, d2 = self._decode_buffers(B, H, W, N, paired=(kind == "dec_paired"))
                 run = lambda: self._run_decode(static_in[0], static_in[1], H, W, o, d1, d2, ws)
                 outs = (o, d1, d2)
             for dst, src in zip(static_in, inputs):
@@ -219,17 +232,19 @@
         return outs
 
     @torch.inference_mode()
-    def decode_pair(self, feat1, feat2, H, W, return_tokens=False):
+    def decode_pair(self, feat1, feat2, H, W, return_tokens=False, paired=False, unfused_head_tail=False):
         feat1 = feat1.to(self.device, torch.float32).contiguous()
         feat2 = feat2.to(self.device, torch.float32).contiguous()
         B, N = feat1.shape[0], feat1.shape[1]
-        if self.use_graphs:
-            (a, b), d1, d2 = self._replay(("dec", B, H, W), (feat1, feat2))
-            a, b = {k: v.clone() for k, v in a.items()}, {k: v.clone() for k, v in b.items()}
+        if self.use_graphs and not unfused_head_tail:
+            (_, _, full), d1, d2 = self._replay(("dec_paired" if paired else "dec", B, H, W), (feat1, feat2))
+            full = {k: v.clone() for k, v in full.items()}
+            a, b = ({k: (v[:, s] if paired else v[s]) for k, v in full.items()} for s in range(2))
             d1, d2 = d1.clone(), d2.clone()
         else:
-            (a, b), d1, d2 = self._decode_buffers(B, H, W, N)
-            self._run_decode(feat1, feat2, H, W, (a, b), d1, d2, self._workspace(B, H, W))
+            (a, b, _), d1, d2 = self._decode_buffers(B, H, W, N, paired)
+            self._run_decode(feat1, feat2, H, W, (a, b), d1, d2, self._workspace(B, H, W, "dec", unfused_head_tail),
+                             unfused_head_tail)
         if return_tokens:
             return a, b, d1, d2
         return a, b
diff --git a/mast3r-slam-quality-dualtsdf_amd/mast3r_slam/mast3r_utils.py b/mast3r-slam-quality-dualtsdf_amd/mast3r_slam/mast3r_utils.py
--- a/mast3r-slam-quality-dualtsdf_amd/mast3r_slam/mast3r_utils.py
+++ b/mast3r-slam-quality-dualtsdf_amd/mast3r_slam/mast3r_utils.py
@@ -51,6 +51,20 @@
     return torch.stack(X), torch.stack(C), torch.stack(D), torch.stack(Q)
 
 
+_KEYS = ("pts3d", "conf", "desc", "desc_conf")
+
+
+def _downsample16(D16):
+    ds = config["dataset"]["img_downsample"]
+    return D16[..., ::ds, ::ds, :].contiguous() if ds > 1 and D16 is not None else D16
+
+
+def _match(X11, X21, D11, D21, D16, **kw):
+    if D16 is not None and D16[0] is not None:
+        kw["D16"] = D16
+    return matching.match(X11, X21, D11, D21, **kw)
+
+
 @torch.inference_mode()
 def mast3r_symmetric_inference(model, frame_i, frame_j):
     _ensure_feat(model, frame_i)
@@ -64,14 +78,20 @@
 
 @torch.inference_mode()
 def mast3r_decode_symmetric_batch(model, feat_i, pos_i, feat_j, pos_j, shape_i, shape_j, cached=None):
+    return _decode_symmetric_batch(model, feat_i, feat_j, shape_i, cached)[0]
+
+
+@torch.inference_mode()
+def _decode_symmetric_batch(model, feat_i, feat_j, shape_i, cached=None):
     H, W = _hw(shape_i[0])
     B = feat_i.shape[0]
     f1, f2 = torch.cat((feat_i, feat_j)), torch.cat((feat_j, feat_i))
-    keys = ("pts3d", "conf", "desc", "desc_conf")
+    keys = _KEYS
     if not cached:
         ra, rb = model.decode_pair(f1, f2, H, W)
         pick = lambda k: torch.stack((ra[k][:B], rb[k][:B], ra[k][B:], rb[k][B:]))
-        return downsample(pick("pts3d"), pick("conf"), pick("desc"), pick("desc_conf"))
+        return (downsample(pick("pts3d"), pick("conf"), pick("desc"), pick("desc_conf")),
+                (_downsample16(ra.get("desc16")), _downsample16(rb.get("desc16"))))
     keep = [r for r in range(2 * B) if r not in cached]
     out = []
     if f1.is_cuda:
@@ -91,7 +111,7 @@
         for r, res in cached.items():
             full[:, r] = res[q]
         out.append(torch.stack((full[0, :B], full[1, :B], full[0, B:], full[1, B:])))
-    return tuple(out)
+    return tuple(out), None
 
 
 @torch.inference_mode()
@@ -104,7 +124,7 @@
 
 
 def mast3r_match_symmetric(model, feat_i, pos_i, feat_j, pos_j, shape_i, shape_j, cached=None):
-    X, C, D, Q = mast3r_decode_symmetric_batch(model, feat_i, pos_i, feat_j, pos_j, shape_i, shape_j, cached=cached)
+    (X, C, D, Q), D16 = _decode_symmetric_batch(model, feat_i, feat_j, shape_i, cached)
     b = X.shape[1]
     Xii, Xji, Xjj, Xij = X[0], X[1], X[2], X[3]
     Dii, Dji, Djj, Dij = D[0], D[1], D[2], D[3]
@@ -113,7 +133,7 @@
     X21 = torch.cat((Xji, Xij), dim=0)
     D11 = torch.cat((Dii, Djj), dim=0)
     D21 = torch.cat((Dji, Dij), dim=0)
-    idx_1_to_2, valid_match_2 = matching.match(X11, X21, D11, D21)
+    idx_1_to_2, valid_match_2 = _match(X11, X21, D11, D21, D16)
     match_b = X11.shape[0] // 2
     return (idx_1_to_2[:match_b], idx_1_to_2[match_b:], valid_match_2[:match_b], valid_match_2[match_b:],
             Qii.reshape(b, -1, 1), Qjj.reshape(b, -1, 1), Qji.reshape(b, -1, 1), Qij.reshape(b, -1, 1))
@@ -136,21 +156,43 @@
     _ensure_feat(model, keyframe)
     B = len(frames)
     feat_i = torch.cat([f.feat for f in frames])
-    res11, res21 = decoder(model, feat_i, keyframe.feat.expand(B, -1, -1).contiguous(), None, None,
-                           frames[0].img_true_shape, keyframe.img_true_shape)
+    H, W = _hw(frames[0].img_true_shape)
+    feat_k = keyframe.feat.expand(B, -1, -1).contiguous()
+    if not getattr(model, "supports_paired_decode", False):
+        res11, res21 = model.decode_pair(feat_i, feat_k, H, W)
+        for k, f in enumerate(frames):
+            pick = lambda key: torch.stack((res11[key][k], res21[key][k]))
+            d16 = _downsample16(pick("desc16")) if "desc16" in res11 else None
+            f.decoded = (int(keyframe.frame_id), downsample(*(pick(key) for key in _KEYS)), d16)
+        return
+    res11, res21 = model.decode_pair(feat_i, feat_k, H, W, paired=True)
     for k, f in enumerate(frames):
-        pick = lambda key: torch.stack((res11[key][k], res21[key][k]))
-        f.decoded = (int(keyframe.frame_id), downsample(pick("pts3d"), pick("conf"), pick("desc"), pick("desc_conf")))
-
-
-@torch.inference_mode()
+        def pick(key):
+            row = res11[key][k]
+            return row.as_strided((2,) + tuple(row.shape), (row.numel(),) + tuple(row.stride()), row.storage_offset())
+
+        f.decoded = (int(keyframe.frame_id), downsample(*(pick(key) for key in _KEYS)), _downsample16(pick("desc16")))
+
+
+def release_pair_decode(frame, keep):
+    pd = getattr(frame, "pair_decode", None)
+    if pd is None:
+        return
+    frame.pair_decode = (pd[0], tuple(t.clone() for t in pd[1])) if keep else None
+
+
 def mast3r_asymmetric_inference(model, frame_i, frame_j):
+    return _asymmetric_inference(model, frame_i, frame_j)[0]
+
+
+@torch.inference_mode()
+def _asymmetric_inference(model, frame_i, frame_j):
     stash = getattr(frame_i, "decoded", None)
     if stash is not None:
         frame_i.decoded = None
         if stash[0] == int(frame_j.frame_id):
-            frame_i.pair_decode = stash
-            return stash[1]
+            frame_i.pair_decode = stash[:2]
+            return stash[1], stash[2]
     _ensure_feat(model, frame_i)
     _ensure_feat(model, frame_j)
     res11, res21 = decoder(model, frame_i.feat, frame_j.feat, frame_i.pos, frame_j.pos, frame_i.img_true_shape,
@@ -158,16 +200,18 @@
     out = downsample(*_stack([res11, res21]))
     if hasattr(frame_j, "frame_id"):
         frame_i.pair_decode = (int(frame_j.frame_id), out)
-    return out
+    d16 = torch.stack((res11["desc16"][0], res21["desc16"][0])) if "desc16" in res11 else None
+    return out, _downsample16(d16)
 
 
 def mast3r_match_asymmetric(model, frame_i, frame_j, idx_i2j_init=None):
-    X, C, D, Q = mast3r_asymmetric_inference(model, frame_i, frame_j)
+    (X, C, D, Q), D16 = _asymmetric_inference(model, frame_i, frame_j)
     b, h, w = X.shape[:-1]
     b = b // 2
     Xii, Xji = X[:b], X[b:]
     Dii, Dji = D[:b], D[b:]
-    idx_i2j, valid_match_j = matching.match(Xii, Xji, Dii, Dji, idx_1_to_2_init=idx_i2j_init)
+    idx_i2j, valid_match_j = _match(Xii, Xji, Dii, Dji, None if D16 is None else (D16[:b], D16[b:]),
+                                    idx_1_to_2_init=idx_i2j_init)
     Xii, Xji = X.reshape(2, h * w, 3)
     Cii, Cji = C.reshape(2, h * w, 1)
     Qii, Qji = Q.reshape(2, h * w, 1)
diff --git a/mast3r-slam-quality-dualtsdf_amd/mast3r_slam/matching.py b/mast3r-slam-quality-dualtsdf_amd/mast3r_slam/matching.py
--- a/mast3r-slam-quality-dualtsdf_amd/mast3r_slam/matching.py
+++ b/mast3r-slam-quality-dualtsdf_amd/mast3r_slam/matching.py
@@ -5,8 +5,8 @@
 from mast3r_slam.config import config
 
 
-def match(X11, X21, D11, D21, idx_1_to_2_init=None):
-    idx_1_to_2, valid_match2 = match_iterative_proj(X11, X21, D11, D21, idx_1_to_2_init)
+def match(X11, X21, D11, D21, idx_1_to_2_init=None, D16=None):
+    idx_1_to_2, valid_match2 = match_iterative_proj(X11, X21, D11, D21, idx_1_to_2_init, D16)
     return idx_1_to_2, valid_match2
 
 
@@ -47,7 +47,7 @@
     return rays, pts, p_init
 
 
-def match_iterative_proj(X11, X21, D11, D21, idx_1_to_2_init=None):
+def match_iterative_proj(X11, X21, D11, D21, idx_1_to_2_init=None, D16=None):
     cfg = config["matching"]
     b, h, w = X21.shape[:3]
     X11 = X11.contiguous()
@@ -66,8 +66,9 @@
     _m.check(rc, "match_occlusion")
 
     if cfg["radius"] > 0:
+        D11h, D21h = D16 if D16 is not None else (D11.half(), D21.half())
         (p1,) = mast3r_slam_backends.refine_matches(
-            D11.half().contiguous(), D21.reshape(b, h * w, -1).half().contiguous(), p1,
+            D11h.contiguous(), D21h.reshape(b, h * w, -1).contiguous(), p1,
             cfg["radius"], cfg["dilation_max"],
         )
 
diff --git a/mast3r-slam-quality-dualtsdf_amd/mast3r_slam/tracker.py b/mast3r-slam-quality-dualtsdf_amd/mast3r_slam/tracker.py
--- a/mast3r-slam-quality-dualtsdf_amd/mast3r_slam/tracker.py
+++ b/mast3r-slam-quality-dualtsdf_amd/mast3r_slam/tracker.py
@@ -8,7 +8,7 @@
 from lietorch_hip import Sim3
 from mast3r_slam.config import config
 from mast3r_slam.geometry import act_Sim3, constrain_points_to_ray, point_to_ray_dist
-from mast3r_slam.mast3r_utils import mast3r_match_asymmetric
+from mast3r_slam.mast3r_utils import mast3r_match_asymmetric, release_pair_decode
 
 
 class _Pending:
@@ -189,6 +189,7 @@
 
     def track_finish(self, h):
         frame = h.frame
+        release_pair_decode(frame, keep=h.kind == "skip" or h.new_kf)
         if h.kind == "skip":
             frame.T_WC = h.init_T
             if self._shadow is h.shadow:
```

Result: no change. 163.9 (median of 4 runs) (-0.2%).
